# nh273/caro-ai

Hardware: AMD Instinct MI355X
Metric: self-play MCTS node-expansions/sec/GPU (Connect4, 200 sims/move); 1->8 GPU scaling (higher is better)
Workload: dtype f32

## Files before the change

### caro_ai_amd/_lib.py

```python
import ctypes as C
import os

_HERE = os.path.dirname(os.path.abspath(__file__))
LIB_PATH = os.path.join(_HERE, "libcaro_hip.so")
if os.environ.get("CARO_HIP_LIB"):
    LIB_PATH = os.environ["CARO_HIP_LIB"]

GAME_CONNECT4, GAME_MNK, GAME_CARO = 0, 1, 2
RESIGNED = -2


class CaroError(RuntimeError):
    pass


class CaroConfig(C.Structure):
    _fields_ = [
        ("game_kind", C.c_int32), ("n", C.c_int32), ("k", C.c_int32), ("n_games", C.c_int32),
        ("n_stores", C.c_int32), ("n_nets", C.c_int32), ("max_batch", C.c_int32), ("node_cap", C.c_int32),
        ("steps_before_tau_0", C.c_int32), ("first_player_mode", C.c_int32),
        ("c_puct", C.c_float), ("alpha", C.c_double), ("explore", C.c_double),
        ("seed", C.c_uint64), ("uid_base", C.c_uint64), ("uid_stride", C.c_uint64),
        ("device_id", C.c_int32), ("evict", C.c_int32), ("stagger", C.c_int32), ("stagger_recycle", C.c_int32),
        ("games_limit", C.c_int64),
# ... 37 lines not shown
    "caro_leaf_counts": (C.c_int, [_P, _P, _P]),
    "caro_leaf_counts_dev": (C.c_int, [_P, _P]),
    "caro_net_packed_size": (C.c_int64, [C.c_int, C.c_int, C.c_int]),
    "caro_net_create": (C.c_int, [C.c_int, C.c_int, C.c_int, C.c_float, _P, C.c_int64, C.c_int, _P]),
    "caro_net_max_depth": (C.c_int, []),
    "caro_net_packed_size_depth": (C.c_int64, [C.c_int, C.c_int, C.c_int, C.c_int]),
    "caro_net_create_depth": (C.c_int, [C.c_int, C.c_int, C.c_int, C.c_int, C.c_float, _P, C.c_int64, C.c_int, _P]),
    "caro_net_depth": (C.c_int, [_P]),
    "caro_net_winograd_size_depth": (C.c_int64, [C.c_int]),
    "caro_net_winograd2d_size_depth": (C.c_int64, [C.c_int]),
    "caro_net_split_bf16_size_depth": (C.c_int64, [C.c_int]),
    "caro_net_destroy": (None, [_P]),
    "caro_net_enable_winograd": (C.c_int, [_P, _P, C.c_int64]),
    "caro_net_winograd2d_size": (C.c_int, []),
    "caro_net_winograd2d_supported": (C.c_int, [C.c_int, C.c_int]),
    "caro_net_enable_winograd2d": (C.c_int, [_P, _P, C.c_int64]),
    "caro_net_split_bf16_size": (C.c_int64, []),
    "caro_net_enable_split_bf16": (C.c_int, [_P, _P, C.c_int64]),
    "caro_net_boards_per_workgroup": (C.c_int, [_P]),
    "caro_net_uses_slot_list": (C.c_int, [_P]),
    "caro_net_stream_evictions": (C.c_int64, [_P]),
    "caro_net_forward": (C.c_int, [_P, _P, _P, C.c_int, C.c_int64, _P, _P, _P]),
    "caro_stream_create_partition": (C.c_int, [C.c_int, C.c_int, C.c_int, _P]),
    "caro_stream_destroy": (C.c_int, [_P]),
    "caro_search_batch": (C.c_int, [_P, _P, _P, C.c_int, C.c_int, _P, _P, _P, _P, _P, _P]),
    "caro_search_move": (C.c_int, [_P, _P, _P, C.c_int, C.c_int] + [_P] * 10),
    "caro_net_forward_pair": (C.c_int, [_P, _P, _P, _P, C.c_int64, _P, _P, _P]),
    "caro_net_forward_pair_at": (C.c_int, [_P, _P, _P, _P, C.c_int64, C.c_int64, _P, _P, _P]),
    "caro_net_forward_slots": (C.c_int, [_P, _P, _P, _P, _P, C.c_int, C.c_int, _P, _P, _P]),
    "caro_net_forward_slot_list": (C.c_int, [_P, _P, _P, _P, _P, _P, C.c_int, C.c_int, _P, _P, _P]),
    "caro_net_create_hash": (C.c_int, [C.c_int, C.c_int, C.c_int, C.c_uint64, C.c_int, _P]),
    "caro_net_forward_stamped": (C.c_int, [_P, _P, _P, C.c_int, C.c_int64, _P, _P, _P, _P]),
    "caro_net_debug_stamps": (C.c_int, [_P, _P]),
    "caro_get_descent": (C.c_int, [_P, C.c_int, C.c_int, _P, _P, _P, _P, _P, _P]),
    "caro_select_cancel": (C.c_int, [_P]),
    "caro_expand_backup": (C.c_int, [_P, _P, _P, _P]),
    "caro_policy": (C.c_int, [_P, _P, _P, _P]),
    "caro_step": (C.c_int, [_P, _P, _P, _P, _P, _P]),
    "caro_drain_tuples": (C.c_int, [_P, C.c_int64, _P, _P, _P, _P, _P, C.c_int, _P, _P, _P]),
    "caro_drain_tuples_begin": (C.c_int, [_P, C.c_int64, _P, _P, _P, _P, _P, C.c_int, _P]),
    "caro_drain_tuples_end": (C.c_int, [_P, _P, _P]),
    "caro_search_staggered": (C.c_int, [_P, _P, _P, C.c_int, C.c_int, _P, _P, _P, _P, _P]),
    "caro_drain_parked_begin": (C.c_int, [_P, C.c_int64, _P, _P, _P, _P, _P, _P]),
    "caro_engine_set_resign": (C.c_int, [_P, C.c_double, C.c_double]),
    "caro_drain_tuples_begin_q": (C.c_int, [_P, C.c_int64, _P, _P, _P, _P, _P, C.c_int, _P, _P]),
    "caro_drain_parked_begin_q": (C.c_int, [_P, C.c_int64, _P, _P, _P, _P, _P, _P, _P]),
    "caro_engine_set_playout_cap": (C.c_int, [_P, C.c_double, C.c_int]),
    "caro_drain_tuples_begin_x": (C.c_int, [_P, C.c_int64, _P, _P, _P, _P, _P, C.c_int, _P, _P, _P]),
    "caro_drain_parked_begin_x": (C.c_int, [_P, C.c_int64, _P, _P, _P, _P, _P, _P, _P, _P]),
    "caro_engine_set_early_stop": (C.c_int, [_P, C.c_int]),
    "caro_drain_tuples_begin_ex": (C.c_int, [_P, C.c_int64, _P, _P, _P, _P, _P, C.c_int, C.POINTER(CaroDrainExtra), _P]),
    "caro_drain_parked_begin_ex": (C.c_int, [_P, C.c_int64, _P, _P, _P, _P, _P, C.POINTER(CaroDrainExtra), _P]),
    "caro_counters": (C.c_int, [_P, _P, _P]),
    "caro_live_games": (C.c_int, [_P, _P, _P]),
    "caro_pending_leaves": (C.c_int, [_P, _P, _P]),
    "caro_debug_stamps": (C.c_int, [_P, C.c_int]),
    "caro_debug_read": (C.c_int, [_P, _P, C.c_int64, _P]),
    "caro_debug_sqrt_check": (C.c_int, [C.c_uint32, _P]),
    "caro_profile_enable": (C.c_int, [_P, C.c_int]),
    "caro_profile_read": (C.c_int, [_P, _P, _P, C.c_int]),
    "caro_profile_begin": (C.c_int, [_P, C.c_int, _P]),
    "caro_profile_end": (None, [_P, C.c_int, _P]),
    "caro_tree_sizes": (C.c_int, [_P, _P, _P]),
    "caro_tree_live": (C.c_int, [_P, _P, _P]),
    "caro_lookup_nodes": (C.c_int, [_P, C.c_int64] + [_P] * 10),
    "caro_get_roots": (C.c_int, [_P] * 6),
    "caro_poke_nodes": (C.c_int, [_P, C.c_int64] + [_P] * 9),
    "caro_backup_path": (C.c_int, [_P, C.c_int, C.c_int, C.c_float, C.c_int, C.c_int, _P, _P, _P]),
    "caro_dump_tree": (C.c_int, [_P, C.c_int, C.c_int, C.c_int64] + [_P] * 8),
}
EXPORTS = sorted(_SIGNATURES)

_lib = None


def load():
    global _lib
    if _lib is not None:
        return _lib
    if not os.path.exists(LIB_PATH):
        raise CaroError("%s is missing: build it with `python -m caro_ai_amd.build` "
                        "(hipcc --offload-arch=gfx950); there is no CPU fallback" % LIB_PATH)
    try:
        lib = C.CDLL(LIB_PATH)
    except OSError as e:
        raise CaroError("cannot load %s: %s" % (LIB_PATH, e))
    for name, (res, args) in _SIGNATURES.items():
        fn = getattr(lib, name)
        fn.restype = res
        fn.argtypes = args
    _lib = lib
    return lib


def check(rc):
    if rc != 0:
        msg = load().caro_last_error()
        raise CaroError("libcaro_hip error %d: %s" % (rc, msg.decode() if msg else "?"))
```

### caro_ai_amd/csrc/caro_engine.hip

```cpp
#include <hip/hip_runtime.h>

#include <cstddef>
#include <cstdio>
#include <cstdlib>
#include <cstring>
#include <string>
#include <type_traits>
#include <vector>

#include "../../include/caro_hip.h"
#include "../../include/caro_noise.h"
#include "caro_rules.h"
#include "caro_variants.h"

namespace caro {

constexpr uint32_t NSTRONG = 1u << 30;
constexpr uint32_t NMASK = NSTRONG - 1u;
constexpr int ST_DROPPED = 0, ST_TERMINAL = 1, ST_LEAF = 2;
constexpr int MAXB = 64;

enum Counter { C_SIMS, C_LEVELS, C_EXPANSIONS, C_TERMINALS, C_DROPPED, C_OVERFLOW, C_PLIES, C_FINISHED, C_N };

struct View {
  GameParams gp;
  int G, n_stores, n_nets, cap, hcap, A, HW, maxply, maxd, maxB, sbt0, first_mode, ntab, etab;
  int tstride;
  uint32_t slot_rot;
  float c_puct;
  double alpha, explore;
  uint64_t seed, uid_base, uid_stride;
  long long games_limit;
  int32_t* tbl;
  uint64_t* node_key;
  uint32_t* edges;
  int32_t* n_nodes;
  int32_t* n_created;
  uint64_t* root;
  int32_t* player;
  int32_t* ply;
  int32_t* step;
  uint64_t* uid;
  int32_t* done;
  int32_t* result;
  int32_t* final_r;
  int32_t* first;
  uint64_t* h_key;
  int32_t* h_player;
  double* h_pi;
  double* h_q;
  int q_on;
  double resign_t, resign_p;
  int cap_on, cap_fast;
  double cap_p;
  uint8_t* fast;
  uint8_t* h_full;
  int es_on, es_min, ls_M;
  uint8_t* es_cut;
  uint16_t* es_cnt;
  uint16_t* h_mb;
  uint4* d_rec;
  uint4* path_rec;
  uint64_t* d_key;
  int32_t* g_nleaf;
  int32_t* g_off;
  int32_t* g_tree;
  int32_t* g_class;
  int32_t* g_pack;
  int32_t* slot_list;
  int32_t* leaf_count;
  unsigned long long* counters;
  unsigned long long* counters_sum;
  unsigned long long* dbg;
  int stag_S;
  int stag_recycle;
  int stag_pool;
  int32_t* handed;
  int32_t* lm;
  int32_t* pend;
  int32_t* wait;
  int32_t* dirty;
  int32_t* pk_flag;
  int32_t* pk_ply; int32_t* pk_final_r; int32_t* pk_first; int32_t* pk_result; int32_t* pk_step;
  uint64_t* pk_uid;
  uint64_t* ph_key; int32_t* ph_player; double* ph_pi; double* ph_q; uint8_t* ph_full; uint16_t* ph_mb;
  int32_t* dr_off;
  int32_t* dr_gidx;
  int32_t* dr_sel;
  int64_t* dr_tot;
};

template <class R>
__device__ __forceinline__ typename R::Board load_board(const uint64_t* p) {
  typename R::Board b;
#pragma unroll
  for (int i = 0; i < R::KW; ++i) b.w[i] = p[i];
  return b;
}
template <class R>
__device__ __forceinline__ void store_board(uint64_t* p, const typename R::Board& b) {
#pragma unroll
  for (int i = 0; i < R::KW; ++i) p[i] = b.w[i];
}

__device__ __forceinline__ size_t tbase(const View& v, int t) {
  return (size_t)(t * v.ntab + (v.ntab == 2 ? v.tbl[t] : 0)) * (size_t)v.tstride;
}
__device__ __forceinline__ size_t ebase(const View& v, int t) {
  return (size_t)(t * v.etab + (v.etab == 2 ? v.tbl[t] : 0)) * (size_t)v.tstride;
}

constexpr uint64_t EMPTY_KEY = ~0ULL;

template <class R>
__device__ __forceinline__ uint32_t home_slot(const View& v, int t, const typename R::Board& b) {
  return ((uint32_t)R::hash(b) + (uint32_t)t * v.slot_rot) & ((uint32_t)v.hcap - 1u);
}

__device__ __forceinline__ uint8_t cap_is_fast(const View& v, uint64_t uid, int ply) {
  return caro_cap_uniform(v.seed, uid, (uint32_t)ply) < v.cap_p ? 0 : 1;
}
__device__ __forceinline__ void es_ply_start(const View& v, int g) {
  v.es_cut[g] = 0;
  v.es_cnt[g] = 0;
}

template <class GEO>
struct GameRegs {
  typename GEO::R::Board root;
  int done, player, ply, step;
  int tbl[2], nn[2];
  uint64_t uid;
};
template <class GEO>
__device__ __forceinline__ GameRegs<GEO> load_game(const View& v, int g) {
  using R = typename GEO::R;
  GameRegs<GEO> r;
  r.done = v.done[g];
  r.player = v.player[g];
  r.ply = v.ply[g];
  r.step = v.step[g];
  r.uid = v.uid[g];
  r.root = load_board<R>(v.root + (size_t)g * GEO::KW);
#pragma unroll
  for (int st = 0; st < 2; ++st) {
    const int t = g * v.n_stores + (st < v.n_stores ? st : 0);
    r.tbl[st] = v.ntab == 2 ? v.tbl[t] : 0;
    r.nn[st] = v.n_nodes[t];
  }
  return r;
}
__device__ __forceinline__ size_t tbase_sel(const View& v, int t, int sel) {
  return (size_t)(t * v.ntab + sel) * (size_t)v.tstride;
}
__device__ __forceinline__ size_t ebase_sel(const View& v, int t, int sel) {
  return (size_t)(t * v.etab + (v.etab == 2 ? sel : 0)) * (size_t)v.tstride;
}

template <bool ONE>
__device__ __forceinline__ void block_sync() {
  if constexpr (ONE) {
    asm volatile("" ::: "memory");
    __builtin_amdgcn_wave_barrier();
  } else {
    __syncthreads();
  }
}
template <bool ONE>
__device__ __forceinline__ int block_threads() { return ONE ? 64 : (int)blockDim.x; }

template <class R>
__device__ __forceinline__ int probe_from(const View& v, int t, const typename R::Board& b, uint32_t i) {
  const uint32_t mask = (uint32_t)v.hcap - 1u;
  const uint64_t* keys = v.node_key + tbase(v, t) * R::KW;
  for (int it = 0; it < v.hcap; ++it) {
    const uint64_t* k = keys + (size_t)i * R::KW;
    const uint64_t k0 = k[0];
// ... 343 lines not shown
    d.status = ST_TERMINAL;
    d.value = -1.0f;
    return false;
  }
  if (R::full(v.gp, d.cur)) {
    d.status = ST_TERMINAL;
    d.value = 0.0f;
    return false;
  }
  return d.depth < v.maxd;
}

template <class GEO>
__device__ __forceinline__ void early_stop_test(const View& v, int g, int B, int m, bool root_in, const NodeRow<GEO>& r,
                                                int l, int tid) {
  constexpr int LPD = GEO::LPD, APL = GEO::APL;
  int M = v.stag_S ? v.stag_S : v.ls_M;
  if (v.cap_on && v.fast[g]) M = v.cap_fast < M ? v.cap_fast : M;
  if (m < v.es_min || m > M - 2) return;
  int n[APL];
  int ln = -1, la = 0x7fffffff;
#pragma unroll
  for (int j = 0; j < APL; ++j) {
    const int a = l * APL + j;
    n[j] = (root_in && a < v.A) ? (int)(r.nraw[j] & NMASK) : (a < v.A ? 0 : -1);
    if (n[j] > ln) {
      ln = n[j];
      la = a;
    }
  }
  auto imax = [](int x, int y) { return x > y ? x : y; };
  const int n1 = group_allreduce_i32<LPD>(ln, imax);
  const int best = group_allreduce_i32<LPD>(ln == n1 ? la : 0x7fffffff, [](int x, int y) { return x < y ? x : y; });
  int l2 = 0;
#pragma unroll
  for (int j = 0; j < APL; ++j) l2 = (l * APL + j != best && n[j] > l2) ? n[j] : l2;
  const int n2 = group_allreduce_i32<LPD>(l2, imax);
  if (tid == 0 && n1 - n2 > (M - m) * B) v.es_cut[g] = 1;
}

extern __shared__ double caro_dyn_lds[];
template <class GEO>
static inline size_t mail_bytes(int B) {
  return GEO::APL > 1 ? (size_t)((B * GEO::LPD + 63) / 64) * (2 * GEO::AP) * sizeof(double) : 0;
}

template <class GEO>
constexpr int geo_max_batch() { return GEO::LPD >= 64 ? 16 : GEO::LPD >= 32 ? 32 : 64; }

template <class GEO, bool ONE = false>
__device__ __forceinline__ void select_body(const View& v, const GameRegs<GEO>& gr, int B, int mb_index,
                                            const double* __restrict__ noise, int32_t* __restrict__ rows,
                                            float* __restrict__ planes, uint64_t* __restrict__ leaf_keys,
                                            const double* helper_nz = nullptr, volatile int* helper_flag = nullptr) {
  using R = typename GEO::R;
  using Board = typename R::Board;
  constexpr int LPD = GEO::LPD, APL = GEO::APL, AP = GEO::AP, KW = GEO::KW;
  const int g = blockIdx.x;
  const int tid = threadIdx.x;
  const int b = tid / LPD, l = tid % LPD;
  const int first = (tid & 63) - l;

  constexpr int MB = geo_max_batch<GEO>();
  __shared__ uint64_t s_key[MB][KW];
  __shared__ int s_status[MB];
  __shared__ int s_first[MB];
  __shared__ int s_depth[MB];
  __shared__ int s_player[MB];
  __shared__ float s_value[MB];
  __shared__ uint32_t s_dhome[MB];

  if (gr.done || (v.cap_on && !v.stag_S && mb_index >= v.cap_fast && v.fast[g]) ||
      (v.es_on && v.ls_M && mb_index > 0 && v.es_cut[g])) {
    if (tid == 0) {
      v.g_nleaf[g] = 0;
      v.g_class[g] = 0;
      if (rows) v.g_pack[g] = 0;
    }
    return;
  }
  unsigned long long st0 = 0, st_noise = 0, st_root = 0, st_loop = 0;
  if (v.dbg) st0 = __builtin_amdgcn_s_memtime();
  Descent<GEO> d;
  d.cur = gr.root;
  d.aux = R::aux_of(v.gp, d.cur);
  d.lk = R::lane_k(v.gp, l);
  const int player0 = gr.player;
  d.player = player0;
  d.depth = 0;
  d.status = ST_LEAF;
  d.value = 0.0f;
  d.home = 0u;
  const int st_sel = v.n_stores == 2 ? player0 : 0;
  const int t = g * v.n_stores + st_sel;
  const int A = v.A;
  uint4* prec = v.path_rec + ((size_t)g * v.maxB + b) * v.maxd;
  const int tsel = st_sel ? gr.tbl[1] : gr.tbl[0];
  const size_t tb = tbase_sel(v, t, tsel);
  const uint64_t* tkeys = v.node_key + tb * KW;
  const uint32_t* tedges = v.edges + ebase_sel(v, t, tsel) * 4 * AP;

  NodeRow<GEO> r;
  load_row<GEO, true>(r, tkeys, tedges, home_slot<R>(v, t, d.cur), l);
  double nz[APL];
  if (noise) {
#pragma unroll
    for (int j = 0; j < APL; ++j) {
      const int a = l * APL + j;
      nz[j] = a < A ? noise[((size_t)g * B + b) * A + a] : 0.0;
    }
  } else if (helper_nz) {
    while (*helper_flag == 0) __builtin_amdgcn_s_sleep(2);
    __builtin_amdgcn_fence(__ATOMIC_ACQUIRE, "workgroup");
#pragma unroll
    for (int j = 0; j < APL; ++j) nz[j] = helper_nz[b * AP + l * APL + j];
  } else {
    const uint64_t key = caro_noise_key(v.seed, gr.uid, (uint32_t)gr.ply, (uint32_t)(mb_index * B + b));
    noise_group<LPD, APL>(key, l, A, v.alpha, nz, APL > 1 ? caro_dyn_lds + (tid >> 6) * (2 * AP) : nullptr);
  }
  if (v.dbg) st_noise = __builtin_amdgcn_s_memtime();

  constexpr int PREC_LDS = GEO::APL > 1 ? 1 : 512;
  __shared__ uint4 s_prec[PREC_LDS];
  const bool stage = B * v.maxd <= PREC_LDS;
  uint4* lprec = stage ? s_prec + b * v.maxd : nullptr;
  bool live = descend_level<GEO, true>(v, d, t, tkeys, tedges, prec, lprec, l, first, nz, r);
  if (v.es_on) {
    if (tid == 0) {
      v.es_cnt[g] = (uint16_t)(mb_index + 1);
      if (v.ls_M && mb_index == 0) v.es_cut[g] = 0;
    }
    if (v.sbt0 == 0 || gr.step >= v.sbt0) early_stop_test<GEO>(v, g, B, mb_index, d.depth > 0, r, l, tid);
  }
  if (v.dbg) st_root = __builtin_amdgcn_s_memtime();
  while (live) live = descend_level<GEO, false>(v, d, t, tkeys, tedges, prec, lprec, l, first, nullptr, r);
  if (stage) {
    __builtin_amdgcn_wave_barrier();
    for (int i = l; i < d.depth; i += LPD) prec[i] = s_prec[b * v.maxd + i];
  }
  if (v.dbg) st_loop = __builtin_amdgcn_s_memtime();

  if constexpr (ONE) {
    const bool head = l == 0;
    const int st = d.status;
    bool dup = false;
    for (int o = 0; o < B; ++o) {
      const int src = o * LPD;
      bool eq = o < b && __builtin_amdgcn_readlane(st, src) == ST_LEAF;
#pragma unroll
      for (int w = 0; w < KW; ++w) {
        const uint32_t lo = (uint32_t)__builtin_amdgcn_readlane((int)(uint32_t)d.cur.w[w], src);
        const uint32_t hi = (uint32_t)__builtin_amdgcn_readlane((int)(uint32_t)(d.cur.w[w] >> 32), src);
        eq = eq && ((((uint64_t)hi << 32) | lo) == d.cur.w[w]);
      }
      dup = dup || eq;
    }
    const bool first_seen = st == ST_LEAF && !dup;
    const unsigned long long m_first = __ballot(head && first_seen);
    const unsigned long long m_term = __ballot(head && st == ST_TERMINAL);
    const unsigned long long m_drop = __ballot(head && st == ST_LEAF && dup);
    const int my_rank = __popcll(m_first & ((1ull << tid) - 1ull));
    const int levels = group_sum_i32<64>(head ? d.depth : 0);
    int maxdep = 0;
    if (v.dbg) maxdep = group_allreduce_i32<64>(d.depth, [](int x, int y) { return x > y ? x : y; });
    if (head) {
      const size_t di = (size_t)g * v.maxB + b;
      const uint32_t stw = (uint32_t)((st == ST_LEAF && dup) ? ST_DROPPED : st);
      v.d_rec[di] = make_uint4(stw | ((uint32_t)d.depth << 8) | ((uint32_t)my_rank << 16) | ((uint32_t)d.player << 24),
                               __float_as_uint(d.value), d.home, 0u);
      store_board<R>(v.d_key + di * KW, d.cur);
    }
    const int nleaf = __popcll(m_first);
    if (tid == 0) {
      v.g_nleaf[g] = nleaf;
      v.g_tree[g] = t;
      v.g_class[g] = v.n_nets == 2 ? player0 : 0;
      if (v.dbg) {
        unsigned long long* dd = v.dbg + (size_t)g * 8;
        dd[0] = st_noise - st0; dd[1] = st_root - st0; dd[2] = st_loop - st0;
        dd[3] = __builtin_amdgcn_s_memtime() - st0; dd[4] = (unsigned long long)maxdep;
      }
      unsigned long long* ctr = v.counters + (size_t)g * C_N;
      atomicAdd(ctr + C_SIMS, (unsigned long long)B);
      atomicAdd(ctr + C_LEVELS, (unsigned long long)levels);
      atomicAdd(ctr + C_TERMINALS, (unsigned long long)__popcll(m_term));
      atomicAdd(ctr + C_DROPPED, (unsigned long long)__popcll(m_drop));
      if (rows) {
        const int cls = v.n_nets == 2 ? player0 : 0;
        if (nleaf) atomicAdd(rows + cls, nleaf);
        v.g_off[g] = g * B;
        v.g_pack[g] = nleaf | (cls << 8);
      }
    }
    if (rows) {
      const int HW = v.HW;
      int local = 0;
      typename R::PlaneAt pat[R::PLANE_ITEMS];
#pragma unroll
      for (int k = 0; k < R::PLANE_ITEMS; ++k) pat[k] = R::plane_at(v.gp, tid + 64 * k < 2 * HW ? tid + 64 * k : 0);
      for (unsigned long long m = m_first; m; m &= m - 1ull) {
        const int src = __ffsll(m) - 1;
        Board brd;
#pragma unroll
        for (int w = 0; w < KW; ++w) {
          const uint32_t lo = (uint32_t)__builtin_amdgcn_readlane((int)(uint32_t)d.cur.w[w], src);
          const uint32_t hi = (uint32_t)__builtin_amdgcn_readlane((int)(uint32_t)(d.cur.w[w] >> 32), src);
          brd.w[w] = ((uint64_t)hi << 32) | lo;
        }
        const int who = __builtin_amdgcn_readlane(d.player, src);
        const int rowi = g * B + local++;
        float* dst = planes + (size_t)rowi * 2 * HW;
#pragma unroll
        for (int k = 0; k < R::PLANE_ITEMS; ++k)
          if (tid + 64 * k < 2 * HW) dst[tid + 64 * k] = R::plane_val(brd, who, pat[k]);
        if (leaf_keys && tid < KW) {
          uint64_t kw = brd.w[0];
#pragma unroll
          for (int w = 1; w < KW; ++w) kw = tid == w ? brd.w[w] : kw;
          leaf_keys[(size_t)rowi * KW + tid] = kw;
        }
      }
    }
    return;
  }
  if (l == 0) {
#pragma unroll
    for (int w = 0; w < KW; ++w) s_key[b][w] = d.cur.w[w];
    s_status[b] = d.status;
    s_depth[b] = d.depth;
    s_player[b] = d.player;
    s_value[b] = d.value;
    s_dhome[b] = d.home;
  }
  block_sync<ONE>();
  if (tid < 64) {
    const int bb = tid;
    const bool mine = bb < B;
    const int st = mine ? s_status[bb] : ST_DROPPED;
    const int dep = mine ? s_depth[bb] : 0;
    Board key;
#pragma unroll
    for (int w = 0; w < KW; ++w) key.w[w] = mine ? s_key[bb][w] : 0ull;
    bool dup = false;
// ... 121 lines not shown
    const int who = (int)(rx >> 24);
    float* dst = planes + (size_t)rowi * 2 * HW;
    for (int i = tid; i < 2 * HW; i += blockDim.x) dst[i] = R::plane(v.gp, brd, who, i / HW, i % HW);
    if (leaf_keys && tid < KW) leaf_keys[(size_t)rowi * KW + tid] = v.d_key[di * KW + tid];
  }
}

template <int AP>
__device__ __forceinline__ void backup_path(const View& v, int t, float value, bool strong_val, const int32_t* pn,
                                            const int32_t* pa, int len) {
  float cur = -value;
  for (int i = len - 1; i >= 0; --i) {
    uint32_t* row = v.edges + (ebase(v, t) + pn[i]) * 4 * AP;
    const int a = pa[i];
    const uint32_t nraw = row[4 * a];
    const int n = (int)(nraw & NMASK) + 1;
    const uint32_t strong = (nraw & NSTRONG) | (strong_val ? NSTRONG : 0u);
    const float w = __uint_as_float(row[4 * a + 1]) + cur;
    const float q = w / (float)n;
    row[4 * a] = (uint32_t)n | strong;
    row[4 * a + 1] = __float_as_uint(w);
    row[4 * a + 2] = __float_as_uint(q);
    cur = -cur;
  }
}
template <int AP>
__device__ __forceinline__ void backup_path_rec(const View& v, int t, float value, bool strong_val, const uint4* rec,
                                                int len) {
  float cur = -value;
  for (int i = len - 1; i >= 0; --i) {
    const uint32_t na = rec[i].x;
    uint32_t* row = v.edges + (ebase(v, t) + (na & 0xFFFFFFu)) * 4 * AP;
    const int a = (int)(na >> 24);
    const uint32_t nraw = row[4 * a];
    const int n = (int)(nraw & NMASK) + 1;
    const uint32_t strong = (nraw & NSTRONG) | (strong_val ? NSTRONG : 0u);
    const float w = __uint_as_float(row[4 * a + 1]) + cur;
    row[4 * a] = (uint32_t)n | strong;
    row[4 * a + 1] = __float_as_uint(w);
    row[4 * a + 2] = __float_as_uint(w / (float)n);
    cur = -cur;
  }
}

template <class GEO>
struct ExpandPre {
  static constexpr int NPR = (MAXB * 0 + 64 * GEO::APL + 63) / 64;
  uint4 rec;
  typename GEO::R::Board brd;
  float row_val;
  uint4 p0, p1;
  float pr[NPR];
  int nleaf;
};
template <class GEO, bool ONE>
__device__ __forceinline__ ExpandPre<GEO> expand_preload(const View& v, int g, int B, int off, const float* __restrict__ probs,
                                                         const float* __restrict__ values) {
  using R = typename GEO::R;
  constexpr int KW = GEO::KW, AP = GEO::AP;
  ExpandPre<GEO> e;
  const int lane = threadIdx.x;
  e.nleaf = v.g_nleaf[g];
  e.rec = make_uint4(ST_DROPPED, 0u, 0u, 0u);
  e.row_val = 0.f;
#pragma unroll
  for (int w = 0; w < KW; ++w) e.brd.w[w] = 0;
  if (lane < B) {
    const size_t di = (size_t)g * v.maxB + lane;
    e.rec = v.d_rec[di];
    e.brd = load_board<R>(v.d_key + di * KW);
    if ((long long)off + lane < (long long)v.G * v.maxB) e.row_val = values[off + lane];
  }
  e.p0 = e.p1 = make_uint4(0u, 0u, 0u, 0u);
  if (B <= 8 && lane < 64 && (lane >> 3) < B) {
    const uint4* pr = v.path_rec + ((size_t)g * v.maxB + (lane >> 3)) * v.maxd;
    if ((lane & 7) < v.maxd) e.p0 = pr[lane & 7];
    if (8 + (lane & 7) < v.maxd) e.p1 = pr[8 + (lane & 7)];
  }
#pragma unroll
  for (int k = 0; k < ExpandPre<GEO>::NPR; ++k) {
    e.pr[k] = 0.f;
    if (ONE) {
      const int idx = lane + 64 * k, b = idx / AP, a = idx - b * AP;
      if (idx < B * AP && a < v.A && lane < 64) e.pr[k] = probs[(size_t)(off + b) * v.A + a];
    }
  }
  return e;
}

template <class GEO, bool ONE = false>
__device__ __forceinline__ void expand_body(const View& v, GameRegs<GEO>& gr, int B, const ExpandPre<GEO>& pre, int off,
                                            const float* __restrict__ probs) {
  using R = typename GEO::R;
  using Board = typename R::Board;
  constexpr int AP = GEO::AP, KW = GEO::KW;
  constexpr int MAXE = GEO::APL > 1 ? 256 : 512;
  constexpr int MAXB = geo_max_batch<GEO>();
  __shared__ int e_node[MAXE];
  __shared__ short e_act[MAXE];
  __shared__ float e_val[MAXE];
  __shared__ unsigned char e_strong[MAXE];
  __shared__ uint32_t e_n[MAXE], e_w[MAXE];
  __shared__ int s_total;
  __shared__ uint64_t s_brd[MAXB][KW];
  __shared__ int s_node[MAXB], s_row[MAXB];
  __shared__ uint32_t s_home[MAXB];
  __shared__ unsigned char s_free[MAXB];
  __shared__ int q_len[MAXB], q_off[MAXB], q_b[MAXB];
  __shared__ float q_val[MAXB];
  __shared__ unsigned char q_strong[MAXB];
  __shared__ int s_nq;
  __shared__ uint4 s_p0[64], s_p1[64];
  __shared__ float s_rowval[MAXB];
  const int g = blockIdx.x;
  if (gr.done) return;
  const int lane = threadIdx.x;
  unsigned long long* xs = v.dbg ? v.dbg + ((size_t)v.G + g) * 8 : nullptr;
#define CARO_XS(n) if (xs && lane == 0) xs[n] = __builtin_amdgcn_s_memtime();
  CARO_XS(0)
  const int st_sel = v.n_stores == 2 ? gr.player : 0;
  const int t = g * v.n_stores + st_sel;
  const int nleaf = pre.nleaf;
  const int base = st_sel ? gr.nn[1] : gr.nn[0];
  const bool overflow = base + nleaf > v.cap;
  const int A = v.A;
  const int tsel = st_sel ? gr.tbl[1] : gr.tbl[0];
  const size_t tb = tbase_sel(v, t, tsel);
  const size_t eb = ebase_sel(v, t, tsel);
  const int my_st = (int)(pre.rec.x & 0xFFu), my_len = (int)((pre.rec.x >> 8) & 0xFFu);
  const int my_local = (int)((pre.rec.x >> 16) & 0xFFu);
  const uint32_t my_home = pre.rec.z;
  float my_val = __uint_as_float(pre.rec.y);
  const Board& brd = pre.brd;
  const bool pre_paths = B <= 8 && block_threads<ONE>() >= 64;
  if (pre_paths && lane < 64) {
    s_p0[lane] = pre.p0;
    s_p1[lane] = pre.p1;
  }
  const bool is_leaf = lane < B && my_st == ST_LEAF && !overflow;
  if (lane < B) s_rowval[lane] = pre.row_val;
  block_sync<ONE>();
  if (lane < B) {
    s_node[lane] = -2;
    if (is_leaf) {
      my_val = s_rowval[my_local];
      s_home[lane] = my_home & 0x7fffffffu;
      s_free[lane] = (my_home >> 31) != 0u;
      s_row[lane] = off + my_local;
      s_node[lane] = -1;
#pragma unroll
      for (int w = 0; w < KW; ++w) s_brd[lane][w] = brd.w[w];
    }
  }
  block_sync<ONE>();
  CARO_XS(1)
  const bool whole_wave = ONE || blockDim.x >= 64;
  const bool wave0 = whole_wave && lane < 64;
  if (!overflow) {
    if (wave0) {
      bool clash = false;
      for (int bb = 0; bb < B; ++bb) {
        const int ob = __builtin_amdgcn_readlane((int)is_leaf, bb);
        const uint32_t oh = (uint32_t)__builtin_amdgcn_readlane((int)(my_home & 0x7fffffffu), bb);
        clash = clash || (bb < lane && ob && oh == (my_home & 0x7fffffffu));
      }
      const bool fast = is_leaf && (my_home >> 31) != 0u && !clash;
      if (fast) {
        uint64_t* k = v.node_key + (tb + (my_home & 0x7fffffffu)) * KW;
#pragma unroll
        for (int w = KW - 1; w >= 0; --w) k[w] = brd.w[w];
        s_node[lane] = (int)(my_home & 0x7fffffffu);
      }
      const unsigned long long slow = __ballot(is_leaf && !fast);
      if (slow) {
        asm volatile("" ::: "memory");
        __builtin_amdgcn_wave_barrier();
        if (lane == 0)
          for (unsigned long long m = slow; m; m &= m - 1ull) {
            const int b = __ffsll(m) - 1;
            Board lb;
#pragma unroll
            for (int w = 0; w < KW; ++w) lb.w[w] = s_brd[b][w];
            s_node[b] = insert_key<R>(v, t, lb);
          }
      }
    } else if (!whole_wave && lane == 0) {
      for (int b = 0; b < B; ++b) {
        if (s_node[b] == -2) continue;
        Board lb;
#pragma unroll
        for (int w = 0; w < KW; ++w) lb.w[w] = s_brd[b][w];
        s_node[b] = insert_key<R>(v, t, lb);
      }
    }
    if (lane == 0) {
      unsigned long long* ctr = v.counters + (size_t)g * C_N;
      v.n_nodes[t] = base + nleaf;
      atomicAdd(v.n_created + t, nleaf);
      atomicAdd(ctr + C_EXPANSIONS, (unsigned long long)nleaf);
    }
    if (st_sel) gr.nn[1] = base + nleaf;
    else gr.nn[0] = base + nleaf;
  } else if (lane == 0) {
    atomicAdd(v.counters + (size_t)g * C_N + C_OVERFLOW, 1ull);
  }
  CARO_XS(2)
  const unsigned long long m_term = __ballot(lane < B && my_st == ST_TERMINAL);
  const unsigned long long m_leaf = __ballot(is_leaf);
  const int n_term = __popcll(m_term);
  const unsigned long long below = (1ull << lane) - 1ull;
  int qpos = -1;
  if (lane < B && my_st == ST_TERMINAL) qpos = __popcll(m_term & below);
  else if (is_leaf) qpos = n_term + __popcll(m_leaf & below);
  if (qpos >= 0) {
    q_len[qpos] = my_len;
    q_b[qpos] = lane;
    q_val[qpos] = my_val;
    q_strong[qpos] = my_st == ST_LEAF;
  }
  if (lane == 0) s_nq = n_term + __popcll(m_leaf);
  block_sync<ONE>();
  const int nq = s_nq;
  if (lane == 0) {
    int acc = 0;
    for (int k = 0; k < nq; ++k) {
      q_off[k] = acc;
      acc += q_len[k];
    }
    s_total = acc;
  }
  block_sync<ONE>();
  CARO_XS(3)
  const int total = s_total;
  if (total <= MAXE)
    for (int j = lane; j < total; j += block_threads<ONE>()) {
      int k = 0;
      while (k + 1 < nq && q_off[k + 1] <= j) ++k;
      const int r = j - q_off[k];
      const int i = q_len[k] - 1 - r;
      uint4 rec;
      if (pre_paths && i < 8) rec = s_p0[q_b[k] * 8 + i];
      else if (pre_paths && i < 16) rec = s_p1[q_b[k] * 8 + i - 8];
      else rec = v.path_rec[((size_t)g * v.maxB + q_b[k]) * v.maxd + i];
      e_node[j] = (int)(rec.x & 0xFFFFFFu);
      e_act[j] = (short)(rec.x >> 24);
      e_n[j] = rec.y;
      e_w[j] = rec.z;
      e_val[j] = (r & 1) ? q_val[k] : -q_val[k];
      e_strong[j] = q_strong[k];
    }
  CARO_XS(4)
  if (!overflow)
    for (int idx = lane; idx < B * AP; idx += block_threads<ONE>()) {
      const int b = idx / AP, a = idx - b * AP;
      const int node = s_node[b];
      float pv = 0.f;
      if (ONE) {
        const int src = node >= 0 ? (s_row[b] - off) * AP + a : lane;
#pragma unroll
        for (int k = 0; k < ExpandPre<GEO>::NPR; ++k) {
          const float x = __shfl(pre.pr[k], src & 63, 64);
          pv = (src >> 6) == k ? x : pv;
        }
      } else if (node >= 0 && a < A) {
        pv = probs[(size_t)s_row[b] * A + a];
      }
      if (node < 0) continue;
      uint32_t* row = v.edges + (eb + node) * 4 * AP;
      if (a >= A) pv = 0.f;
      reinterpret_cast<uint4*>(row)[a] = make_uint4(0u, 0u, 0u, __float_as_uint(pv));
    }
  if (total > MAXE) {
    if (lane == 0)
      for (int k = 0; k < nq; ++k) {
        const size_t di = (size_t)g * v.maxB + q_b[k];
        backup_path_rec<AP>(v, t, q_val[k], q_strong[k] != 0, v.path_rec + di * v.maxd, q_len[k]);
      }
    return;
  }
  block_sync<ONE>();
  CARO_XS(5)
  const int n = total;
  if (whole_wave && n <= 128) {
    if (wave0) {
    const int j0 = lane, j1 = lane + 64;
    const bool v0 = j0 < n, v1 = j1 < n;
    const int key0 = v0 ? (e_node[j0] << 8) | (int)(unsigned short)e_act[j0] : -1;
    const int key1 = v1 ? (e_node[j1] << 8) | (int)(unsigned short)e_act[j1] : -1;
    unsigned long long todo0 = __ballot(v0), todo1 = __ballot(v1);
    bool own0 = false, own1 = false;
    unsigned long long g0m0 = 0ull, g0m1 = 0ull, g1m1 = 0ull;
    while (todo0 | todo1) {
      const bool lo = todo0 != 0ull;
      const int lead = lo ? __ffsll((unsigned long long)todo0) - 1 : __ffsll((unsigned long long)todo1) - 1;
      const int k = lo ? __builtin_amdgcn_readlane(key0, lead) : __builtin_amdgcn_readlane(key1, lead);
      const unsigned long long m0 = __ballot(v0 && key0 == k);
      const unsigned long long m1 = __ballot(v1 && key1 == k);
      if (lane == lead) {
        if (lo) { own0 = true; g0m0 = m0; g0m1 = m1; }
        else { own1 = true; g1m1 = m1; }
      }
      todo0 &= ~m0;
      todo1 &= ~m1;
    }
    uint32_t* row0 = own0 ? v.edges + (eb + (key0 >> 8)) * 4 * AP : nullptr;
    uint32_t* row1 = own1 ? v.edges + (eb + (key1 >> 8)) * 4 * AP : nullptr;
    const int a0 = key0 & 0xff, a1 = key1 & 0xff;
    if (own0) {
      const uint32_t n0 = e_n[j0];
      int cnt = (int)(n0 & NMASK);
      uint32_t strong = n0 & NSTRONG;
      float w = __uint_as_float(e_w[j0]);
      for (unsigned long long m = g0m0; m; m &= m - 1ull) {
        const int e = __ffsll(m) - 1;
        cnt += 1;
        w = w + e_val[e];
        if (e_strong[e]) strong = NSTRONG;
      }
      for (unsigned long long m = g0m1; m; m &= m - 1ull) {
        const int e = 64 + __ffsll(m) - 1;
        cnt += 1;
        w = w + e_val[e];
        if (e_strong[e]) strong = NSTRONG;
      }
// ... 22 lines not shown
    const int node = e_node[j], a = e_act[j];
    bool owner = true;
    for (int k = 0; k < j; ++k) owner = owner && !(e_node[k] == node && e_act[k] == a);
    if (!owner) continue;
    uint32_t* row = v.edges + (eb + node) * 4 * AP;
    const uint32_t nraw = e_n[j];
    int cnt = (int)(nraw & NMASK);
    uint32_t strong = nraw & NSTRONG;
    float w = __uint_as_float(e_w[j]);
    for (int k = j; k < n; ++k) {
      if (e_node[k] == node && e_act[k] == a) {
        cnt += 1;
        w = w + e_val[k];
        if (e_strong[k]) strong = NSTRONG;
      }
    }
    row[4 * a] = (uint32_t)cnt | strong;
    row[4 * a + 1] = __float_as_uint(w);
    row[4 * a + 2] = __float_as_uint(w / (float)cnt);
  }
  CARO_XS(6)
  if (xs && lane == 0) xs[7] = (unsigned long long)total;
#undef CARO_XS
}

template <class GEO>
__global__ void k_expand_backup(View v, const float* __restrict__ probs, const float* __restrict__ values) {
  GameRegs<GEO> gr = load_game<GEO>(v, blockIdx.x);
  const int B = v.leaf_count[2], off = v.g_off[blockIdx.x];
  const ExpandPre<GEO> pre = expand_preload<GEO, false>(v, blockIdx.x, B, off, probs, values);
  expand_body<GEO>(v, gr, B, pre, off, probs);
}

template <class GEO>
__device__ __forceinline__ void noise_wave(const View& v, int B, int go, uint64_t uid, uint32_t ply, int mb,
                                           double* s_nz, volatile int* s_flag) {
  constexpr int LPD = GEO::LPD, APL = GEO::APL, AP = GEO::AP;
  const int lane = threadIdx.x & 63;
  const int b = lane / LPD, l = lane % LPD;
  if (go) {
    double nz[APL];
    const uint64_t key = caro_noise_key(v.seed, uid, ply, (uint32_t)(mb * B + b));
    __shared__ double s_mail[APL > 1 ? 2 * AP : 1];
    noise_group<LPD, APL>(key, l, v.A, v.alpha, nz, s_mail);
#pragma unroll
    for (int j = 0; j < APL; ++j) s_nz[b * AP + l * APL + j] = nz[j];
  }
  __builtin_amdgcn_fence(__ATOMIC_RELEASE, "workgroup");
  __builtin_amdgcn_wave_barrier();
  if (lane == 0) *s_flag = 1;
}

template <class GEO>
__global__ void k_tree(View v, int B, int mb_index, const double* __restrict__ noise, const float* __restrict__ probs,
                       const float* __restrict__ values, float* __restrict__ planes, uint64_t* __restrict__ leaf_keys,
                       int32_t* __restrict__ rows_cur, int32_t* __restrict__ rows_next, int do_expand,
                       int do_select) {
  __shared__ double s_nz[MAXB * 0 + 64 * GEO::APL];
  __shared__ int s_flag;
  if (threadIdx.x == 0) s_flag = 0;
  __syncthreads();
  if (threadIdx.x >= 64) {
    const int g = blockIdx.x;
    const int go = do_select && !noise && !v.done[g] && !(v.cap_on && mb_index >= v.cap_fast && v.fast[g]) &&
                   !(v.es_on && mb_index > 0 && v.es_cut[g]);
    noise_wave<GEO>(v, B, go, go ? v.uid[g] : 0ull, go ? (uint32_t)v.ply[g] : 0u, mb_index, s_nz, &s_flag);
    return;
  }
  __builtin_amdgcn_s_setprio(3);
  if (blockIdx.x == 0 && threadIdx.x == 0) {
    rows_next[0] = 0;
    rows_next[1] = 0;
    rows_next[2] = B;
    rows_cur[2] = B;
  }
  unsigned long long t0 = 0;
  if (v.dbg) t0 = __builtin_amdgcn_s_memtime();
  GameRegs<GEO> gr = load_game<GEO>(v, blockIdx.x);
  const ExpandPre<GEO> pre = expand_preload<GEO, true>(v, blockIdx.x, B, blockIdx.x * B, probs, values);
  if (do_expand) {
    expand_body<GEO, true>(v, gr, B, pre, blockIdx.x * B, probs);
    block_sync<true>();
  }
  const unsigned long long t1 = v.dbg ? __builtin_amdgcn_s_memtime() : 0;
  if (v.dbg && threadIdx.x == 0 && !do_select) v.dbg[(size_t)blockIdx.x * 8 + 5] = t1 - t0;
  if (do_select) select_body<GEO, true>(v, gr, B, mb_index, noise, rows_cur, planes, leaf_keys, s_nz, &s_flag);
  if (v.dbg && threadIdx.x == 0 && do_select) {
    v.dbg[(size_t)blockIdx.x * 8 + 6] = t1 - t0;
    v.dbg[(size_t)blockIdx.x * 8 + 7] = __builtin_amdgcn_s_memtime() - t0;
  }
}

template <class GEO>
__device__ __forceinline__ void root_policy(const View& v, int g, int t, const typename GEO::R::Board& root,
                                            double* s_pi, int* s_n) {
  using R = typename GEO::R;
  constexpr int AP = GEO::AP;
  const int node = probe<R>(v, t, root);
  for (int a = threadIdx.x; a < AP; a += blockDim.x)
    s_n[a] = (node >= 0 && a < v.A) ? (int)(v.edges[((ebase(v, t) + node) * AP + a) * 4] & NMASK) : 0;
  __syncthreads();
  __shared__ int s_best;
  __shared__ double s_total;
  if (threadIdx.x == 0) {
    const int tau = (v.sbt0 > 0 && v.step[g] < v.sbt0) ? 1 : 0;
    int best = 0;
    long long tot = 0;
    for (int a = 0; a < v.A; ++a) {
      if (s_n[a] > s_n[best]) best = a;
      tot += s_n[a];
    }
    s_best = tau == 0 ? best : -1;
    s_total = (double)tot;
  }
  __syncthreads();
  for (int a = threadIdx.x; a < AP; a += blockDim.x) {
    double p = 0.0;
    if (a < v.A) p = s_best >= 0 ? (a == s_best ? 1.0 : 0.0) : (double)s_n[a] / s_total;
    s_pi[a] = p;
  }
  __syncthreads();
}

template <class GEO>
__global__ void k_policy(View v, double* __restrict__ pi_out, int32_t* __restrict__ counts_out) {
  using R = typename GEO::R;
  constexpr int AP = GEO::AP, KW = GEO::KW;
  __shared__ double s_pi[AP];
  __shared__ int s_n[AP];
  const int g = blockIdx.x;
  const typename R::Board root = load_board<R>(v.root + (size_t)g * KW);
  const int t = g * v.n_stores + (v.n_stores == 2 ? v.player[g] : 0);
  root_policy<GEO>(v, g, t, root, s_pi, s_n);
  for (int a = threadIdx.x; a < v.A; a += blockDim.x) {
    if (pi_out) pi_out[(size_t)g * v.A + a] = s_pi[a];
    if (counts_out) counts_out[(size_t)g * v.A + a] = s_n[a];
  }
}

// ... 417 lines not shown
    v.pk_step[g] = gr.step;
    v.pk_uid[g] = uid;
    v.pk_flag[g] = 1;
  }
  block_sync<ONE>();
  if (!v.stag_recycle || v.stag_pool || !game_wanted(v, g, uid + v.uid_stride)) {
    if (threadIdx.x == 0) v.done[g] = 2;
    gr.done = 2;
    return false;
  }
  const uint64_t nuid = uid + v.uid_stride;
  const int fp = v.first_mode == 2 ? (int)(nuid & 1ull) : v.first_mode;
  gr.root = R::initial(v.gp);
  gr.player = fp;
  gr.ply = 0;
  gr.step = 0;
  gr.uid = nuid;
  gr.done = 0;
  const bool flip = v.etab != 2;
#pragma unroll
  for (int st = 0; st < 2; ++st) {
    if (flip) gr.tbl[st] = 1 - gr.tbl[st];
    gr.nn[st] = 0;
  }
  if (threadIdx.x == 0) {
#pragma unroll
    for (int st = 0; st < 2; ++st) {
      if (st < v.n_stores) {
        const int t = g * v.n_stores + st;
        if (flip) {
          v.tbl[t] = gr.tbl[st];
          v.dirty[t] = 1;
        }
        v.n_nodes[t] = 0;
        v.n_created[t] = 0;
      }
    }
    store_board<R>(v.root + (size_t)g * KW, gr.root);
    v.player[g] = fp;
    v.first[g] = fp;
    v.ply[g] = 0;
    v.step[g] = 0;
    v.uid[g] = nuid;
    v.done[g] = 0;
    v.result[g] = 0;
    v.final_r[g] = 0;
    if (v.cap_on) v.fast[g] = cap_is_fast(v, nuid, 0);
    if (v.es_on) es_ply_start(v, g);
  }
  return true;
}

template <class GEO>
__global__ void k_tree_stag(View v, int B, const float* __restrict__ probs, const float* __restrict__ values,
                            float* __restrict__ planes, uint64_t* __restrict__ leaf_keys,
                            int32_t* __restrict__ rows_cur, int32_t* __restrict__ rows_next) {
  constexpr int AP = GEO::AP;
  __shared__ double s_pi[AP];
  __shared__ int s_n[AP];
  __shared__ double s_nz[64 * GEO::APL];
  __shared__ int s_flag;
  const int g = blockIdx.x;
  if (threadIdx.x == 0) s_flag = 0;
  const int w = v.wait[g];
  int lm = v.lm[g];
  const int pend = v.pend[g];
  const int due = (v.cap_on && v.fast[g]) ? v.cap_fast : v.stag_S;
  const int cut = v.es_on ? v.es_cut[g] : 0;
  GameRegs<GEO> gr = load_game<GEO>(v, g);
  ExpandPre<GEO> pre;
  if (threadIdx.x < 64) pre = expand_preload<GEO, true>(v, g, B, g * B, probs, values);
  __syncthreads();
  if (threadIdx.x >= 64) {
    const int go = w == 0 && gr.done == 0;
    int lm_h = go ? lm : 0;
    uint32_t ply_h = go ? (uint32_t)gr.ply : 0u;
    if (lm_h >= due || (go && cut)) {
      lm_h = 0;
      ply_h += 1u;
    }
    noise_wave<GEO>(v, B, go, go ? gr.uid : 0ull, ply_h, lm_h, s_nz, &s_flag);
    return;
  }
  __builtin_amdgcn_s_setprio(3);
  if (blockIdx.x == 0 && threadIdx.x == 0) {
    rows_next[0] = 0;
    rows_next[1] = 0;
    rows_next[2] = B;
    rows_cur[2] = B;
  }
  const unsigned long long t0 = v.dbg ? __builtin_amdgcn_s_memtime() : 0;
  if (w > 0) {
    if (threadIdx.x == 0) {
      v.wait[g] = w - 1;
      v.g_nleaf[g] = 0;
      v.g_class[g] = 0;
      v.g_pack[g] = 0;
    }
    return;
  }
  if (gr.done == 2) {
    if (threadIdx.x == 0) {
      v.g_nleaf[g] = 0;
      v.g_class[g] = 0;
      v.g_pack[g] = 0;
    }
    return;
  }
  if (pend) {
    expand_body<GEO, true>(v, gr, B, pre, g * B, probs);
    block_sync<true>();
  }
  const unsigned long long t1 = v.dbg ? __builtin_amdgcn_s_memtime() : 0;
  int over = gr.done == 1;
  if (!over && (lm >= due || cut)) {
    over = step_body<GEO, true>(v, g, gr, nullptr, s_pi, s_n, nullptr, nullptr, nullptr);
    lm = 0;
  }
  if (over) {
    if (park_and_restart<GEO>(v, g, gr)) over = 0;
  }
  const unsigned long long t2 = v.dbg ? __builtin_amdgcn_s_memtime() : 0;
  select_body<GEO, true>(v, gr, B, lm, nullptr, rows_cur, planes, leaf_keys, s_nz, &s_flag);
  if (threadIdx.x == 0) {
    v.lm[g] = over ? 0 : lm + 1;
    v.pend[g] = over ? 0 : 1;
    if (v.dbg) {
      v.dbg[(size_t)g * 8 + 5] = ((t2 - t1) & 0xFFFFFFull) | (__builtin_amdgcn_s_memrealtime() << 24);
      v.dbg[(size_t)g * 8 + 6] = t1 - t0;
      v.dbg[(size_t)g * 8 + 7] = __builtin_amdgcn_s_memtime() - t0;
      v.dbg[(size_t)g * 8 + 4] |= (unsigned long long)__builtin_amdgcn_s_getreg((31 << 11) | 4) << 8;
    }
  }
}

template <class GEO>
__global__ void k_tree_stag_mw(View v, int B, const float* __restrict__ probs, const float* __restrict__ values,
                               float* __restrict__ planes, uint64_t* __restrict__ leaf_keys,
                               int32_t* __restrict__ rows_cur, int32_t* __restrict__ rows_next) {
  constexpr int AP = GEO::AP;
  __shared__ double s_pi[AP];
  __shared__ int s_n[AP];
  const int g = blockIdx.x;
  if (g == 0 && threadIdx.x == 0) {
    rows_next[0] = 0;
    rows_next[1] = 0;
    rows_next[2] = B;
    rows_cur[2] = B;
  }
  const int w = v.wait[g];
  int lm = v.lm[g];
  const int pend = v.pend[g];
  const int due = (v.cap_on && v.fast[g]) ? v.cap_fast : v.stag_S;
  const int cut = v.es_on ? v.es_cut[g] : 0;
  GameRegs<GEO> gr = load_game<GEO>(v, g);
  const ExpandPre<GEO> pre = expand_preload<GEO, false>(v, g, B, g * B, probs, values);
  __syncthreads();
  if (w > 0 || gr.done == 2) {
    if (threadIdx.x == 0) {
      if (w > 0) v.wait[g] = w - 1;
      v.g_nleaf[g] = 0;
      v.g_class[g] = 0;
      v.g_pack[g] = 0;
    }
    return;
  }
  if (pend) {
    expand_body<GEO, false>(v, gr, B, pre, g * B, probs);
    __syncthreads();
  }
  int over = gr.done == 1;
  if (!over && (lm >= due || cut)) {
    over = step_body<GEO>(v, g, gr, nullptr, s_pi, s_n, nullptr, nullptr, nullptr);
    lm = 0;
    if (v.etab == 2) {
      __syncthreads();
// ... 426 lines not shown
template <class GEO>
__global__ void k_noise(uint64_t seed, long long M, int A, double alpha, const uint64_t* uid, const uint32_t* ply,
                        const uint32_t* sim, double* out) {
  constexpr int LPD = GEO::LPD, APL = GEO::APL;
  const int grp = threadIdx.x / LPD, l = threadIdx.x % LPD;
  const long long m = (long long)blockIdx.x * (blockDim.x / LPD) + grp;
  const long long mm = m < M ? m : M - 1;
  const uint64_t key = caro_noise_key(seed, uid[mm], ply[mm], sim[mm]);
  double nz[APL];
  __shared__ double s_mail[APL > 1 ? 2 * GEO::AP : 1];
  noise_group<LPD, APL>(key, l, A, alpha, nz, s_mail);
  if (m < M)
    for (int j = 0; j < APL; ++j) {
      const int a = l * APL + j;
      if (a < A) out[(size_t)m * A + a] = nz[j];
    }
}

}

using namespace caro;

static thread_local std::string g_err;
static int fail(int code, const std::string& msg) {
  g_err = msg;
  return code;
}
#define HIPCHK(x)                                                                                  \
  do {                                                                                             \
    hipError_t e_ = (x);                                                                           \
    if (e_ != hipSuccess)                                                                          \
      return fail(CARO_E_HIP, std::string(#x) + ": " + hipGetErrorString(e_));                     \
  } while (0)

struct caro_engine {
  caro_config cfg;
  Variant var;
  View v;
  std::vector<void*> allocs;
  int32_t* pinned;
  int64_t* pinned64;
  int32_t* scratch;
  int32_t* live;
  int select_pending;
  int drain_pending;
  int ls_mid;
  int stag_batch;
  hipEvent_t drain_ev;
  int prof_on;
  int prof_gate;
  uint64_t prof_ctr;
  uint64_t prof_cal;
  int32_t* rows;
  int rows_par;
  int fused_ok;
  std::vector<hipEvent_t> ev;
  std::vector<int> ev_kind;
  size_t ev_used;
  double prof_ms[8];
  long long prof_n[8];
};

constexpr unsigned PROF_EVERY = 23;
enum ProfKind { PK_SELECT = 0, PK_COMPACT = 1, PK_EXPAND = 2, PK_STEP = 3, PK_NET = 4, PK_NULL1 = 5, PK_NULL2 = 6, PK_N = 8 };
__global__ void k_prof_null() {}
static void prof_calibrate(caro_engine* h, hipStream_t st);

static void prof_flush(caro_engine* h) {
  for (size_t i = 0; i < h->ev_used; ++i) {
    float ms = 0.f;
    if (hipEventSynchronize(h->ev[2 * i + 1]) == hipSuccess &&
        hipEventElapsedTime(&ms, h->ev[2 * i], h->ev[2 * i + 1]) == hipSuccess) {
      h->prof_ms[h->ev_kind[i]] += ms;
      h->prof_n[h->ev_kind[i]] += 1;
    }
  }
  h->ev_used = 0;
}
static int prof_begin(caro_engine* h, int kind, hipStream_t st) {
  if (!h->prof_on || !h->prof_gate) return -1;
  if (h->ev_used * 2 + 2 > h->ev.size()) {
    if (h->ev.size() >= 2 * 16384) prof_flush(h);
    else
      for (int i = 0; i < 512; ++i) {
        hipEvent_t e;
        if (hipEventCreate(&e) != hipSuccess) return -1;
        h->ev.push_back(e);
      }
  }
  const int i = (int)h->ev_used++;
  if ((size_t)i >= h->ev_kind.size()) h->ev_kind.resize(i + 1);
  h->ev_kind[i] = kind;
  (void)hipEventRecord(h->ev[2 * i], st);
  return i;
}
static void prof_end(caro_engine* h, int i, hipStream_t st) {
  if (i >= 0) (void)hipEventRecord(h->ev[2 * i + 1], st);
}
static void prof_calibrate(caro_engine* h, hipStream_t st) {
  if (!h->prof_on || !h->prof_gate || (h->prof_cal++ & 3)) return;
  const int a = prof_begin(h, PK_NULL1, st);
  hipLaunchKernelGGL(k_prof_null, dim3(1), dim3(64), 0, st);
  prof_end(h, a, st);
  const int b = prof_begin(h, PK_NULL2, st);
  hipLaunchKernelGGL(k_prof_null, dim3(1), dim3(64), 0, st);
  hipLaunchKernelGGL(k_prof_null, dim3(1), dim3(64), 0, st);
  prof_end(h, b, st);
}

template <class T>
static int dalloc(caro_engine* h, T** p, size_t n) {
  void* q = nullptr;
  hipError_t e = hipMalloc(&q, n * sizeof(T) + 256);
  if (e != hipSuccess) return fail(CARO_E_NOMEM, std::string("hipMalloc failed: ") + hipGetErrorString(e));
  h->allocs.push_back(q);
  *p = (T*)q;
  return 0;
}

extern "C" {

const char* caro_last_error(void) { return g_err.c_str(); }
void caro__set_error(const char* msg) { g_err = msg ? msg : ""; }
int caro_version(void) { return 101; }

#include "caro_host.inc"

int caro_rules_move_batch(int kind, int n, int k, int64_t M, uint64_t* keys, const int32_t* moves,
                          const int32_t* players, int32_t* won, int32_t* full, void* stream) {
  const Variant var = pick_variant(kind, n);
  const GameParams gp = make_gp(kind, n, k);
  if (M <= 0) return 0;
  const unsigned grid = (unsigned)((M + 255) / 256);
  DISPATCH(var, hipLaunchKernelGGL(k_rules_move<GEO>, dim3(grid), dim3(256), 0, (hipStream_t)stream, gp,
                                   (long long)M, keys, moves, players, won, full));
  HIPCHK(hipGetLastError());
  return 0;
}
int caro_rules_legal_batch(int kind, int n, int k, int64_t M, const uint64_t* keys, uint8_t* legal, void* stream) {
  const Variant var = pick_variant(kind, n);
  const GameParams gp = make_gp(kind, n, k);
  if (M <= 0) return 0;
  const unsigned grid = (unsigned)((M * gp.A + 255) / 256);
  DISPATCH(var, hipLaunchKernelGGL(k_rules_legal<GEO>, dim3(grid), dim3(256), 0, (hipStream_t)stream, gp,
                                   (long long)M, keys, legal));
  HIPCHK(hipGetLastError());
  return 0;
}
int caro_rules_encode_batch(int kind, int n, int k, int64_t M, const uint64_t* keys, const int32_t* who,
                            float* planes, void* stream) {
  const Variant var = pick_variant(kind, n);
  const GameParams gp = make_gp(kind, n, k);
  if (M <= 0) return 0;
  const unsigned grid = (unsigned)((M * 2 * gp.rows * gp.cols + 255) / 256);
  DISPATCH(var, hipLaunchKernelGGL(k_rules_encode<GEO>, dim3(grid), dim3(256), 0, (hipStream_t)stream, gp,
                                   (long long)M, keys, who, planes));
  HIPCHK(hipGetLastError());
  return 0;
}
int caro_noise_batch(uint64_t seed, int64_t M, int A, double alpha, const uint64_t* uid, const uint32_t* ply,
                     const uint32_t* sim, double* out, void* stream) {
  if (M <= 0) return 0;
  Variant var = A == 7 ? V_C4 : A <= 16 ? V_M16 : A <= 32 ? V_M32 : A <= 64 ? V_M64 : A <= 128 ? V_M128 : V_M256;
  if (A > 256) return fail(CARO_E_INVAL, "A out of range");
  const int lpd = variant_lpd(var);
  const int per_block = 64 / lpd;
  const unsigned grid = (unsigned)((M + per_block - 1) / per_block);
  DISPATCH(var, hipLaunchKernelGGL(k_noise<GEO>, dim3(grid), dim3(64), 0, (hipStream_t)stream, seed, (long long)M, A,
                                   alpha, uid, ply, sim, out));
  HIPCHK(hipGetLastError());
  return 0;
}

static int reset_games_impl(caro_engine* h, const int32_t* first_player_dev, void* stream);
static void apply_run_params(caro_engine* h, const caro_config* cfg) {
  View& v = h->v;
  v.sbt0 = cfg->steps_before_tau_0;
  v.first_mode = cfg->first_player_mode;
  v.c_puct = cfg->c_puct;
  v.alpha = cfg->alpha;
  v.explore = cfg->explore;
  v.seed = cfg->seed;
  v.uid_base = cfg->uid_base;
  v.uid_stride = cfg->uid_stride ? cfg->uid_stride : (uint64_t)cfg->n_games;
  v.games_limit = cfg->games_limit > 0 ? (long long)cfg->games_limit : 0;
  if (cfg->stagger > 0) {
    v.stag_S = cfg->stagger;
    v.stag_recycle = cfg->stagger_recycle ? 1 : 0;
    v.stag_pool = (cfg->stagger_recycle == 2 && cfg->games_limit > 0) ? 1 : 0;
  }
}
static int fresh_state(caro_engine* h, hipStream_t st) {
  View& v = h->v;
  const size_t T = (size_t)v.G * v.n_stores, G = (size_t)v.G;
  HIPCHK(hipMemsetAsync(v.counters, 0, sizeof(unsigned long long) * C_N * G, st));
  HIPCHK(hipMemsetAsync(v.leaf_count, 0, sizeof(int32_t) * 4, st));
  HIPCHK(hipMemsetAsync(h->rows, 0, sizeof(int32_t) * 8, st));
  HIPCHK(hipMemsetAsync(v.g_nleaf, 0, sizeof(int32_t) * G, st));
  HIPCHK(hipMemsetAsync(v.g_pack, 0, sizeof(int32_t) * G, st));
  h->rows_par = 0;
  h->stag_batch = 0;
  const int rc = reset_games_impl(h, nullptr, st);
  if (rc) return rc;
  if (v.stag_S) {
    HIPCHK(hipMemsetAsync(v.dirty, 0, sizeof(int32_t) * T, st));
    hipLaunchKernelGGL(k_stag_init, dim3((v.G + 255) / 256), dim3(256), 0, st, v);
    HIPCHK(hipGetLastError());
  }
  return 0;
}
int caro_engine_create(const caro_config* cfg, caro_engine** out) {
  if (!cfg || !out) return fail(CARO_E_INVAL, "null argument");
  const Variant var = pick_variant(cfg->game_kind, cfg->n);
  if (var == V_BAD) return fail(CARO_E_INVAL, "unsupported game (connect four, or m,n,k / caro with 2 <= n <= 15)");
  if (cfg->n_games < 1) return fail(CARO_E_INVAL, "n_games must be >= 1");
  if (cfg->n_stores != 1 && cfg->n_stores != 2) return fail(CARO_E_INVAL, "n_stores must be 1 or 2");
  if (cfg->n_nets != 1 && cfg->n_nets != 2) return fail(CARO_E_INVAL, "n_nets must be 1 or 2");
  const int lpd = variant_lpd(var);
  if (cfg->max_batch < 1 || cfg->max_batch > MAXB || cfg->max_batch * lpd > 1024)
    return fail(CARO_E_INVAL, "max_batch out of range for this game (batch * lanes-per-descent <= 1024, batch <= 64)");
  if ((cfg->game_kind == CARO_GAME_MNK || cfg->game_kind == CARO_GAME_CARO) && (cfg->k < 2 || cfg->k > cfg->n))
    return fail(CARO_E_INVAL, "k must satisfy 2 <= k <= n");
  if (cfg->stagger < 0) return fail(CARO_E_INVAL, "stagger must be >= 0");
  if (cfg->stagger > 0) {
    if (cfg->max_batch * lpd < 64 || (cfg->max_batch * lpd) % 64 != 0)
      return fail(CARO_E_INVAL, "staggered mode needs whole wavefronts per game (max_batch x lanes per descent a multiple of 64)");
    if (cfg->evict && cfg->max_batch * lpd == 64)
      return fail(CARO_E_INVAL, "staggered mode with eviction: the multi-wavefront kernel only (max_batch x lanes per descent > 64)");
  }
  int ndev = 0;
  if (hipGetDeviceCount(&ndev) != hipSuccess || ndev <= 0)
    return fail(CARO_E_NODEV, "no HIP device: libcaro_hip needs a GPU (there is no CPU fallback)");
  if (cfg->device_id < 0 || cfg->device_id >= ndev) return fail(CARO_E_INVAL, "device_id out of range");
  HIPCHK(hipSetDevice(cfg->device_id));

  caro_engine* h = new caro_engine();
  h->cfg = *cfg;
  h->var = var;
  h->select_pending = 0;
  h->ls_mid = 0;
  h->prof_on = 0;
  h->prof_gate = 1;
  h->prof_ctr = 0;
  h->prof_cal = 0;
  h->rows = nullptr;
  h->rows_par = 0;
  {
    const char* e = getenv("CARO_NO_FUSED_TREE");
    h->fused_ok = !(e && e[0] == '1');
  }
  h->ev_used = 0;
  for (int i = 0; i < 8; ++i) { h->prof_ms[i] = 0; h->prof_n[i] = 0; }
  View& v = h->v;
  memset(&v, 0, sizeof v);
  v.gp = make_gp(cfg->game_kind, cfg->n, cfg->k);
  v.G = cfg->n_games;
  v.n_stores = cfg->n_stores;
  v.n_nets = cfg->n_nets;
  v.A = v.gp.A;
  v.HW = v.gp.rows * v.gp.cols;
  v.maxply = v.HW;
  v.maxd = v.HW;
  v.maxB = cfg->max_batch;
  v.ntab = (cfg->evict || cfg->stagger > 0) ? 2 : 1;
  v.etab = cfg->evict ? 2 : 1;
  apply_run_params(h, cfg);
  v.cap = cfg->node_cap > 0 ? cfg->node_cap : 4096;
  static_assert(MAXB <= 255, "leaf rank travels in 8 bits of d_rec.x");
  if (v.cap > (1 << 23)) { delete h; return fail(CARO_E_INVAL, "node_cap too large: at most 2^23 nodes per tree (slot ids travel in 24 bits)"); }
  int hc = 64;
  while (hc < 2 * v.cap) hc <<= 1;
  v.hcap = hc;
  if (v.A > 256 || v.maxd > 255) { delete h; return fail(CARO_E_INVAL, "board too large for the path records (actions < 256, depth <= 255)"); }
  {
    const char* e = getenv("CARO_TREE_SKEW");
    const long skew = e ? strtol(e, nullptr, 0) : 0;
    if (skew < 0 || skew > 65536) { delete h; return fail(CARO_E_INVAL, "CARO_TREE_SKEW must be 0 .. 65536 slots"); }
    v.tstride = hc + (int)skew;
    e = getenv("CARO_SLOT_ROT");
    v.slot_rot = e ? (uint32_t)strtoul(e, nullptr, 0) : 0u;
  }
  const int KW = variant_kw(var), AP = variant_ap(var);
  const size_t T = (size_t)v.G * v.n_stores, G = (size_t)v.G;
  int rc = 0;
#define DA(p, n) if ((rc = dalloc(h, &p, (n))) != 0) { caro_engine_destroy(h); return rc; }
  DA(v.tbl, T);
  DA(v.node_key, T * v.ntab * v.tstride * KW);
  DA(v.edges, T * v.etab * v.tstride * 4 * AP);
  DA(v.n_nodes, T);
  DA(v.n_created, T);
  DA(v.root, G * KW);
  DA(v.player, G); DA(v.ply, G); DA(v.step, G); DA(v.uid, G); DA(v.done, G); DA(v.result, G); DA(v.final_r, G);
  DA(v.first, G);
  DA(v.h_key, G * v.maxply * KW);
  DA(v.h_player, G * v.maxply);
  DA(v.h_pi, G * v.maxply * v.A);
  DA(v.path_rec, G * v.maxB * v.maxd);
  DA(v.d_rec, G * v.maxB);
  DA(v.d_key, G * v.maxB * KW);
  DA(v.g_nleaf, G); DA(v.g_off, G); DA(v.g_tree, G); DA(v.g_class, G); DA(v.g_pack, G);
  DA(v.slot_list, 2 * G * v.maxB);
  DA(v.leaf_count, 4);
  DA(v.counters, G * C_N);
  DA(v.counters_sum, C_N);
  DA(v.dr_off, G); DA(v.dr_gidx, G); DA(v.dr_sel, G); DA(v.dr_tot, 2);
  DA(h->scratch, (size_t)v.maxd + 8);
  DA(h->live, 1);
  DA(h->rows, 8);
  if (cfg->stagger > 0) {
    DA(v.lm, G); DA(v.pend, G); DA(v.wait, G); DA(v.dirty, T);
    DA(v.pk_flag, G); DA(v.pk_ply, G); DA(v.pk_final_r, G); DA(v.pk_first, G); DA(v.pk_result, G); DA(v.pk_step, G);
    DA(v.pk_uid, G);
    DA(v.handed, 1);
    DA(v.ph_key, G * v.maxply * KW);
    DA(v.ph_player, G * v.maxply);
    DA(v.ph_pi, G * v.maxply * v.A);
  }
#undef DA
  HIPCHK(hipHostMalloc((void**)&h->pinned, 64, hipHostMallocDefault));
  HIPCHK(hipHostMalloc((void**)&h->pinned64, 128, hipHostMallocDefault));
  *out = h;
  rc = fresh_state(h, nullptr);
  if (rc) { caro_engine_destroy(h); *out = nullptr; return rc; }
  HIPCHK(hipDeviceSynchronize());
  return 0;
}

int caro_engine_restart(caro_engine* h, const caro_config* cfg, void* stream) {
  if (!h || !cfg) return fail(CARO_E_INVAL, "null argument");
  const caro_config& o = h->cfg;
  if (cfg->game_kind != o.game_kind || cfg->n != o.n || cfg->k != o.k || cfg->n_games != o.n_games ||
      cfg->n_stores != o.n_stores || cfg->n_nets != o.n_nets || cfg->max_batch != o.max_batch ||
      cfg->node_cap != o.node_cap || (cfg->evict != 0) != (o.evict != 0) || cfg->device_id != o.device_id ||
      (cfg->stagger > 0) != (o.stagger > 0))
    return fail(CARO_E_INVAL, "caro_engine_restart: the configuration differs from the engine's in a field that shapes its "
                              "memory (game, n_games, n_stores, n_nets, max_batch, node_cap, evict, device, staggered or not)");
  if (cfg->stagger < 0) return fail(CARO_E_INVAL, "stagger must be >= 0");
  if (h->drain_pending) return fail(CARO_E_STATE, "caro_engine_restart with a drain pending (caro_drain_tuples_end first)");
  if (h->select_pending) return fail(CARO_E_STATE, "caro_engine_restart with a pending caro_select");
  HIPCHK(hipSetDevice(o.device_id));
  h->cfg = *cfg;
  apply_run_params(h, cfg);
  return fresh_state(h, (hipStream_t)stream);
}

int caro_engine_set_resign(caro_engine* h, double threshold, double playthrough) {
  if (!h) return fail(CARO_E_INVAL, "null engine");
  if (!(threshold >= -1.0 && threshold <= 1.0)) return fail(CARO_E_INVAL, "resign threshold must be in [-1, 1]");
  if (!(playthrough >= 0.0 && playthrough <= 1.0)) return fail(CARO_E_INVAL, "resign playthrough must be in [0, 1]");
  View& v = h->v;
  if (!v.q_on) {
    HIPCHK(hipSetDevice(h->cfg.device_id));
    const size_t n = (size_t)v.G * v.maxply;
    int rc = dalloc(h, &v.h_q, n);
    if (rc) return rc;
    HIPCHK(hipMemset(v.h_q, 0, n * sizeof(double)));
    if (v.stag_S) {
      if ((rc = dalloc(h, &v.ph_q, n)) != 0) return rc;
      HIPCHK(hipMemset(v.ph_q, 0, n * sizeof(double)));
    }
    v.q_on = 1;
  }
  v.resign_t = threshold;
  v.resign_p = playthrough;
  return 0;
}

int caro_engine_set_playout_cap(caro_engine* h, double p_full, int fast) {
  if (!h) return fail(CARO_E_INVAL, "null engine");
  if (!(p_full >= 0.0 && p_full <= 1.0)) return fail(CARO_E_INVAL, "playout cap p_full must be in [0, 1]");
  if (fast < 2) return fail(CARO_E_INVAL, "playout cap fast must be >= 2 (a fast first ply must expand its root)");
  View& v = h->v;
  if (v.stag_S && fast > v.stag_S) return fail(CARO_E_INVAL, "playout cap fast must be <= caro_config.stagger");
// ... 83 lines not shown
  return 0;
}

static int select_impl(caro_engine* h, int batch, int mb_index, int budget, const double* noise, float* planes,
                       uint64_t* leaf_keys, void* stream);
int caro_select(caro_engine* h, int batch, int mb_index, const double* noise, float* planes, uint64_t* leaf_keys,
                void* stream) {
  return select_impl(h, batch, mb_index, 0, noise, planes, leaf_keys, stream);
}
static int select_impl(caro_engine* h, int batch, int mb_index, int budget, const double* noise, float* planes,
                       uint64_t* leaf_keys, void* stream) {
  if (!h || !planes) return fail(CARO_E_INVAL, "null argument");
  if (batch < 1 || batch > h->v.maxB) return fail(CARO_E_INVAL, "batch exceeds max_batch of the engine");
  if (h->v.stag_S) return fail(CARO_E_STATE, "caro_select: the engine runs in staggered mode (per-game clocks, pending minibatches, parked games); use caro_search_staggered / caro_drain_parked_begin");
  if (h->select_pending) return fail(CARO_E_STATE, "caro_select called twice without caro_expand_backup");
  const int lpd = variant_lpd(h->var);
  hipStream_t st = (hipStream_t)stream;
  const int p0 = prof_begin(h, PK_SELECT, st);
  View sv = h->v;
  sv.ls_M = budget;
  DISPATCH(h->var, hipLaunchKernelGGL(k_select<GEO>, dim3(h->v.G), dim3(batch * lpd), mail_bytes<GEO>(batch), st, sv,
                                      batch, mb_index, noise));
  prof_end(h, p0, st);
  const int p1 = prof_begin(h, PK_COMPACT, st);
  DISPATCH(h->var, hipLaunchKernelGGL(k_encode<GEO>, dim3(h->v.G), dim3(128), 0, st, h->v, batch, planes, leaf_keys));
  prof_end(h, p1, st);
  HIPCHK(hipGetLastError());
  h->select_pending = 1;
  h->ls_mid = 1;
  return 0;
}

int caro_leaf_counts(caro_engine* h, int32_t counts[2], void* stream) {
  if (!h || !counts) return fail(CARO_E_INVAL, "null argument");
  HIPCHK(hipMemcpyAsync(h->pinned, h->v.leaf_count, 2 * sizeof(int32_t), hipMemcpyDeviceToHost, (hipStream_t)stream));
  HIPCHK(hipStreamSynchronize((hipStream_t)stream));
  counts[0] = h->pinned[0];
  counts[1] = h->pinned[1];
  return 0;
}

int caro_expand_backup(caro_engine* h, const float* probs, const float* values, void* stream) {
  if (!h) return fail(CARO_E_INVAL, "null engine");
  if (!h->select_pending) return fail(CARO_E_STATE, "caro_expand_backup without a pending caro_select");
  const int p0 = prof_begin(h, PK_EXPAND, (hipStream_t)stream);
  DISPATCH(h->var, hipLaunchKernelGGL(k_expand_backup<GEO>, dim3(h->v.G), dim3(64), 0, (hipStream_t)stream, h->v,
                                      probs, values));
  prof_end(h, p0, (hipStream_t)stream);
  HIPCHK(hipGetLastError());
  h->select_pending = 0;
  return 0;
}

static int search_batch_impl(caro_engine* h, caro_net* net0, caro_net* net1, int searches, int batch, const double* noise,
                             float* planes, uint64_t* leaf_keys, float* probs, float* values, void* stream, int with_step,
                             const double* uniforms, int32_t* actions, int32_t* done, int32_t* result) {
  if (!h || !net0 || !planes || !probs || !values) return fail(CARO_E_INVAL, "null argument");
  if (h->v.n_nets == 2 && !net1) return fail(CARO_E_INVAL, "engine has two nets, net1 is null");
  if (searches < 1) return fail(CARO_E_INVAL, "searches must be >= 1");
  const int64_t max_rows = (int64_t)h->v.G * batch;
  const size_t noise_stride = (size_t)h->v.G * batch * h->v.A;
  if (batch < 1 || batch > h->v.maxB) return fail(CARO_E_INVAL, "batch exceeds max_batch of the engine");
  if (h->v.stag_S) return fail(CARO_E_STATE, "caro_search_batch: the engine runs in staggered mode (per-game clocks, pending minibatches, parked games); use caro_search_staggered / caro_drain_parked_begin");
  if (h->select_pending) return fail(CARO_E_STATE, "caro_search_batch with a pending caro_select");
  hipStream_t st = (hipStream_t)stream;
  const int bthreads = batch * variant_lpd(h->var);
  const bool fused1 = h->fused_ok && bthreads == 64;
  const bool fused = h->fused_ok && bthreads >= 64 && bthreads % 64 == 0;
  h->ls_mid = 1;
  View sv = h->v;
  sv.ls_M = searches;
  if (!caro_net_uses_slot_list(net0)) sv.slot_list = nullptr;
  for (int mb = 0; mb < searches; ++mb) {
    h->prof_gate = (h->prof_ctr++ % PROF_EVERY) == 0;
    int rc = 0;
    const int32_t* counts = h->v.leaf_count;
    if (fused) {
      int32_t* cur = h->rows + 4 * h->rows_par;
      int32_t* nxt = h->rows + 4 * (h->rows_par ^ 1);
      h->rows_par ^= 1;
      counts = cur;
      const int p1 = prof_begin(h, PK_SELECT, st);
      if (fused1) {
        DISPATCH(h->var, hipLaunchKernelGGL(k_tree<GEO>, dim3(h->v.G), dim3(128), 0, st, sv, batch, mb,
                                            noise ? noise + (size_t)mb * noise_stride : nullptr, probs, values, planes,
                                            leaf_keys, cur, nxt, mb > 0 ? 1 : 0, 1));
      } else {
        DISPATCH(h->var, hipLaunchKernelGGL(k_tree_mw<GEO>, dim3(h->v.G), dim3(bthreads), mail_bytes<GEO>(batch), st,
                                            sv, batch, mb, noise ? noise + (size_t)mb * noise_stride : nullptr, probs,
                                            values, planes, leaf_keys, cur, nxt, mb > 0 ? 1 : 0, 1, 0,
                                            (const double*)nullptr, (int32_t*)nullptr, (int32_t*)nullptr,
                                            (int32_t*)nullptr));
      }
      prof_end(h, p1, st);
      if (hipGetLastError() != hipSuccess) { h->prof_gate = 1; return fail(CARO_E_HIP, "k_tree launch failed"); }
    } else {
      rc = select_impl(h, batch, mb, searches, noise ? noise + (size_t)mb * noise_stride : nullptr, planes, leaf_keys,
                       stream);
      if (rc) { h->prof_gate = 1; return rc; }
    }
    const int p0 = prof_begin(h, PK_NET, st);
    if (fused)
      rc = caro_net_forward_slot_list(net0, h->v.n_nets == 2 ? net1 : nullptr, planes, counts, h->v.g_pack,
                                      fused1 ? nullptr : sv.slot_list, h->v.G, batch, probs, values, stream);
    else if (h->v.n_nets == 2)
      rc = caro_net_forward_pair_at(net0, net1, planes, counts, -1, max_rows, probs, values, stream);
    else rc = caro_net_forward(net0, planes, counts, 0, max_rows, probs, values, stream);
    prof_end(h, p0, st);
    prof_calibrate(h, st);
    if (!rc && !fused) rc = caro_expand_backup(h, probs, values, stream);
    if (rc) { h->prof_gate = 1; return rc; }
  }
  if (fused) {
    int32_t* cur = h->rows + 4 * h->rows_par;
    int32_t* nxt = h->rows + 4 * (h->rows_par ^ 1);
    h->rows_par ^= 1;
    const int p1 = prof_begin(h, PK_EXPAND, st);
    if (fused1) {
      DISPATCH(h->var, hipLaunchKernelGGL(k_tree<GEO>, dim3(h->v.G), dim3(128), 0, st, h->v, batch, searches,
                                          (const double*)nullptr, probs, values, planes, leaf_keys, cur, nxt, 1, 0));
    } else {
      DISPATCH(h->var, hipLaunchKernelGGL(k_tree_mw<GEO>, dim3(h->v.G), dim3(bthreads), 0, st, h->v, batch, searches,
                                          (const double*)nullptr, probs, values, planes, leaf_keys, cur, nxt, 1, 0,
                                          with_step ? 1 : 0, uniforms, actions, done, result));
      if (with_step) {
        with_step = 0;
        h->ls_mid = 0;
      }
    }
    prof_end(h, p1, st);
    if (hipGetLastError() != hipSuccess) { h->prof_gate = 1; return fail(CARO_E_HIP, "k_tree launch failed"); }
  }
  h->prof_gate = 1;
  return with_step ? caro_step(h, uniforms, actions, done, result, stream) : 0;
}

int caro_search_batch(caro_engine* h, caro_net* net0, caro_net* net1, int searches, int batch, const double* noise,
                      float* planes, uint64_t* leaf_keys, float* probs, float* values, void* stream) {
  return search_batch_impl(h, net0, net1, searches, batch, noise, planes, leaf_keys, probs, values, stream, 0, nullptr,
                           nullptr, nullptr, nullptr);
}

int caro_search_move(caro_engine* h, caro_net* net0, caro_net* net1, int searches, int batch, const double* noise,
                     const double* uniforms, float* planes, uint64_t* leaf_keys, float* probs, float* values,
                     int32_t* actions, int32_t* done, int32_t* result, void* stream) {
  return search_batch_impl(h, net0, net1, searches, batch, noise, planes, leaf_keys, probs, values, stream, 1, uniforms,
                           actions, done, result);
}

int caro_search_staggered(caro_engine* h, caro_net* net0, caro_net* net1, int launches, int batch, float* planes,
                          uint64_t* leaf_keys, float* probs, float* values, void* stream) {
  if (!h || !net0 || !planes || !probs || !values) return fail(CARO_E_INVAL, "null argument");
  if (!h->v.stag_S) return fail(CARO_E_STATE, "the engine was not created in staggered mode (caro_config.stagger)");
  if (h->v.n_nets == 2 && !net1) return fail(CARO_E_INVAL, "engine has two nets, net1 is null");
  if (launches < 1) return fail(CARO_E_INVAL, "launches must be >= 1");
  const int bthreads = batch * variant_lpd(h->var);
  if (batch < 1 || batch > h->v.maxB || bthreads < 64 || bthreads % 64 != 0)
    return fail(CARO_E_INVAL, "staggered mode: batch x lanes per descent must be a multiple of 64");
  if (h->cfg.evict && bthreads == 64)
    return fail(CARO_E_INVAL, "staggered mode with eviction: batch x lanes per descent must be above 64");
  if (h->stag_batch && h->stag_batch != batch) return fail(CARO_E_INVAL, "staggered mode: the batch size is fixed by the first call");
  h->stag_batch = batch;
  hipStream_t st = (hipStream_t)stream;
  View sv = h->v;
  if (!caro_net_uses_slot_list(net0)) sv.slot_list = nullptr;
  for (int j = 0; j < launches; ++j) {
    h->prof_gate = (h->prof_ctr++ % PROF_EVERY) == 0;
    int32_t* cur = h->rows + 4 * h->rows_par;
    int32_t* nxt = h->rows + 4 * (h->rows_par ^ 1);
    h->rows_par ^= 1;
    const int p1 = prof_begin(h, PK_SELECT, st);
    if (bthreads == 64) {
      DISPATCH(h->var, hipLaunchKernelGGL(k_tree_stag<GEO>, dim3(h->v.G), dim3(128), 0, st, h->v, batch, probs, values,
                                          planes, leaf_keys, cur, nxt));
    } else {
      DISPATCH(h->var, hipLaunchKernelGGL(k_tree_stag_mw<GEO>, dim3(h->v.G), dim3(bthreads), mail_bytes<GEO>(batch), st,
                                          sv, batch, probs, values, planes, leaf_keys, cur, nxt));
    }
    prof_end(h, p1, st);
    if (hipGetLastError() != hipSuccess) { h->prof_gate = 1; return fail(CARO_E_HIP, "k_tree_stag launch failed"); }
    const int p0 = prof_begin(h, PK_NET, st);
    const int rc = caro_net_forward_slot_list(net0, h->v.n_nets == 2 ? net1 : nullptr, planes, cur, h->v.g_pack,
                                              bthreads == 64 ? nullptr : sv.slot_list, h->v.G, batch, probs, values,
                                              stream);
    prof_end(h, p0, st);
    prof_calibrate(h, st);
    if (rc) { h->prof_gate = 1; return rc; }
    if (h->v.stag_pool && j % 5 == 4)
      DISPATCH(h->var, hipLaunchKernelGGL(k_stag_assign<GEO>, dim3(1), dim3(1024), 0, st, h->v));
  }
  h->prof_gate = 1;
  return 0;
}

int caro_drain_parked_begin(caro_engine* h, int64_t cap, uint64_t* states, int32_t* players, double* pi, int32_t* z,
                            int64_t* games, void* stream) {
  return caro_drain_parked_begin_q(h, cap, states, players, pi, z, games, nullptr, stream);
}
int caro_drain_parked_begin_q(caro_engine* h, int64_t cap, uint64_t* states, int32_t* players, double* pi, int32_t* z,
                              int64_t* games, double* root_q, void* stream) {
  return caro_drain_parked_begin_x(h, cap, states, players, pi, z, games, root_q, nullptr, stream);
}
int caro_drain_parked_begin_x(caro_engine* h, int64_t cap, uint64_t* states, int32_t* players, double* pi, int32_t* z,
                              int64_t* games, double* root_q, uint8_t* full, void* stream) {
  caro_drain_extra ex = {(uint32_t)sizeof(caro_drain_extra), root_q, full, nullptr};
  return caro_drain_parked_begin_ex(h, cap, states, players, pi, z, games, &ex, stream);
}
static int drain_extra(const caro_drain_extra* in, caro_drain_extra* out) {
  *out = caro_drain_extra{(uint32_t)sizeof(caro_drain_extra), nullptr, nullptr, nullptr};
  if (!in) return 0;
  if (in->size < offsetof(caro_drain_extra, root_q_dev)) return fail(CARO_E_INVAL, "caro_drain_extra.size is not set");
  if (in->size >= offsetof(caro_drain_extra, root_q_dev) + sizeof(double*)) out->root_q_dev = in->root_q_dev;
  if (in->size >= offsetof(caro_drain_extra, full_dev) + sizeof(uint8_t*)) out->full_dev = in->full_dev;
  if (in->size >= offsetof(caro_drain_extra, minibatches_dev) + sizeof(uint16_t*)) out->minibatches_dev = in->minibatches_dev;
  return 0;
}
int caro_drain_parked_begin_ex(caro_engine* h, int64_t cap, uint64_t* states, int32_t* players, double* pi, int32_t* z,
                               int64_t* games, const caro_drain_extra* extra, void* stream) {
  if (!h || !states || !players || !pi || !z) return fail(CARO_E_INVAL, "null argument");
  caro_drain_extra ex;
  if (int rc = drain_extra(extra, &ex)) return rc;
  double* root_q = ex.root_q_dev;
  uint8_t* full = ex.full_dev;
  uint16_t* mbs = ex.minibatches_dev;
  if (mbs && !h->v.es_on) return fail(CARO_E_STATE, "caro_drain_parked_begin_ex: minibatches_dev before caro_engine_set_early_stop (no minibatch counts recorded)");
  if (root_q && !h->v.q_on) return fail(CARO_E_STATE, "caro_drain_parked_begin_q before caro_engine_set_resign (no root Q recorded)");
  if (full && !h->v.cap_on) return fail(CARO_E_STATE, "caro_drain_parked_begin_x before caro_engine_set_playout_cap (no ply classes recorded)");
  if (!h->v.stag_S) return fail(CARO_E_STATE, "the engine was not created in staggered mode (caro_config.stagger)");
  if (h->drain_pending) return fail(CARO_E_STATE, "caro_drain_parked_begin twice without caro_drain_tuples_end");
  hipStream_t st = (hipStream_t)stream;
  if (!h->drain_ev) HIPCHK(hipEventCreateWithFlags(&h->drain_ev, hipEventDisableTiming));
  View pv = h->v;
  pv.done = h->v.pk_flag; pv.ply = h->v.pk_ply; pv.final_r = h->v.pk_final_r; pv.first = h->v.pk_first;
  pv.result = h->v.pk_result; pv.step = h->v.pk_step; pv.uid = h->v.pk_uid;
  pv.h_key = h->v.ph_key; pv.h_player = h->v.ph_player; pv.h_pi = h->v.ph_pi; pv.h_q = h->v.ph_q;
  pv.h_full = h->v.ph_full;
  pv.h_mb = h->v.ph_mb;
// ... 41 lines not shown
  return caro_drain_tuples_begin_x(h, cap, states, players, pi, z, games, recycle, root_q, nullptr, stream);
}
int caro_drain_tuples_begin_x(caro_engine* h, int64_t cap, uint64_t* states, int32_t* players, double* pi, int32_t* z,
                              int64_t* games, int recycle, double* root_q, uint8_t* full, void* stream) {
  caro_drain_extra ex = {(uint32_t)sizeof(caro_drain_extra), root_q, full, nullptr};
  return caro_drain_tuples_begin_ex(h, cap, states, players, pi, z, games, recycle, &ex, stream);
}
int caro_drain_tuples_begin_ex(caro_engine* h, int64_t cap, uint64_t* states, int32_t* players, double* pi, int32_t* z,
                               int64_t* games, int recycle, const caro_drain_extra* extra, void* stream) {
  if (!h || !states || !players || !pi || !z) return fail(CARO_E_INVAL, "null argument");
  caro_drain_extra ex;
  if (int rc = drain_extra(extra, &ex)) return rc;
  double* root_q = ex.root_q_dev;
  uint8_t* full = ex.full_dev;
  uint16_t* mbs = ex.minibatches_dev;
  if (mbs && !h->v.es_on) return fail(CARO_E_STATE, "caro_drain_tuples_begin_ex: minibatches_dev before caro_engine_set_early_stop (no minibatch counts recorded)");
  if (root_q && !h->v.q_on) return fail(CARO_E_STATE, "caro_drain_tuples_begin_q before caro_engine_set_resign (no root Q recorded)");
  if (full && !h->v.cap_on) return fail(CARO_E_STATE, "caro_drain_tuples_begin_x before caro_engine_set_playout_cap (no ply classes recorded)");
  if (h->v.stag_S) return fail(CARO_E_STATE, "caro_drain_tuples_begin: the engine runs in staggered mode (per-game clocks, pending minibatches, parked games); use caro_search_staggered / caro_drain_parked_begin");
  if (h->select_pending) return fail(CARO_E_STATE, "caro_drain_tuples with a pending caro_select");
  if (h->drain_pending) return fail(CARO_E_STATE, "caro_drain_tuples_begin twice without caro_drain_tuples_end");
  hipStream_t st = (hipStream_t)stream;
  if (!h->drain_ev) HIPCHK(hipEventCreateWithFlags(&h->drain_ev, hipEventDisableTiming));
  hipLaunchKernelGGL(k_drain_scan, dim3(1), dim3(1024), 0, st, h->v, (long long)cap);
  DISPATCH(h->var, hipLaunchKernelGGL(k_drain_copy<GEO>, dim3(h->v.G), dim3(256), 0, st, h->v, states, players, pi, z,
                                      games, root_q, full, mbs, recycle));
  HIPCHK(hipGetLastError());
  HIPCHK(hipMemcpyAsync(h->pinned64 + 8, h->v.dr_tot, 2 * sizeof(int64_t), hipMemcpyDeviceToHost, st));
  HIPCHK(hipEventRecord(h->drain_ev, st));
  h->drain_pending = 1;
  return 0;
}

int caro_drain_tuples_end(caro_engine* h, int64_t* n_tuples, int64_t* n_games) {
  if (!h || !n_tuples || !n_games) return fail(CARO_E_INVAL, "null argument");
  if (!h->drain_pending) return fail(CARO_E_STATE, "caro_drain_tuples_end without caro_drain_tuples_begin");
  HIPCHK(hipEventSynchronize(h->drain_ev));
  h->drain_pending = 0;
  *n_tuples = h->pinned64[8];
  *n_games = h->pinned64[9];
  return 0;
}

int caro_drain_tuples(caro_engine* h, int64_t cap, uint64_t* states, int32_t* players, double* pi, int32_t* z,
                      int64_t* games, int recycle, int64_t* n_tuples, int64_t* n_games, void* stream) {
  if (!n_tuples || !n_games) return fail(CARO_E_INVAL, "null argument");
  const int rc = caro_drain_tuples_begin(h, cap, states, players, pi, z, games, recycle, stream);
  return rc ? rc : caro_drain_tuples_end(h, n_tuples, n_games);
}

int caro_counters(caro_engine* h, int64_t counters[8], void* stream) {
  if (!h || !counters) return fail(CARO_E_INVAL, "null argument");
  hipLaunchKernelGGL(k_sum_counters, dim3(1), dim3(256), 0, (hipStream_t)stream, h->v);
  HIPCHK(hipMemcpyAsync(h->pinned64, h->v.counters_sum, C_N * sizeof(int64_t), hipMemcpyDeviceToHost,
                        (hipStream_t)stream));
  HIPCHK(hipStreamSynchronize((hipStream_t)stream));
  for (int i = 0; i < 8; ++i) counters[i] = i < C_N ? h->pinned64[i] : 0;
  return 0;
}

int caro_leaf_counts_dev(caro_engine* h, const int32_t** counts_dev) {
  if (!h || !counts_dev) return fail(CARO_E_INVAL, "null argument");
  *counts_dev = h->v.leaf_count;
  return 0;
}

int caro_stream_create_partition(int device_id, int part, int nparts, void** stream_out) {
  if (!stream_out || nparts < 1 || part < 0 || part >= nparts) return fail(CARO_E_INVAL, "bad partition");
  HIPCHK(hipSetDevice(device_id));
  hipDeviceProp_t prop;
  HIPCHK(hipGetDeviceProperties(&prop, device_id));
  const int ncu = prop.multiProcessorCount;
  const int words = (ncu + 31) / 32;
  std::vector<uint32_t> mask(words, 0u);
  const int lo = (int)((long long)ncu * part / nparts), hi = (int)((long long)ncu * (part + 1) / nparts);
  for (int c = lo; c < hi; ++c) mask[c >> 5] |= 1u << (c & 31);
  hipStream_t st = nullptr;
  HIPCHK(hipExtStreamCreateWithCUMask(&st, (uint32_t)words, mask.data()));
  *stream_out = (void*)st;
  return 0;
}
int caro_stream_destroy(void* stream) {
  if (stream) HIPCHK(hipStreamDestroy((hipStream_t)stream));
  return 0;
}

int caro_debug_stamps(caro_engine* h, int on) {
  if (!h) return fail(CARO_E_INVAL, "null engine");
  if (on && !h->v.dbg) {
    void* q = nullptr;
    HIPCHK(hipMalloc(&q, (size_t)h->v.G * 16 * sizeof(unsigned long long)));
    HIPCHK(hipMemset(q, 0, (size_t)h->v.G * 16 * sizeof(unsigned long long)));
    h->allocs.push_back(q);
    h->v.dbg = (unsigned long long*)q;
  } else if (!on) {
    h->v.dbg = nullptr;
  }
  return 0;
}
int caro_debug_read(caro_engine* h, uint64_t* out_host, int64_t n_u64, void* stream) {
  if (!h || !out_host || !h->v.dbg) return fail(CARO_E_INVAL, "no stamp buffer");
  if (n_u64 > (int64_t)h->v.G * 16) n_u64 = (int64_t)h->v.G * 16;
  HIPCHK(hipStreamSynchronize((hipStream_t)stream));
  HIPCHK(hipMemcpy(out_host, h->v.dbg, n_u64 * sizeof(uint64_t), hipMemcpyDeviceToHost));
  return 0;
}

int caro_debug_sqrt_check(uint32_t n_max, uint64_t* bad_host) {
  if (!bad_host || n_max > (1u << 24)) return fail(CARO_E_INVAL, "bad argument");
  unsigned long long* bad = nullptr;
  HIPCHK(hipMalloc(&bad, sizeof(unsigned long long)));
// ... 152 lines not shown
```

### caro_ai_amd/csrc/caro_net.hip

```cpp
#include <hip/hip_runtime.h>

#include <algorithm>
#include <cstdlib>
#include <cstring>
#include <string>
#include <vector>

#include "../../include/caro_hip.h"
#include "../../include/caro_noise.h"

namespace cnet {

typedef float f32x16 __attribute__((ext_vector_type(16)));

constexpr int NF = 64;
constexpr int ZROW = 255;
constexpr int ACT = 256 * NF;
constexpr int WCHUNK = 64 * 64;
constexpr int NRES = 5;
constexpr int MAX_NRES = 40;
constexpr int TPC = 3;
constexpr int NTAPS = NRES * 9;
constexpr int LDS_FLOATS = ACT + 2 * TPC * WCHUNK;

// ... 250 lines not shown
  }
  for (int k = tid; k < nb * A; k += NTH) {
    const int bi = k / A;
    float mx = -3.4e38f;
    if (wide) {
      const float* pm = pmax + bi * 16;
#pragma unroll
      for (int j = 0; j < 16; ++j) mx = fmaxf(mx, pm[j]);
    } else {
      const float* lg = logit + bi * A;
      int a = 0;
      for (; a + 8 <= A; a += 8) {
        const float t0 = lg[a], t1 = lg[a + 1], t2 = lg[a + 2], t3 = lg[a + 3], t4 = lg[a + 4], t5 = lg[a + 5], t6 = lg[a + 6], t7 = lg[a + 7];
        mx = fmaxf(fmaxf(fmaxf(fmaxf(mx, t0), fmaxf(t1, t2)), fmaxf(fmaxf(t3, t4), fmaxf(t5, t6))), t7);
      }
      for (; a < A; ++a) mx = fmaxf(mx, lg[a]);
    }
    ebuf[k] = expf(logit[k] - mx);
  }
  __syncthreads();
  if (wide) {
    for (int idx = tid; idx < nb * 16; idx += NTH) {
      const int bi = idx >> 4, j = idx & 15;
      const float* eb = ebuf + bi * A;
      float part = 0.f;
      for (int a = j; a < A; a += 16) part += eb[a];
      pmax[idx] = part;
    }
    __syncthreads();
    if (tid < nb) {
      float sum = 0.f;
#pragma unroll
      for (int j = 0; j < 16; ++j) sum += pmax[tid * 16 + j];
      stat[2 * tid + 1] = sum;
    }
  } else if (tid < nb) {
    float sum = 0.f;
    const float* eb = ebuf + tid * A;
    int a = 0;
    for (; a + 8 <= A; a += 8) {
      const float t0 = eb[a], t1 = eb[a + 1], t2 = eb[a + 2], t3 = eb[a + 3], t4 = eb[a + 4], t5 = eb[a + 5], t6 = eb[a + 6], t7 = eb[a + 7];
      sum += t0; sum += t1; sum += t2; sum += t3; sum += t4; sum += t5; sum += t6; sum += t7;
    }
    for (; a < A; ++a) sum += eb[a];
    stat[2 * tid + 1] = sum;
  }
  __syncthreads();
  for (int k = tid; k < nb * A; k += NTH) {
    const int bi = k / A;
    probs[(size_t)omap[bi] * A + (k - bi * A)] = ebuf[k] / stat[2 * bi + 1];
  }
}

template <int NTH = NT>
__device__ __forceinline__ void tile_rows(const int32_t* __restrict__ gpack, int G, int B, int cls, int base,
                                          int board0, int nb, int* sc, int* smap, int tid) {
  if (!gpack) {
    if (tid < nb) smap[tid] = base + tid;
    __syncthreads();
    return;
  }
  const int lane = tid & 63, wave = tid >> 6;
  const int cpt = (G + NTH - 1) / NTH;
  const int g_lo = min(G, tid * cpt), g_hi = min(G, g_lo + cpt);
  int mine = 0;
  for (int g = g_lo; g < g_hi; ++g) {
    const int v = gpack[g];
    mine += (v >> 8) == cls ? (v & 0xFF) : 0;
  }
  int inc = mine;
#pragma unroll
  for (int d = 1; d < 64; d <<= 1) {
    const int t = __shfl_up(inc, d, 64);
    if (lane >= d) inc += t;
  }
  if (lane == 63) sc[wave] = inc;
  __syncthreads();
  int ex = inc - mine;
  for (int w = 0; w < wave; ++w) ex += sc[w];
  if (ex < board0 + nb && ex + mine > board0) {
    for (int g = g_lo; g < g_hi; ++g) {
      const int v = gpack[g];
      if ((v >> 8) != cls) continue;
      const int n = v & 0xFF;
      for (int j = 0; j < n; ++j) {
        const int r = ex + j - board0;
        if (r >= 0 && r < nb) smap[r] = g * B + j;
      }
      ex += n;
    }
  }
  __syncthreads();
}


constexpr int GP_PRE = 4;
__device__ __forceinline__ void tile_rows_pre(const int (&gv)[GP_PRE], int cpt, int mine, int B, int cls, int board0,
                                              int nb, int* sc, int* smap, int tid) {
  const int lane = tid & 63, wave = tid >> 6;
  int inc = mine;
#pragma unroll
  for (int d = 1; d < 64; d <<= 1) {
    const int t = __shfl_up(inc, d, 64);
    if (lane >= d) inc += t;
  }
  if (lane == 63) sc[wave] = inc;
  __syncthreads();
  int ex = inc - mine;
  for (int w = 0; w < wave; ++w) ex += sc[w];
  if (ex < board0 + nb && ex + mine > board0) {
#pragma unroll
    for (int u = 0; u < GP_PRE; ++u) {
      const int v = gv[u];
      if (u >= cpt || (v >> 8) != cls) continue;
      const int n = v & 0xFF, g = tid * cpt + u;
      for (int j = 0; j < n; ++j) {
        const int r = ex + j - board0;
        if (r >= 0 && r < nb) smap[r] = g * B + j;
      }
      ex += n;
    }
  }
  __syncthreads();
}

__device__ __forceinline__ unsigned lds_addr(const void* q) {
  return (unsigned)(size_t)(__attribute__((address_space(3))) const void*)q;
}
__device__ __forceinline__ void dma_b128(const void* gsrc, unsigned lds_wave_base) {
  asm volatile("s_mov_b32 m0, %0\n\ts_nop 0\n\tglobal_load_lds_dwordx4 %1, off" ::"s"(lds_wave_base), "v"(gsrc) : "memory");
}
__device__ __forceinline__ void dma_b128_s(const void* sbase, unsigned voff, unsigned lds_wave_base) {
  asm volatile("s_mov_b32 m0, %0\n\ts_nop 0\n\tglobal_load_lds_dwordx4 %1, %2" ::"s"(lds_wave_base), "v"(voff), "s"(sbase) : "memory");
}

#ifndef CARO_X3_TIMERS
#define CARO_X3_TIMERS 0
#endif
typedef __bf16 bf16x8 __attribute__((ext_vector_type(8)));
typedef __bf16 bf16x2 __attribute__((ext_vector_type(2)));
typedef float f32x2 __attribute__((ext_vector_type(2)));
typedef float f32x4v __attribute__((ext_vector_type(4)));
constexpr int X3_H = 3 * 4 * 64;
constexpr int X3_TAP_U4 = 2 * X3_H;
constexpr int X3_PAD_TAPS = 2;
constexpr int X3_RING_H1 = 3 * X3_H;

__device__ __forceinline__ uint32_t pk_bf16(f32x2 v) { return __builtin_bit_cast(uint32_t, __builtin_convertvector(v, bf16x2)); }
__device__ __forceinline__ f32x2 unpk_bf16(uint32_t w) {
  f32x2 r;
  r.x = __builtin_bit_cast(float, w << 16);
  r.y = __builtin_bit_cast(float, w & 0xFFFF0000u);
  return r;
}
__device__ __forceinline__ void split3(f32x2 v, uint32_t& hi, uint32_t& mid, uint32_t& lo) {
  hi = pk_bf16(v);
  const f32x2 r1 = v - unpk_bf16(hi);
  mid = pk_bf16(r1);
  const f32x2 r2 = r1 - unpk_bf16(mid);
  lo = pk_bf16(r2);
}
__device__ __forceinline__ f32x2 join3(uint32_t hi, uint32_t mid, uint32_t lo) {
  return (unpk_bf16(hi) + unpk_bf16(mid)) + unpk_bf16(lo);
}

__global__ __launch_bounds__(NT, 2) void k_net_forward_x3(NetParams p0, NetParams p1, const float* __restrict__ planes,
                                                            const int32_t* __restrict__ counts, int which, int row1,
                                                            float* __restrict__ probs, float* __restrict__ values,
                                                            unsigned long long* __restrict__ stamps,
                                                            const int32_t* __restrict__ gpack, int gG, int gB,
                                                            float* __restrict__ featbuf, int32_t* __restrict__ rowlist) {
  __shared__ __attribute__((aligned(16))) float lds[LDS_FLOATS];
  float* act = lds;
  float* wbuf = lds + ACT;

  int L, row0, board0;
// ... 939 lines not shown
      const float bias = p.b_p[a];
#pragma unroll
      for (int r = 0; r < 16; ++r) logit[(8 * (r >> 2) + 4 * h + (r & 3)) * HLG + a] = acc[r] + bias;
    }
  }
  for (int k = tid; k < nbrd * 20; k += NT) {
    const int bi = k / 20, u = k - bi * 20;
    float s = p.b_v1[u];
    const float* w = wv1 + u * HW;
    const float* f = F + bi * HFS;
#pragma unroll 8
    for (int c = 0; c < HW; ++c) s = fmaf(f[c], w[c], s);
    hid[k] = leaky(s, slope);
  }
  __syncthreads();
  if (tid < nbrd) {
    float s = p.b_v2[0];
    for (int u = 0; u < 20; ++u) s = fmaf(hid[tid * 20 + u], p.w_v2[u], s);
    values[orow[tid]] = tanhf(s);
  }
  const int bi = tid >> 4, j = tid & 15;
  float* lg = logit + bi * HLG;
  float mx = -3.4e38f;
  for (int a = j; a < A; a += 16) mx = fmaxf(mx, lg[a]);
#pragma unroll
  for (int m = 1; m < 16; m <<= 1) mx = fmaxf(mx, __shfl_xor(mx, m, 16));
  float ps = 0.f;
  for (int a = j; a < A; a += 16) {
    const float e = expf(lg[a] - mx);
    lg[a] = e;
    ps += e;
  }
  part[tid] = ps;
  __syncthreads();
  if (j == 0) {
    float sum = 0.f;
#pragma unroll
    for (int q = 0; q < 16; ++q) sum += part[bi * 16 + q];
    rsum[bi] = sum;
  }
  __syncthreads();
  if (bi < nbrd) {
    const float sum = rsum[bi];
    float* out = probs + (size_t)orow[bi] * A;
    for (int a = j; a < A; a += 16) out[a] = lg[a] / sum;
  }
}


__global__ __launch_bounds__(256) void k_net_hash(int HW2, int A, unsigned long long salt0, unsigned long long salt1,
                                                  const float* __restrict__ planes,
                                                  const int32_t* __restrict__ counts, int which, int row1,
                                                  float* __restrict__ probs, float* __restrict__ values,
                                                  const int32_t* __restrict__ gpack, int gG, int gB) {
  const int lane = threadIdx.x & 63;
  const long long w = (long long)blockIdx.x * 4 + (threadIdx.x >> 6);
  long long row;
  int cls = 0;
  if (gpack) {
    const int g = (int)(w / gB), j = (int)(w - (long long)g * gB);
    if (g >= gG) return;
    const int v = gpack[g];
    if (j >= (v & 0xFF)) return;
    cls = v >> 8;
    row = w;
  } else if (which < 2) {
    if (w >= counts[which]) return;
    row = w + (which ? counts[0] : 0);
    cls = 0;
  } else {
    const int L0 = counts[0], L1 = counts[1];
    if (w < L0) { row = w; cls = 0; }
    else if (w < L0 + L1) { row = (row1 >= 0 ? row1 : L0) + (w - L0); cls = 1; }
    else return;
  }
  const float* pl = planes + (size_t)row * HW2;
  unsigned long long h = 0;
  for (int j = lane; j < HW2; j += 64)
    if (pl[j] != 0.0f) h += caro_mix64(0x5851f42d4c957f2dULL + (unsigned long long)j) | 1ULL;
#pragma unroll
  for (int m = 1; m < 64; m <<= 1) h += __shfl_xor(h, m, 64);
  h += cls ? salt1 : salt0;
  for (int a = lane; a < A; a += 64) {
    const unsigned long long ha = caro_mix64(h + 0x9E3779B97F4A7C15ULL * (unsigned long long)(a + 1));
    probs[(size_t)row * A + a] = (float)(((ha >> 20) & 1023ULL) + 1ULL) / 8192.0f;
  }
  if (lane == 0) {
    const unsigned long long hv = caro_mix64(h ^ 0xA5A5A5A5A5A5A5A5ULL);
    values[row] = (float)((long long)((hv >> 20) % 2001ULL) - 1000LL) / 1024.0f;
  }
}

}

extern "C" void caro__set_error(const char* msg);

struct caro_net {
  int kind;
  uint64_t salt;
  cnet::NetParams p;
  float* dev;
  float* ww_dev;
  uint32_t* wtab_dev;
  float* ww2_dev;
  float* wpT_dev;
  uint16_t* wx3_dev;
  struct HeadRows { void* stream; float* feat; int32_t* rowl; int64_t rows; uint64_t used; } hrows[8];
  int n_hrows;
  uint64_t hrows_clock;
  int64_t hrows_evictions;
  int device;
  unsigned long long* dbg_stamps;
};

static int nfail(int code, const std::string& m) {
  caro__set_error(m.c_str());
  return code;
}

static unsigned net_grid(const caro_net* n, int64_t max_rows) {
  int64_t grid = (max_rows + n->p.TB - 1) / n->p.TB;
  if (n->p.ww && n->p.ncu > 0) {
    const int64_t ncu = n->p.ncu, full = ncu * n->p.TB;
    const int tbs[2] = {n->p.TB4, n->p.TB2};
    for (int tb : tbs) {
      if (tb <= 0) continue;
      int64_t small = (max_rows + tb - 1) / tb;
      if (small > ncu) small = ncu;
      if (small > grid) grid = small;
      if (max_rows > full) {
        int64_t split = ncu + (max_rows - full + tb - 1) / tb;
        if (split > 2 * ncu) split = 2 * ncu;
        if (split > grid) grid = split;
      }
    }
  }
  return (unsigned)grid;
}

extern "C" {

static bool depth_ok(int depth) { return depth >= 1 && depth <= cnet::MAX_NRES; }
static int bad_depth(int depth) {
  return nfail(CARO_E_INVAL, "unsupported net depth " + std::to_string(depth) + ": the kernels run 1 .. " +
                                 std::to_string(cnet::MAX_NRES) + " residual blocks");
}

int64_t caro_net_packed_size_depth(int H, int W, int A, int depth) {
  if (!depth_ok(depth)) return bad_depth(depth);
  const int64_t HW = (int64_t)H * W;
  return 9 * 2 * 64 + 64 + (int64_t)depth * 9 * cnet::WCHUNK + depth * 64 + 3 * 64 + 3 +
         20 * HW + 20 + 20 + 1 + (int64_t)A * 2 * HW + A;
}
int64_t caro_net_packed_size(int H, int W, int A) { return caro_net_packed_size_depth(H, W, A, cnet::NRES); }
int caro_net_max_depth(void) { return cnet::MAX_NRES; }
int caro_net_depth(const caro_net* n) { return n && n->kind == 0 ? n->p.nres : 0; }

int caro_net_create(int H, int W, int A, float negative_slope, const float* packed_host, int64_t n_floats,
                    int device_id, caro_net** out) {
  return caro_net_create_depth(H, W, A, cnet::NRES, negative_slope, packed_host, n_floats, device_id, out);
}

int caro_net_create_depth(int H, int W, int A, int depth, float negative_slope, const float* packed_host,
                          int64_t n_floats, int device_id, caro_net** out) {
  if (!packed_host || !out) return nfail(CARO_E_INVAL, "null argument");
  if (H < 2 || W < 2 || H > 15 || W > 15 || A < 1 || A > 255) return nfail(CARO_E_INVAL, "unsupported board / action count");
  if (!depth_ok(depth)) return bad_depth(depth);
  if (n_floats != caro_net_packed_size_depth(H, W, A, depth))
    return nfail(CARO_E_INVAL, depth == cnet::NRES ? "packed weight buffer has the wrong size"
                                                   : "packed weight buffer has the wrong size for a net of " +
                                                         std::to_string(depth) + " residual blocks");
  int ndev = 0;
  if (hipGetDeviceCount(&ndev) != hipSuccess || ndev <= 0)
    return nfail(CARO_E_NODEV, "no HIP device: libcaro_hip needs a GPU (there is no CPU fallback)");
  if (device_id < 0 || device_id >= ndev) return nfail(CARO_E_INVAL, "device_id out of range");
  if (hipSetDevice(device_id) != hipSuccess) return nfail(CARO_E_HIP, "hipSetDevice failed");
  caro_net* n = new caro_net();
  n->kind = 0;
  n->salt = 0;
  n->device = device_id;
  n->ww_dev = nullptr;
  n->wtab_dev = nullptr;
  n->ww2_dev = nullptr;
  n->wpT_dev = nullptr;
  n->wx3_dev = nullptr;
  n->n_hrows = 0;
  n->hrows_clock = 0;
  n->hrows_evictions = 0;
  const size_t pad = (size_t)cnet::TPC * cnet::WCHUNK;
  if (hipMalloc((void**)&n->dev, (n_floats + pad) * sizeof(float)) != hipSuccess) {
    delete n;
    return nfail(CARO_E_NOMEM, "hipMalloc failed");
  }
  if (hipMemset(n->dev + n_floats, 0, pad * sizeof(float)) != hipSuccess ||
      hipMemcpy(n->dev, packed_host, n_floats * sizeof(float), hipMemcpyHostToDevice) != hipSuccess) {
    (void)hipFree(n->dev);
    delete n;
    return nfail(CARO_E_HIP, "hipMemcpy failed");
  }
  cnet::NetParams& p = n->p;
  const int HW = H * W;
  p.H = H; p.W = W; p.HW = HW; p.A = A; p.TB = 255 / HW; p.slope = negative_slope;
  if (p.TB * A > 1024 || p.TB > 32) p.TB = p.TB > 32 ? 32 : p.TB;
  const float* q = n->dev;
  p.w_in = q;   q += 9 * 2 * 64;
  p.b_in = q;   q += 64;
  p.nres = depth;
  p.w_res = q;  q += (size_t)depth * 9 * cnet::WCHUNK;
  p.b_res = q;  q += depth * 64;
  p.w_head = q; q += 3 * 64;
  p.b_head = q; q += 3;
  p.w_v1 = q;   q += 20 * HW;
  p.b_v1 = q;   q += 20;
  p.w_v2 = q;   q += 20;
  p.b_v2 = q;   q += 1;
  p.w_p = q;    q += (size_t)A * 2 * HW;
  p.b_p = q;    q += A;
  p.ww = nullptr;
  p.wtab = nullptr;
  p.ww2 = nullptr;
  p.w_pT = nullptr;
  p.wx3 = nullptr;
  p.ncu = 0; p.TB2 = 0; p.TB4 = 0;
  if (cnet::head_span_host(HW, A) > cnet::HEAD_STAGE_MAX) {
    const size_t half = ((size_t)HW * A + 3) & ~(size_t)3, np = 2 * half;
    const float* wp_host = packed_host + (p.w_p - n->dev);
    std::vector<float> t(np, 0.f);
    const int nq = HW / 4;
    for (int a = 0; a < A; ++a)
      for (int pl = 0; pl < 2; ++pl)
// ... 130 lines not shown
  return 0;
}

int64_t caro_net_split_bf16_size(void) { return (int64_t)cnet::NTAPS * cnet::X3_TAP_U4 * 8; }
int64_t caro_net_split_bf16_size_depth(int depth) {
  return depth_ok(depth) ? (int64_t)depth * 9 * cnet::X3_TAP_U4 * 8 : bad_depth(depth);
}
int caro_net_enable_split_bf16(caro_net* n, const uint16_t* parts_host, int64_t n_u16) {
  if (!n || !parts_host) return nfail(CARO_E_INVAL, "null argument");
  if (n->kind != 0) return nfail(CARO_E_STATE, "not a conv net");
  if (n->p.ww || n->p.ww2) return nfail(CARO_E_STATE, "net is already in another arithmetic mode");
  if (n->p.nres != cnet::NRES)
    return nfail(CARO_E_INVAL, "bf16x3 form: built for nets of " + std::to_string(cnet::NRES) + " residual blocks only, this net has " +
                                   std::to_string(n->p.nres) + " (use a float32 mode)");
  const int64_t want = caro_net_split_bf16_size();
  if (n_u16 != want) return wrong_image(n, "split weight image");
  if (hipSetDevice(n->device) != hipSuccess) return nfail(CARO_E_HIP, "hipSetDevice failed");
  const size_t pad = (size_t)cnet::X3_PAD_TAPS * cnet::X3_TAP_U4 * 8;
  if (!n->wx3_dev) {
    if (hipMalloc((void**)&n->wx3_dev, (want + pad) * sizeof(uint16_t)) != hipSuccess) return nfail(CARO_E_NOMEM, "hipMalloc failed");
    if (hipMemset(n->wx3_dev + want, 0, pad * sizeof(uint16_t)) != hipSuccess) return nfail(CARO_E_HIP, "hipMemset failed");
  }
  if (hipMemcpy(n->wx3_dev, parts_host, want * sizeof(uint16_t), hipMemcpyHostToDevice) != hipSuccess)
    return nfail(CARO_E_HIP, "hipMemcpy failed");
  n->p.wx3 = n->wx3_dev;
  return 0;
}

int64_t caro_net_stream_evictions(const caro_net* n) { return n ? n->hrows_evictions : 0; }

void caro_net_destroy(caro_net* n) {
  if (!n) return;
  if (n->ww_dev) (void)hipFree(n->ww_dev);
  if (n->wtab_dev) (void)hipFree(n->wtab_dev);
  if (n->ww2_dev) (void)hipFree(n->ww2_dev);
  if (n->wpT_dev) (void)hipFree(n->wpT_dev);
  if (n->wx3_dev) (void)hipFree(n->wx3_dev);
  for (int k = 0; k < n->n_hrows; ++k) {
    if (n->hrows[k].feat) (void)hipFree(n->hrows[k].feat);
    if (n->hrows[k].rowl) (void)hipFree(n->hrows[k].rowl);
  }
  if (n->dev) (void)hipFree(n->dev);
  delete n;
}

int caro_net_create_hash(int H, int W, int A, uint64_t salt, int device_id, caro_net** out) {
  if (!out) return nfail(CARO_E_INVAL, "null argument");
  if (H < 2 || W < 2 || H > 15 || W > 15 || A < 1 || A > 255) return nfail(CARO_E_INVAL, "unsupported board / action count");
  int ndev = 0;
  if (hipGetDeviceCount(&ndev) != hipSuccess || ndev <= 0)
    return nfail(CARO_E_NODEV, "no HIP device: libcaro_hip needs a GPU (there is no CPU fallback)");
  if (device_id < 0 || device_id >= ndev) return nfail(CARO_E_INVAL, "device_id out of range");
  caro_net* n = new caro_net();
  memset(&n->p, 0, sizeof n->p);
  n->kind = 1;
  n->salt = salt;
  n->device = device_id;
  n->dev = nullptr;
  n->ww_dev = nullptr;
  n->wtab_dev = nullptr;
  n->ww2_dev = nullptr;
  n->wpT_dev = nullptr;
  n->wx3_dev = nullptr;
  n->n_hrows = 0;
  n->hrows_clock = 0;
  n->hrows_evictions = 0;
  n->p.H = H; n->p.W = W; n->p.HW = H * W; n->p.A = A; n->p.TB = 4;
  *out = n;
  return 0;
}

static int head_rows_for(caro_net* n0, void* stream, int64_t need, caro_net::HeadRows** out) {
  caro_net::HeadRows* hr = nullptr;
  for (int k = 0; k < n0->n_hrows; ++k)
    if (n0->hrows[k].stream == stream) hr = &n0->hrows[k];
  if (!hr) {
    if (n0->n_hrows == 8) {
      hr = &n0->hrows[0];
      for (int k = 1; k < 8; ++k)
        if (n0->hrows[k].used < hr->used) hr = &n0->hrows[k];
      if (hipDeviceSynchronize() != hipSuccess) return nfail(CARO_E_HIP, "hipDeviceSynchronize failed");
      n0->hrows_evictions += 1;
      hr->stream = stream;
    } else {
      hr = &n0->hrows[n0->n_hrows++];
      hr->stream = stream; hr->feat = nullptr; hr->rowl = nullptr; hr->rows = 0;
    }
  }
  hr->used = ++n0->hrows_clock;
  if (hr->rows < need) {
    if (hr->feat) (void)hipFree(hr->feat);
    if (hr->rowl) (void)hipFree(hr->rowl);
    hr->feat = nullptr; hr->rowl = nullptr; hr->rows = 0;
    if (hipMalloc((void**)&hr->feat, (size_t)need * 3 * n0->p.HW * sizeof(float)) != hipSuccess ||
        hipMalloc((void**)&hr->rowl, (size_t)need * sizeof(int32_t)) != hipSuccess)
      return nfail(CARO_E_NOMEM, "hipMalloc of the head feature rows failed");
    hr->rows = need;
  }
  *out = hr;
  return 0;
}

static int net_launch(caro_net* n0, caro_net* n1, const float* planes_dev, const int32_t* counts_dev, int which,
                      int row1, int64_t max_rows, float* probs_dev, float* values_dev, const int32_t* gpack, int G,
                      int B, unsigned long long* stamps, void* stream, const int32_t* slist = nullptr) {
  hipStream_t st = (hipStream_t)stream;
  if (n0->kind == 1) {
    const int64_t waves = gpack ? (int64_t)G * B : max_rows;
    const unsigned grid = (unsigned)((waves + 3) / 4);
    hipLaunchKernelGGL(cnet::k_net_hash, dim3(grid), dim3(256), 0, st, 2 * n0->p.HW, n0->p.A,
                       (unsigned long long)n0->salt, (unsigned long long)n1->salt, planes_dev, counts_dev, which, row1,
                       probs_dev, values_dev, gpack, G, B);
  } else {
    const unsigned grid = net_grid(n0, max_rows) + (which == 2 ? 1u : 0u);
    const bool d5 = n0->p.nres == cnet::NRES && n1->p.nres == cnet::NRES;
    if (n0->p.ww2) {
      caro_net::HeadRows* hr = nullptr;
      if (int rc = head_rows_for(n0, stream, max_rows + (row1 > 0 ? row1 : 0) + 64, &hr)) return rc;
      hipLaunchKernelGGL(d5 ? cnet::k_net_forward_w2 : cnet::k_net_forward_w2_any, dim3(grid), dim3(cnet::NT), 0, st,
                         n0->p, n1->p, planes_dev, counts_dev, which, row1, probs_dev, values_dev,
                         stamps ? stamps : n0->dbg_stamps, gpack, G, B, hr->feat, hr->rowl, slist);
      if (hipGetLastError() != hipSuccess) return nfail(CARO_E_HIP, "net kernel launch failed");
      const unsigned hgrid = (unsigned)((max_rows + cnet::HB - 1) / cnet::HB) + (which == 2 ? 1u : 0u);
      hipLaunchKernelGGL(cnet::k_net_heads, dim3(hgrid), dim3(cnet::NT), 0, st, n0->p, n1->p, counts_dev, which, row1,
                         hr->feat, hr->rowl, probs_dev, values_dev);
    }
    else if (n0->p.ww)
      hipLaunchKernelGGL(d5 ? cnet::k_net_forward_w : cnet::k_net_forward_w_any, dim3(grid), dim3(cnet::NT), 0, st,
                         n0->p, n1->p, planes_dev, counts_dev, which, row1, probs_dev, values_dev,
                         stamps ? stamps : n0->dbg_stamps, gpack, G, B);
    else if (n0->p.wx3) {
      const bool batched = n0->p.TB == 1 && n0->p.w_pT && n0->p.HW <= cnet::HEADS_MAX_CELLS;
      caro_net::HeadRows* hr = nullptr;
      if (batched)
        if (int rc = head_rows_for(n0, stream, max_rows + (row1 > 0 ? row1 : 0) + 64, &hr)) return rc;
      hipLaunchKernelGGL(cnet::k_net_forward_x3, dim3(grid), dim3(cnet::NT), 0, st, n0->p, n1->p, planes_dev,
                         counts_dev, which, row1, probs_dev, values_dev, stamps, gpack, G, B, hr ? hr->feat : nullptr,
                         hr ? hr->rowl : nullptr);
      if (hr) {
        if (hipGetLastError() != hipSuccess) return nfail(CARO_E_HIP, "net kernel launch failed");
        const unsigned hgrid = (unsigned)((max_rows + cnet::HB - 1) / cnet::HB) + (which == 2 ? 1u : 0u);
        hipLaunchKernelGGL(cnet::k_net_heads, dim3(hgrid), dim3(cnet::NT), 0, st, n0->p, n1->p, counts_dev, which, row1,
                           hr->feat, hr->rowl, probs_dev, values_dev);
      }
    }
    else
      hipLaunchKernelGGL(d5 ? cnet::k_net_forward : cnet::k_net_forward_any, dim3(grid), dim3(cnet::NT), 0, st, n0->p,
                         n1->p, planes_dev, counts_dev, which, row1, probs_dev, values_dev, stamps, gpack, G, B);
  }
  if (hipGetLastError() != hipSuccess) return nfail(CARO_E_HIP, "net kernel launch failed");
  return 0;
}
static int pair_ok(const caro_net* n0, const caro_net* n1) {
  if (n0->p.H != n1->p.H || n0->p.W != n1->p.W || n0->p.A != n1->p.A) return nfail(CARO_E_INVAL, "nets differ in shape");
  if (n0->kind != n1->kind || 
      (n0->p.ww == nullptr) != (n1->p.ww == nullptr) || (n0->p.ww2 == nullptr) != (n1->p.ww2 == nullptr) ||
      (n0->p.wx3 == nullptr) != (n1->p.wx3 == nullptr))
    return nfail(CARO_E_INVAL, "nets differ in kind / arithmetic mode");
  return 0;
}

int caro_net_boards_per_workgroup(const caro_net* n) { return n ? n->p.TB : 0; }
int caro_net_uses_slot_list(const caro_net* n) { return n && n->p.ww2 ? 1 : 0; }

int caro_net_forward(caro_net* n, const float* planes_dev, const int32_t* counts_dev, int which, int64_t max_rows,
                     float* probs_dev, float* values_dev, void* stream) {
  if (!n || !planes_dev || !counts_dev || !probs_dev || !values_dev) return nfail(CARO_E_INVAL, "null argument");
  if (which != 0 && which != 1) return nfail(CARO_E_INVAL, "which must be 0 or 1");
  if (max_rows <= 0) return 0;
  return net_launch(n, n, planes_dev, counts_dev, which, -1, max_rows, probs_dev, values_dev, nullptr, 0, 0, nullptr,
                    stream);
}

int caro_net_forward_pair_at(caro_net* n0, caro_net* n1, const float* planes_dev, const int32_t* counts_dev,
                             int64_t row1_base, int64_t max_rows, float* probs_dev, float* values_dev, void* stream) {
  if (!n0 || !n1 || !planes_dev || !counts_dev || !probs_dev || !values_dev) return nfail(CARO_E_INVAL, "null argument");
  if (int rc = pair_ok(n0, n1)) return rc;
  if (max_rows <= 0) return 0;
  return net_launch(n0, n1, planes_dev, counts_dev, 2, (int)row1_base, max_rows, probs_dev, values_dev, nullptr, 0, 0,
                    nullptr, stream);
}

int caro_net_forward_pair(caro_net* n0, caro_net* n1, const float* planes_dev, const int32_t* counts_dev,
                          int64_t max_rows, float* probs_dev, float* values_dev, void* stream) {
  return caro_net_forward_pair_at(n0, n1, planes_dev, counts_dev, -1, max_rows, probs_dev, values_dev, stream);
}

int caro_net_forward_slots(caro_net* n0, caro_net* n1, const float* planes_dev, const int32_t* counts_dev,
                           const int32_t* gpack_dev, int n_games, int batch, float* probs_dev, float* values_dev,
                           void* stream) {
  if (!n0 || !planes_dev || !counts_dev || !gpack_dev || !probs_dev || !values_dev)
    return nfail(CARO_E_INVAL, "null argument");
  if (n_games < 1 || batch < 1 || batch > 255) return nfail(CARO_E_INVAL, "bad slot geometry");
  if (n1)
    if (int rc = pair_ok(n0, n1)) return rc;
  return net_launch(n0, n1 ? n1 : n0, planes_dev, counts_dev, n1 ? 2 : 0, -1, (int64_t)n_games * batch, probs_dev,
                    values_dev, gpack_dev, n_games, batch, nullptr, stream);
}

int caro_net_forward_slot_list(caro_net* n0, caro_net* n1, const float* planes_dev, const int32_t* counts_dev,
                               const int32_t* gpack_dev, const int32_t* slot_list_dev, int n_games, int batch,
                               float* probs_dev, float* values_dev, void* stream) {
  if (!n0 || !planes_dev || !counts_dev || !gpack_dev || !probs_dev || !values_dev)
    return nfail(CARO_E_INVAL, "null argument");
  if (n_games < 1 || batch < 1 || batch > 255) return nfail(CARO_E_INVAL, "bad slot geometry");
  if (n1)
    if (int rc = pair_ok(n0, n1)) return rc;
  return net_launch(n0, n1 ? n1 : n0, planes_dev, counts_dev, n1 ? 2 : 0, -1, (int64_t)n_games * batch, probs_dev,
                    values_dev, gpack_dev, n_games, batch, nullptr, stream, n0->p.ww2 ? slot_list_dev : nullptr);
}

int caro_net_forward_stamped(caro_net* n, const float* planes_dev, const int32_t* counts_dev, int which,
                             int64_t max_rows, float* probs_dev, float* values_dev, uint64_t* stamps_dev,
                             void* stream) {
  if (!n || !stamps_dev) return nfail(CARO_E_INVAL, "null argument");
  if (n->kind != 0) return nfail(CARO_E_STATE, "stamps: conv kernels only");
  return net_launch(n, n, planes_dev, counts_dev, which, -1, max_rows, probs_dev, values_dev, nullptr, 0, 0,
                    (unsigned long long*)stamps_dev, stream);
}

int caro_net_debug_stamps(caro_net* n, uint64_t* stamps_dev) {
  if (!n) return nfail(CARO_E_INVAL, "null argument");
  n->dbg_stamps = (unsigned long long*)stamps_dev;
  return 0;
}

}
```

### caro_ai_amd/csrc/caro_net_kernels.inc

```

__global__ __launch_bounds__(NT, 2) void CARO_KN(k_net_forward)(NetParams p0, NetParams p1, const float* __restrict__ planes,
                                                         const int32_t* __restrict__ counts, int which, int row1,
                                                         float* __restrict__ probs, float* __restrict__ values,
                                                         unsigned long long* __restrict__ stamps,
                                                         const int32_t* __restrict__ gpack, int gG, int gB) {
  __shared__ __attribute__((aligned(16))) float lds[LDS_FLOATS];
  float* act = lds;
  float* wbuf = lds + ACT;

  int L, row0, board0;
  bool second = false;
  if (which < 2) {
    L = counts[which];
    row0 = which ? counts[0] : 0;
    board0 = blockIdx.x * p0.TB;
  } else {
    const int L0 = counts[0];
    const int t0 = (L0 + p0.TB - 1) / p0.TB;
    second = (int)blockIdx.x >= t0;
    L = second ? counts[1] : L0;
    row0 = second ? (row1 >= 0 ? row1 : L0) : 0;
    board0 = (second ? (int)blockIdx.x - t0 : (int)blockIdx.x) * p0.TB;
  }
  if (board0 >= L) return;
// ... 98 lines not shown
    }
#undef CARO_LOAD_SET
#undef CARO_MFMA_SET
    if (last_in_chunk && has_next) {
      float4* dst = reinterpret_cast<float4*>(wbuf + (cur ^ 1) * TPC * WCHUNK);
      dst[tid] = wn0;
      dst[tid + NT] = wn1;
      dst[tid + 2 * NT] = wn2;
      dst[tid + 3 * NT] = wn3;
      dst[tid + 4 * NT] = wn4;
      dst[tid + 5 * NT] = wn5;
    }
    if (tap == 8) {
      __syncthreads();
      const float* bias = p.b_res + layer * NF;
      const float bc0 = bias[i], bc1 = bias[32 + i];
      float old0[16], old1[16];
#pragma unroll
      for (int e = 0; e < 16; ++e) {
        const int row = wave * 32 + (e & 3) + 8 * (e >> 2) + 4 * h;
        old0[e] = act[aoff(row, i)];
        old1[e] = act[aoff(row, 32 + i)];
      }
#pragma unroll
      for (int e = 0; e < 16; ++e) {
        const int row = wave * 32 + (e & 3) + 8 * (e >> 2) + 4 * h;
        const bool real = row < R;
        const float n0 = old0[e] + leaky(acc0[e] + bc0, slope);
        const float n1 = old1[e] + leaky(acc1[e] + bc1, slope);
        act[aoff(row, i)] = real ? n0 : 0.f;
        act[aoff(row, 32 + i)] = real ? n1 : 0.f;
        acc0[e] = 0.f;
        acc1[e] = 0.f;
      }
    }
    if (last_in_chunk || tap == 8) __syncthreads();
  }
  unsigned long long t_trunk1 = 0;
  if (stamps) t_trunk1 = __builtin_amdgcn_s_memtime();
  heads_f32<false>(p, act, wbuf, probs, values, slot_v, nb, R, tid);
  if (stamps && tid == 0) {
    stamps[4 * blockIdx.x] = __builtin_amdgcn_s_memtime() - t_c0;
    stamps[4 * blockIdx.x + 1] = __builtin_amdgcn_s_memrealtime() - t_r0;
    stamps[4 * blockIdx.x + 2] = t_trunk0 - t_c0;
    stamps[4 * blockIdx.x + 3] = t_trunk1 - t_c0;
  }
}

__global__ __launch_bounds__(NT, 2) void CARO_KN(k_net_forward_w)(NetParams p0, NetParams p1,
                                                           const float* __restrict__ planes,
                                                           const int32_t* __restrict__ counts, int which, int row1,
                                                           float* __restrict__ probs, float* __restrict__ values,
                                                           unsigned long long* __restrict__ stamps,
                                                           const int32_t* __restrict__ gpack, int gG, int gB) {
  __shared__ __attribute__((aligned(256))) float lds[LDS_FLOATS];
  float* act = lds;
  float* wbuf = lds + ACT;

  const unsigned long long t_abs0 = stamps ? __builtin_amdgcn_s_memrealtime() : 0;
  const int gcpt = gpack ? (gG + NT - 1) / NT : 0;
  const bool gpre = gpack && gcpt <= GP_PRE;
  int gv[GP_PRE];
#pragma unroll
  for (int u = 0; u < GP_PRE; ++u) {
    const int g = (int)threadIdx.x * gcpt + u;
    gv[u] = gpre && u < gcpt && g < gG ? gpack[g] : 0;
  }
  int L, row0, board0, nb, nb_cap = p0.TB;
  int ks = 1;
  bool second = false;
  if (which < 2) {
    L = counts[which];
    row0 = which ? counts[0] : 0;
    board0 = blockIdx.x * p0.TB;
    const int full = p0.ncu * p0.TB;
    if (p0.ncu > 0) {
      if (p0.TB4 > 0 && L <= p0.ncu * p0.TB4) ks = 4;
      else if (p0.TB2 > 0 && L <= p0.ncu * p0.TB2) ks = 2;
      if (ks > 1) {
        nb_cap = ks == 4 ? p0.TB4 : p0.TB2;
        board0 = (int)blockIdx.x * nb_cap;
      } else if (L > full) {
        const int over = L - full;
        if (p0.TB4 > 0 && over <= p0.ncu * p0.TB4) ks = 4;
        else if (p0.TB2 > 0 && over <= p0.ncu * p0.TB2) ks = 2;
        if (ks > 1) {
          if ((int)blockIdx.x < p0.ncu) {
            ks = 1;
          } else {
            nb_cap = ks == 4 ? p0.TB4 : p0.TB2;
            board0 = full + ((int)blockIdx.x - p0.ncu) * nb_cap;
          }
        }
      }
    }
  } else {
    const int L0 = counts[0], L1 = counts[1];
    if (p0.ncu > 1) {
      if (p0.TB4 > 0 && L0 + L1 <= (p0.ncu - 1) * p0.TB4) ks = 4;
      else if (p0.TB2 > 0 && L0 + L1 <= (p0.ncu - 1) * p0.TB2) ks = 2;
      if (ks > 1) nb_cap = ks == 4 ? p0.TB4 : p0.TB2;
    }
    const int t0 = (L0 + nb_cap - 1) / nb_cap;
    second = (int)blockIdx.x >= t0;
    L = second ? L1 : L0;
    row0 = second ? (row1 >= 0 ? row1 : L0) : 0;
    board0 = (second ? (int)blockIdx.x - t0 : (int)blockIdx.x) * nb_cap;
  }
  if (board0 >= L) return;
  const NetParams p = second ? p1 : p0;
  unsigned long long t_c0 = 0, t_r0 = 0;
  if (stamps) {
    t_c0 = __builtin_amdgcn_s_memtime();
    t_r0 = __builtin_amdgcn_s_memrealtime();
  }
  nb = min(nb_cap, L - board0);
  const int HW = p.HW;
  const int R = nb * HW;
  const int tid = threadIdx.x;

  int gmine = 0;
#pragma unroll
  for (int u = 0; u < GP_PRE; ++u) gmine += (gv[u] >> 8) == (second ? 1 : 0) ? (gv[u] & 0xFF) : 0;
  asm volatile("" : "+v"(gmine));
  float* win = wbuf + 2 * WCH;
  if (tid < 320) dma_b128(reinterpret_cast<const float4*>(p.w_in) + tid,
                          __builtin_amdgcn_readfirstlane(lds_addr(win) + (unsigned)(tid >> 6) * 1024u));
  fetch_chunk(p.ww, 0, lds_addr(wbuf), tid);
  fetch_chunk(p.ww, 1, lds_addr(wbuf), tid);
  for (int k = tid + (R * NF) / 4; k < ACT / 4; k += NT) reinterpret_cast<float4*>(lds)[k] = make_float4(0.f, 0.f, 0.f, 0.f);
  static_assert(2 * (WCH / 4 / NT) == 8, "s_waitcnt vmcnt(8) below counts 2 chunks x WCH / 4 / NT transfers per thread");
  static_assert(320 * 4 >= 9 * 2 * NF, "the 320-lane transfer must cover w_in [9][2][64]");
  asm volatile("s_waitcnt vmcnt(8)" ::: "memory");
  int* smap = reinterpret_cast<int*>(win + 1536);
  if (gpre) tile_rows_pre(gv, gcpt, gmine, gB, second ? 1 : 0, board0, nb, smap + 64, smap, tid);
  else tile_rows(gpack, gG, gB, second ? 1 : 0, row0 + board0, board0, nb, smap + 64, smap, tid);
  conv_in_mfma(p, planes, smap, act, win, R, tid);
  const int slot_v = tid < nb ? smap[tid] : 0;
  unsigned long long t_trunk0 = 0;
  if (stamps) t_trunk0 = __builtin_amdgcn_s_memtime();
  asm volatile("s_waitcnt vmcnt(0)" ::: "memory");
  __syncthreads();
  const int hspan = head_span(HW, p.A) <= HEAD_STAGE_MAX ? head_span(HW, p.A) : 0;
  if (ks == 1) trunk_w<1, CARO_NR>(p, act, wbuf, nb, tid, hspan);
  else if (ks == 2) trunk_w<2, CARO_NR>(p, act, wbuf, nb, tid, hspan);
  else trunk_w<4, CARO_NR>(p, act, wbuf, nb, tid, hspan);
  unsigned long long t_trunk1 = 0;
  if (stamps) t_trunk1 = __builtin_amdgcn_s_memtime();
  if (hspan) heads_f32<true>(p, act, wbuf, probs, values, slot_v, nb, R, tid);
  else heads_f32<false>(p, act, wbuf, probs, values, slot_v, nb, R, tid);
  if (stamps && tid == 0) {
    stamps[4 * blockIdx.x] = __builtin_amdgcn_s_memtime() - t_c0;
    stamps[4 * blockIdx.x + 1] = gpack ? ((__builtin_amdgcn_s_memrealtime() - t_abs0) & 0xFFFFFull) | (t_abs0 << 20)
                                       : __builtin_amdgcn_s_memrealtime() - t_r0;
    stamps[4 * blockIdx.x + 2] = t_trunk0 - t_c0;
    stamps[4 * blockIdx.x + 3] = t_trunk1 - t_c0;
  }
}

__global__ __launch_bounds__(NT, 2) void CARO_KN(k_net_forward_w2)(NetParams p0, NetParams p1,
                                                            const float* __restrict__ planes,
                                                            const int32_t* __restrict__ counts, int which, int row1,
                                                            float* __restrict__ probs, float* __restrict__ values,
                                                            unsigned long long* __restrict__ stamps,
                                                            const int32_t* __restrict__ gpack, int gG, int gB,
                                                            float* __restrict__ featbuf, int32_t* __restrict__ rowlist,
                                                            const int32_t* __restrict__ slist) {
  __shared__ __attribute__((aligned(256))) float lds[LDS_FLOATS];
  float* act = lds;
  float* wbuf = lds + ACT;
  const int gcpt = gpack && !slist ? (gG + NT - 1) / NT : 0;
  const bool gpre = gpack && !slist && gcpt <= GP_PRE;
  int gv[GP_PRE];
#pragma unroll
  for (int u = 0; u < GP_PRE; ++u) {
    const int g = (int)threadIdx.x * gcpt + u;
    gv[u] = gpre && u < gcpt && g < gG ? gpack[g] : 0;
  }
  int L, row0, board0;
  bool second = false;
  if (which < 2) {
    L = counts[which];
    row0 = which ? counts[0] : 0;
    board0 = blockIdx.x;
  } else {
    const int L0 = counts[0];
    second = (int)blockIdx.x >= L0;
    L = second ? counts[1] : L0;
    row0 = second ? (row1 >= 0 ? row1 : L0) : 0;
// ... 50 lines not shown
```

### caro_ai_amd/engine.py

```python
import ctypes as C

import numpy as np
import torch

from caro_ai_amd import _lib
from caro_ai_amd import early_stop
from caro_ai_amd import config as cfg

COUNTER_NAMES = ["sims", "levels", "expansions", "terminals", "dropped", "overflows", "plies", "finished"]


HIP_NET_MODES = {"hip": "f32", "hipw": "f32w", "hipw1": "f32w1", "hipw2": "f32w2", "hipx3": "bf16x3"}

def lanes_per_descent(game):
    A = game.action_space
    return 8 if A == 7 else 16 if A <= 16 else 32 if A <= 32 else 64


def staggered_geometry(game, batch, evict=False):
    t = int(batch) * lanes_per_descent(game)
    return t >= 64 and t % 64 == 0 and (t > 64 or not evict)


def _ptr(t):
    return C.c_void_p(t.data_ptr()) if t is not None else None


def torch_evaluator(net, form="gemm"):
    from caro_ai_amd.lib.model import GemmNet, Net
    net.eval()
    if form == "gemm" and isinstance(net, Net):
        dev = next(net.parameters()).device
        net = GemmNet(net).to(dev).eval()

    @torch.no_grad()
    def fn(planes):
        logits, values = net(planes)
        return torch.softmax(logits.float(), dim=1).contiguous(), values.float().reshape(-1).contiguous()

    return fn


class SelfPlayEngine:
    VIEW_LIMIT_BYTES = 16 << 20
    DEFAULT_CAP_LIMIT = 1 << 16
    EVICT_DEFAULT_CAP = 1 << 13

    def __init__(self, game, n_games, net1=None, net2=None, evaluators=None, n_stores=1, max_batch=None,
                 node_cap=None, steps_before_tau_0=cfg.STEPS_BEFORE_TAU_0, first_player_mode=2,
                 c_puct=cfg.C_PUCT, alpha=cfg.ALPHA, explore=cfg.EXPLORE, seed=0, uid_base=0, uid_stride=None,
                 device="cuda:0", searches_hint=cfg.MCTS_SEARCHES, inference="hipw", evict=False, stagger=False,
                 stagger_recycle=True, games_limit=0):
        if not torch.cuda.is_available():
            raise _lib.CaroError("SelfPlayEngine needs a GPU (torch.cuda.is_available() is False); "
                                 "there is no CPU fallback")
        self.L = _lib.load()
        self.game = game
        self.device = torch.device(device)
        self.G = int(n_games)
        self.A = game.action_space
        self.KW = game.key_words
        self.obs_shape = tuple(game.obs_shape)
        self.HW = self.obs_shape[1] * self.obs_shape[2]
        self.max_batch = int(max_batch or cfg.MCTS_BATCH_SIZE)
        if evaluators is None:
            nets = [net1] if net2 is None or net2 is net1 else [net1, net2]
            if inference in HIP_NET_MODES:
                from caro_ai_amd.net_hip import HipNet
                mode = HIP_NET_MODES[inference]
                evaluators = [HipNet(n, str(self.device), mode=mode) for n in nets]
            else:
                evaluators = [torch_evaluator(n.to(self.device), form=inference) for n in nets]
        self.evaluators = list(evaluators)
        self.async_net = all(getattr(e, "device_counts", False) for e in self.evaluators)
        self.n_nets = len(self.evaluators)
        assert self.n_nets in (1, 2)
        if node_cap is None:
            node_cap = self.default_node_cap(searches_hint, self.max_batch, self.HW, evict)
        c = _lib.CaroConfig()
        c.game_kind, c.n, c.k = game.kind, game.n, game.k
        c.n_games, c.n_stores, c.n_nets = self.G, n_stores, self.n_nets
        c.max_batch, c.node_cap = self.max_batch, int(node_cap)
        c.steps_before_tau_0, c.first_player_mode = steps_before_tau_0, first_player_mode
        c.c_puct, c.alpha, c.explore = c_puct, alpha, explore
        c.seed, c.uid_base = seed, uid_base
        c.uid_stride = uid_stride if uid_stride is not None else self.G
        c.device_id = self.device.index or 0
        c.evict = 1 if evict else 0
        self.stagger = bool(stagger)
        self.stag_S = int(searches_hint)
        if self.stagger and not self.async_net:
            raise _lib.CaroError("stagger=True needs device-side evaluators (the fused HIP net or HashNet)")
        c.stagger = self.stag_S if self.stagger else 0
        c.stagger_recycle = int(stagger_recycle)
        c.games_limit = int(games_limit or 0)
        self.stagger_recycle = bool(stagger_recycle)
        self.cfg = c
        self.n_stores = n_stores
        torch.cuda.set_device(self.device)
        h = C.c_void_p()
        _lib.check(self.L.caro_engine_create(C.byref(c), C.byref(h)))
        self.h = h
        rows = self.G * self.max_batch
        self.planes = torch.zeros((rows,) + self.obs_shape, dtype=torch.float32, device=self.device)
        self.leaf_keys = torch.zeros((rows, self.KW), dtype=torch.int64, device=self.device)
        self._probs = torch.zeros((rows, self.A), dtype=torch.float32, device=self.device)
        self._values = torch.zeros(rows, dtype=torch.float32, device=self.device)
        self._counts = (C.c_int32 * 2)()
        cd = C.c_void_p()
        _lib.check(self.L.caro_leaf_counts_dev(self.h, C.byref(cd)))
        self._counts_dev = cd
        self.maxply = self.HW
        self._row_bytes = 8 * self.KW + 8 * self.A + 8
        self.net_rows = 0
        self.net_calls = 0
        self._prof = False
        self._drain_open = False
        self.resign = None
        self.playout_cap = None
        self.early_stop = None

    @classmethod
    def default_node_cap(cls, searches, max_batch, cells, evict=False):
        bound = int(searches) * int(max_batch) * int(cells) + 64
        if bound <= cls.DEFAULT_CAP_LIMIT:
            return bound
        if not evict:
            raise _lib.CaroError(
                "SelfPlayEngine: %d searches x %d descents x %d cells needs up to %d nodes per tree, more than the %d a "
                "default tree holds; pass evict=True (unreachable nodes are dropped after every move, result-neutral: "
                "node_cap then bounds the LIVE nodes) or an explicit node_cap"
                % (searches, max_batch, cells, bound, cls.DEFAULT_CAP_LIMIT))
        return cls.EVICT_DEFAULT_CAP

    def close(self):
        if getattr(self, "h", None):
            self.L.caro_engine_destroy(self.h)
            self.h = None

    RUN_FIELDS = ("seed", "uid_base", "uid_stride", "games_limit", "steps_before_tau_0", "first_player_mode", "c_puct",
                  "alpha", "explore", "stagger_recycle")

    def restart(self, evaluators=None, searches=None, **run):
        bad = set(run) - set(self.RUN_FIELDS)
        assert not bad, "restart() cannot change %s: these shape the engine's memory" % sorted(bad)
        if self._drain_open:
            self.flush()
        c = self.cfg
        for k, val in run.items():
            setattr(c, k, int(val) if k == "stagger_recycle" else val)
        if searches is not None and self.stagger:
            self.stag_S = int(searches)
            c.stagger = self.stag_S
        self.stagger_recycle = bool(c.stagger_recycle)
        if evaluators is not None:
# ... 198 lines not shown
        _lib.check(self.L.caro_drain_tuples_end(self.h, C.addressof(nt), C.addressof(ng)))
        nt, ng = nt.value, ng.value
        if nt == 0 and ng == 0:
            self._dr = None
            out = {"states": s.new_empty((0, self.KW)), "players": p.new_empty((0,)), "pi": pi.new_empty((0, self.A)),
                   "z": z.new_empty((0,)), "games": games.new_empty((0, 4))}
            if q is not None:
                out["root_q"] = q.new_empty((0,))
            if f is not None:
                out["full"] = f.new_empty((0,))
            if m is not None:
                out["mb"] = m.new_empty((0,))
            return out
        out = {"states": s[:nt], "players": p[:nt], "pi": pi[:nt], "z": z[:nt], "games": games[:ng]}
        if q is not None:
            out["root_q"] = q[:nt]
        if f is not None:
            out["full"] = f[:nt]
        if m is not None:
            out["mb"] = m[:nt]
        if s.shape[0] * self._row_bytes > self.VIEW_LIMIT_BYTES and 4 * nt < s.shape[0]:
            out = {k: v.clone() for k, v in out.items()}
            self._dr = None
        return out

    def drain(self, recycle=True, cap=None):
        self.drain_begin(recycle, cap)
        return self.drain_end()

    def search_step(self, searches, batch):
        if self.async_net and not self.stagger:
            nets = [e.h for e in self.evaluators] + [None]
            _lib.check(self.L.caro_search_move(self.h, nets[0], nets[1], searches, batch, None, None, _ptr(self.planes),
                                               _ptr(self.leaf_keys), _ptr(self._probs), _ptr(self._values), None, None,
                                               None, self._stream()))
            self.net_calls += searches * self.n_nets
        else:
            self.search(searches, batch)
            self.step()

    def move(self, searches, batch, recycle=True):
        self.search_step(searches, batch)
        out = self.drain_end() if self._drain_open else None
        self.drain_begin(recycle)
        self._drain_open = True
        return out

    def flush(self):
        if not self._drain_open:
            return None
        self._drain_open = False
        return self.drain_end()

    def counters(self):
        out = (C.c_int64 * 8)()
        _lib.check(self.L.caro_counters(self.h, out, self._stream()))
        return dict(zip(COUNTER_NAMES, list(out)))

    def profile(self, on=True):
        _lib.check(self.L.caro_profile_enable(self.h, 1 if on else 0))
        self._prof = bool(on)

    def profile_read(self, reset=True):
        ms = (C.c_double * 8)()
        n = (C.c_int64 * 8)()
        _lib.check(self.L.caro_profile_read(self.h, ms, n, 1 if reset else 0))
        return {k: (ms[i], n[i]) for i, k in enumerate(["select", "compact", "expand_backup", "step", "net", "null1", "null2"])}

    def live_games(self):
        out = C.c_int32(0)
        _lib.check(self.L.caro_live_games(self.h, C.addressof(out), self._stream()))
        return out.value

    def pending_leaves(self):
        out = C.c_int32(0)
        _lib.check(self.L.caro_pending_leaves(self.h, C.addressof(out), self._stream()))
        return out.value

    def tree_sizes(self):
        out = torch.empty(self.G * self.n_stores, dtype=torch.int32, device=self.device)
        _lib.check(self.L.caro_tree_sizes(self.h, _ptr(out), self._stream()))
        return out.cpu().numpy().reshape(self.G, self.n_stores)

    def tree_live(self):
        out = torch.empty(self.G * self.n_stores, dtype=torch.int32, device=self.device)
        _lib.check(self.L.caro_tree_live(self.h, _ptr(out), self._stream()))
        return out.cpu().numpy().reshape(self.G, self.n_stores)

    def roots(self):
        keys = torch.empty((self.G, self.KW), dtype=torch.int64, device=self.device)
        pl = torch.empty(self.G, dtype=torch.int32, device=self.device)
        ply = torch.empty(self.G, dtype=torch.int32, device=self.device)
        uid = torch.empty(self.G, dtype=torch.int64, device=self.device)
        _lib.check(self.L.caro_get_roots(self.h, _ptr(keys), _ptr(pl), _ptr(ply), _ptr(uid), self._stream()))
        return (keys.cpu().numpy().view(np.uint64), pl.cpu().numpy(), ply.cpu().numpy(),
                uid.cpu().numpy().view(np.uint64))

    def lookup(self, games, stores, states):
        M = len(states)
        dev = self.device
        g = torch.as_tensor(games, dtype=torch.int32).to(dev)
        s = torch.as_tensor(stores, dtype=torch.int32).to(dev)
        keys = torch.from_numpy(self.game.to_keys(states).view(np.int64)).to(dev)
        found = torch.zeros(M, dtype=torch.int32, device=dev)
        N = torch.zeros((M, self.A), dtype=torch.int32, device=dev)
        strong = torch.zeros((M, self.A), dtype=torch.int32, device=dev)
# ... 190 lines not shown
```

### include/caro_hip.h

```cpp
#ifndef CARO_HIP_H
#define CARO_HIP_H

#include <stdint.h>

#ifdef __cplusplus
extern "C" {
#endif

#define CARO_GAME_CONNECT4 0
#define CARO_GAME_MNK 1
#define CARO_GAME_CARO 2

#define CARO_E_INVAL (-22)
#define CARO_E_NOMEM (-12)
#define CARO_E_HIP (-5)
#define CARO_E_NODEV (-19)
#define CARO_E_STATE (-71)

#define CARO_RESIGNED (-2)

typedef struct caro_engine caro_engine;

typedef struct caro_config {
  int32_t game_kind;
// ... 43 lines not shown
                     const uint32_t* sim_dev, double* out_dev, void* stream);

int caro_engine_create(const caro_config* cfg, caro_engine** out);
void caro_engine_destroy(caro_engine* h);
int caro_engine_restart(caro_engine* h, const caro_config* cfg, void* stream);
int caro_reset_games(caro_engine* h, const int32_t* first_player_dev, void* stream);
int caro_set_roots(caro_engine* h, const uint64_t* keys_dev, const int32_t* players_dev, void* stream);

int caro_select(caro_engine* h, int batch, int mb_index, const double* noise_dev, float* planes_dev,
                uint64_t* leaf_keys_dev, void* stream);
int caro_get_descent(caro_engine* h, int game, int b, int32_t* info_dev, float* value_dev, uint64_t* leaf_key_dev,
                     uint64_t* path_keys_dev, int32_t* path_actions_dev, void* stream);
int caro_select_cancel(caro_engine* h);
int caro_leaf_counts(caro_engine* h, int32_t counts[2], void* stream);
int caro_leaf_counts_dev(caro_engine* h, const int32_t** counts_dev);
int caro_expand_backup(caro_engine* h, const float* probs_dev, const float* values_dev, void* stream);

int caro_policy(caro_engine* h, double* pi_dev, int32_t* counts_dev, void* stream);
int caro_step(caro_engine* h, const double* uniforms_dev, int32_t* actions_dev, int32_t* done_dev,
              int32_t* result_dev, void* stream);
int caro_drain_tuples(caro_engine* h, int64_t cap, uint64_t* states_dev, int32_t* players_dev, double* pi_dev,
                      int32_t* z_dev, int64_t* games_dev, int recycle, int64_t* n_tuples, int64_t* n_games,
                      void* stream);
int caro_drain_tuples_begin(caro_engine* h, int64_t cap, uint64_t* states_dev, int32_t* players_dev, double* pi_dev,
                            int32_t* z_dev, int64_t* games_dev, int recycle, void* stream);
int caro_drain_tuples_end(caro_engine* h, int64_t* n_tuples, int64_t* n_games);

int caro_engine_set_resign(caro_engine* h, double threshold, double playthrough);
int caro_drain_tuples_begin_q(caro_engine* h, int64_t cap, uint64_t* states_dev, int32_t* players_dev, double* pi_dev,
                              int32_t* z_dev, int64_t* games_dev, int recycle, double* root_q_dev, void* stream);
int caro_drain_parked_begin_q(caro_engine* h, int64_t cap, uint64_t* states_dev, int32_t* players_dev, double* pi_dev,
                              int32_t* z_dev, int64_t* games_dev, double* root_q_dev, void* stream);

int caro_engine_set_playout_cap(caro_engine* h, double p_full, int fast);
int caro_drain_tuples_begin_x(caro_engine* h, int64_t cap, uint64_t* states_dev, int32_t* players_dev, double* pi_dev,
                              int32_t* z_dev, int64_t* games_dev, int recycle, double* root_q_dev, uint8_t* full_dev,
                              void* stream);
int caro_drain_parked_begin_x(caro_engine* h, int64_t cap, uint64_t* states_dev, int32_t* players_dev, double* pi_dev,
                              int32_t* z_dev, int64_t* games_dev, double* root_q_dev, uint8_t* full_dev, void* stream);

int caro_engine_set_early_stop(caro_engine* h, int min_minibatches);
typedef struct caro_drain_extra {
  uint32_t size;
  double* root_q_dev;
  uint8_t* full_dev;
  uint16_t* minibatches_dev;
} caro_drain_extra;
int caro_drain_tuples_begin_ex(caro_engine* h, int64_t cap, uint64_t* states_dev, int32_t* players_dev, double* pi_dev,
                               int32_t* z_dev, int64_t* games_dev, int recycle, const caro_drain_extra* extra,
                               void* stream);
int caro_drain_parked_begin_ex(caro_engine* h, int64_t cap, uint64_t* states_dev, int32_t* players_dev, double* pi_dev,
                               int32_t* z_dev, int64_t* games_dev, const caro_drain_extra* extra, void* stream);

int caro_counters(caro_engine* h, int64_t counters[8], void* stream);
int caro_profile_enable(caro_engine* h, int on);
int caro_profile_begin(caro_engine* h, int kind, void* stream);
void caro_profile_end(caro_engine* h, int slot, void* stream);
int caro_profile_read(caro_engine* h, double ms[8], int64_t launches[8], int reset);
int caro_debug_stamps(caro_engine* h, int on);
int caro_debug_read(caro_engine* h, uint64_t* out_host, int64_t n_u64, void* stream);
int caro_debug_sqrt_check(uint32_t n_max, uint64_t* bad_host);
int caro_live_games(caro_engine* h, int32_t* live, void* stream);
int caro_pending_leaves(caro_engine* h, int32_t* pending, void* stream);

int caro_tree_sizes(caro_engine* h, int32_t* out_dev, void* stream);
int caro_tree_live(caro_engine* h, int32_t* out_dev, void* stream);
int caro_lookup_nodes(caro_engine* h, int64_t M, const int32_t* game_dev, const int32_t* store_dev,
                      const uint64_t* keys_dev, int32_t* found_dev, int32_t* N_dev, float* W_dev, float* Q_dev,
                      float* P_dev, int32_t* strong_dev, void* stream);
int caro_get_roots(caro_engine* h, uint64_t* keys_dev, int32_t* players_dev, int32_t* ply_dev, uint64_t* uid_dev,
                   void* stream);
int caro_poke_nodes(caro_engine* h, int64_t M, const int32_t* game_dev, const int32_t* store_dev,
                    const uint64_t* keys_dev, const int32_t* N_dev, const float* W_dev, const float* Q_dev,
                    const float* P_dev, const int32_t* strong_dev, void* stream);
int caro_backup_path(caro_engine* h, int game, int store, float value, int value_is_f32, int len,
                     const uint64_t* keys_dev, const int32_t* actions_dev, void* stream);
int caro_dump_tree(caro_engine* h, int game, int store, int64_t cap, uint64_t* keys_dev, int32_t* N_dev,
                   float* W_dev, float* Q_dev, float* P_dev, int32_t* strong_dev, int64_t* n_nodes, void* stream);

typedef struct caro_net caro_net;
int64_t caro_net_packed_size(int H, int W, int A);
int caro_net_create(int H, int W, int A, float negative_slope, const float* packed_host, int64_t n_floats,
                    int device_id, caro_net** out);
int caro_net_max_depth(void);
int64_t caro_net_packed_size_depth(int H, int W, int A, int depth);
int caro_net_create_depth(int H, int W, int A, int depth, float negative_slope, const float* packed_host,
                          int64_t n_floats, int device_id, caro_net** out);
int caro_net_depth(const caro_net* n);
int64_t caro_net_winograd_size_depth(int depth);
int caro_net_enable_winograd(caro_net* n, const float* ww_host, int64_t n_floats);
int caro_net_winograd2d_size(void);
int64_t caro_net_winograd2d_size_depth(int depth);
int caro_net_winograd2d_supported(int H, int W);
int caro_net_enable_winograd2d(caro_net* n, const float* ww2_host, int64_t n_floats);
int64_t caro_net_split_bf16_size(void);
int64_t caro_net_split_bf16_size_depth(int depth);
int caro_net_enable_split_bf16(caro_net* n, const uint16_t* parts_host, int64_t n_u16);
int64_t caro_net_stream_evictions(const caro_net* n);
void caro_net_destroy(caro_net* n);
int caro_net_boards_per_workgroup(const caro_net* n);
int caro_net_uses_slot_list(const caro_net* n);
int caro_net_forward(caro_net* n, const float* planes_dev, const int32_t* counts_dev, int which, int64_t max_rows,
                     float* probs_dev, float* values_dev, void* stream);

int caro_net_forward_slots(caro_net* n0, caro_net* n1, const float* planes_dev, const int32_t* counts_dev,
                           const int32_t* gpack_dev, int n_games, int batch, float* probs_dev, float* values_dev,
                           void* stream);

int caro_net_forward_slot_list(caro_net* n0, caro_net* n1, const float* planes_dev, const int32_t* counts_dev,
                               const int32_t* gpack_dev, const int32_t* slot_list_dev, int n_games, int batch,
                               float* probs_dev, float* values_dev, void* stream);

int caro_net_create_hash(int H, int W, int A, uint64_t salt, int device_id, caro_net** out);

int caro_stream_create_partition(int device_id, int part, int nparts, void** stream_out);
int caro_stream_destroy(void* stream);
int caro_net_forward_pair(caro_net* n0, caro_net* n1, const float* planes_dev, const int32_t* counts_dev,
                          int64_t max_rows, float* probs_dev, float* values_dev, void* stream);
int caro_net_forward_pair_at(caro_net* n0, caro_net* n1, const float* planes_dev, const int32_t* counts_dev,
                             int64_t row1_base, int64_t max_rows, float* probs_dev, float* values_dev, void* stream);
int caro_net_forward_stamped(caro_net* n, const float* planes_dev, const int32_t* counts_dev, int which,
                             int64_t max_rows, float* probs_dev, float* values_dev, uint64_t* stamps_dev,
                             void* stream);
int caro_net_debug_stamps(caro_net* n, uint64_t* stamps_dev);
int caro_search_batch(caro_engine* h, caro_net* net0, caro_net* net1, int searches, int batch,
                      const double* noise_dev, float* planes_dev, uint64_t* leaf_keys_dev, float* probs_dev,
                      float* values_dev, void* stream);

int caro_search_move(caro_engine* h, caro_net* net0, caro_net* net1, int searches, int batch, const double* noise_dev,
                     const double* uniforms_dev, float* planes_dev, uint64_t* leaf_keys_dev, float* probs_dev,
                     float* values_dev, int32_t* actions_dev, int32_t* done_dev, int32_t* result_dev, void* stream);

int caro_search_staggered(caro_engine* h, caro_net* net0, caro_net* net1, int launches, int batch, float* planes_dev,
                          uint64_t* leaf_keys_dev, float* probs_dev, float* values_dev, void* stream);
int caro_drain_parked_begin(caro_engine* h, int64_t cap, uint64_t* states_dev, int32_t* players_dev, double* pi_dev,
                            int32_t* z_dev, int64_t* games_dev, void* stream);

#ifdef __cplusplus
}
#endif
#endif
```

Baseline: 8.494 million.

## Add GPU evaluation cache to skip network inference for repeated positions

Adds a device-side hash table keyed by board and player that stores policy and value outputs from earlier network evaluations. During selection, first-seen leaves probe the table, and on a hit the cached probabilities and value are written straight into the output rows. The network kernel gets a cached mode that runs only the missed rows, using a miss bitmask packed into g_pack. Expansion inserts new results with CAS-claimed slots and release stores, which adds atomics, extra global traffic and new counters. The cache is on by default when the geometry fits and can be disabled through an environment variable.

Measured after the change: 8.224 million. 0.968x the previous value.

```diff
diff --git a/caro_ai_amd/_lib.py b/caro_ai_amd/_lib.py
--- a/caro_ai_amd/_lib.py
+++ b/caro_ai_amd/_lib.py
@@ -113,6 +113,12 @@
     "caro_drain_tuples_begin_ex": (C.c_int, [_P, C.c_int64, _P, _P, _P, _P, _P, C.c_int, C.POINTER(CaroDrainExtra), _P]),
     "caro_drain_parked_begin_ex": (C.c_int, [_P, C.c_int64, _P, _P, _P, _P, _P, C.POINTER(CaroDrainExtra), _P]),
     "caro_counters": (C.c_int, [_P, _P, _P]),
+    "caro_engine_cache_counters": (C.c_int, [_P, _P, _P]),
+    "caro_engine_cache_clear": (C.c_int, [_P, _P]),
+    "caro_engine_set_cache": (C.c_int, [_P, C.c_int64]),
+    "caro_net_serial": (C.c_uint64, [_P]),
+    "caro_net_cache_ranges": (C.c_int, [_P, _P, _P]),
+    "caro_net_forward_slots_cached": (C.c_int, [_P, _P, _P, _P, _P, _P, C.c_int, C.c_int, _P, _P, C.c_int, _P]),
     "caro_live_games": (C.c_int, [_P, _P, _P]),
     "caro_pending_leaves": (C.c_int, [_P, _P, _P]),
     "caro_debug_stamps": (C.c_int, [_P, C.c_int]),
diff --git a/caro_ai_amd/csrc/caro_engine.hip b/caro_ai_amd/csrc/caro_engine.hip
--- a/caro_ai_amd/csrc/caro_engine.hip
+++ b/caro_ai_amd/csrc/caro_engine.hip
@@ -20,7 +20,8 @@
 constexpr int ST_DROPPED = 0, ST_TERMINAL = 1, ST_LEAF = 2;
 constexpr int MAXB = 64;
 
-enum Counter { C_SIMS, C_LEVELS, C_EXPANSIONS, C_TERMINALS, C_DROPPED, C_OVERFLOW, C_PLIES, C_FINISHED, C_N };
+enum Counter { C_SIMS, C_LEVELS, C_EXPANSIONS, C_TERMINALS, C_DROPPED, C_OVERFLOW, C_PLIES, C_FINISHED,
+               C_CACHE_HITS, C_NET_ROWS, C_CACHE_ROWS, C_N };
 
 struct View {
   GameParams gp;
@@ -84,6 +85,10 @@
   int32_t* pk_ply; int32_t* pk_final_r; int32_t* pk_first; int32_t* pk_result; int32_t* pk_step;
   uint64_t* pk_uid;
   uint64_t* ph_key; int32_t* ph_player; double* ph_pi; double* ph_q; uint8_t* ph_full; uint16_t* ph_mb;
+  int ec_on, ec_ew;
+  uint32_t ec_mask;
+  uint32_t* ec_tab;
+  int ec_lo, ec_full, ec_hi;
   int32_t* dr_off;
   int32_t* dr_gidx;
   int32_t* dr_sel;
@@ -123,6 +128,22 @@
 __device__ __forceinline__ void es_ply_start(const View& v, int g) {
   v.es_cut[g] = 0;
   v.es_cnt[g] = 0;
+}
+
+constexpr int EC_WIN = 4;
+template <class R>
+__device__ __forceinline__ uint64_t ec_tag(const typename R::Board& b, int player) {
+  uint64_t h = 0x9E3779B97F4A7C15ULL + (uint64_t)player;
+#pragma unroll
+  for (int w = 0; w < R::KW; ++w) h = caro_mix64(h ^ b.w[w]) + 0x632BE59BD9B4E019ULL;
+  h = caro_mix64(h);
+  return h < 2ull ? h + 2ull : h;
+}
+__device__ __forceinline__ uint32_t* ec_entry(const View& v, int cls, uint32_t e) {
+  return v.ec_tab + ((size_t)cls * ((size_t)v.ec_mask + 1u) + (e & v.ec_mask)) * (size_t)v.ec_ew;
+}
+__device__ __forceinline__ bool ec_full_form(const View& v, int F) {
+  return (F > v.ec_lo && F <= v.ec_full) || F > v.ec_hi;
 }
 
 template <class GEO>
@@ -572,7 +593,8 @@
 __device__ __forceinline__ void select_body(const View& v, const GameRegs<GEO>& gr, int B, int mb_index,
                                             const double* __restrict__ noise, int32_t* __restrict__ rows,
                                             float* __restrict__ planes, uint64_t* __restrict__ leaf_keys,
-                                            const double* helper_nz = nullptr, volatile int* helper_flag = nullptr) {
+                                            const double* helper_nz = nullptr, volatile int* helper_flag = nullptr,
+                                            float* ec_probs = nullptr, float* ec_values = nullptr) {
   using R = typename GEO::R;
   using Board = typename R::Board;
   constexpr int LPD = GEO::LPD, APL = GEO::APL, AP = GEO::AP, KW = GEO::KW;
@@ -679,7 +701,40 @@
     const unsigned long long m_first = __ballot(head && first_seen);
     const unsigned long long m_term = __ballot(head && st == ST_TERMINAL);
     const unsigned long long m_drop = __ballot(head && st == ST_LEAF && dup);
-    const int my_rank = __popcll(m_first & ((1ull << tid) - 1ull));
+    const int my_rank = __popcll(m_first & ((1ull << first) - 1ull));
+    uint32_t ec_note = 0u;
+    int miss_bits = 0;
+    if constexpr (APL == 1) {
+      if (v.ec_on) {
+        const int cls_ec = v.n_nets == 2 ? player0 : 0;
+        const uint64_t tg = ec_tag<R>(d.cur, d.player);
+        const uint32_t home = (uint32_t)(tg >> 20);
+        uint64_t seen = 1ull;
+        if (first_seen && l < EC_WIN)
+          seen = __hip_atomic_load(reinterpret_cast<const uint64_t*>(ec_entry(v, cls_ec, home + (uint32_t)l)),
+                                   __ATOMIC_ACQUIRE, __HIP_MEMORY_SCOPE_AGENT);
+        const uint32_t gm = (uint32_t)(__ballot(first_seen && l < EC_WIN && seen == tg) >> first) & ((1u << EC_WIN) - 1u);
+        const uint32_t ge = (uint32_t)(__ballot(first_seen && l < EC_WIN && seen == 0ull) >> first) & ((1u << EC_WIN) - 1u);
+        bool hit = false;
+        if (gm) {
+          const uint32_t* e = ec_entry(v, cls_ec, home + (uint32_t)(__ffs((int)gm) - 1));
+          bool same = (int)e[2 + 2 * KW] == d.player;
+#pragma unroll
+          for (int w = 0; w < KW; ++w) same = same && reinterpret_cast<const uint64_t*>(e)[1 + w] == d.cur.w[w];
+          const float* ef = reinterpret_cast<const float*>(e) + 2 + 2 * KW + 1;
+          const float pv = ef[l < A ? l : 0], vv = ef[A];
+          hit = same;
+          if (hit) {
+            const size_t rowi = (size_t)g * B + my_rank;
+            if (l < A) ec_probs[rowi * A + l] = pv;
+            if (l == 0) ec_values[rowi] = vv;
+          }
+        }
+        ec_note = hit ? 1u : (ge ? (uint32_t)__ffs((int)ge) << 8 : 0u);
+        miss_bits = group_allreduce_i32<64>((head && first_seen && !hit) ? 1 << my_rank : 0,
+                                            [](int x, int y) { return x | y; });
+      }
+    }
     const int levels = group_sum_i32<64>(head ? d.depth : 0);
     int maxdep = 0;
     if (v.dbg) maxdep = group_allreduce_i32<64>(d.depth, [](int x, int y) { return x > y ? x : y; });
@@ -687,7 +742,7 @@
       const size_t di = (size_t)g * v.maxB + b;
       const uint32_t stw = (uint32_t)((st == ST_LEAF && dup) ? ST_DROPPED : st);
       v.d_rec[di] = make_uint4(stw | ((uint32_t)d.depth << 8) | ((uint32_t)my_rank << 16) | ((uint32_t)d.player << 24),
-                               __float_as_uint(d.value), d.home, 0u);
+                               __float_as_uint(d.value), d.home, ec_note);
       store_board<R>(v.d_key + di * KW, d.cur);
     }
     const int nleaf = __popcll(m_first);
@@ -709,6 +764,10 @@
         const int cls = v.n_nets == 2 ? player0 : 0;
         if (nleaf) atomicAdd(rows + cls, nleaf);
         v.g_off[g] = g * B;
+        if (v.ec_on) {
+          if (miss_bits) atomicAdd(rows + 4 + cls, __popc(miss_bits));
+          v.g_pack[g] = nleaf | (cls << 8) | (miss_bits << 16) | (1 << 24);
+        } else
         v.g_pack[g] = nleaf | (cls << 8);
       }
     }
@@ -936,6 +995,7 @@
   uint4 p0, p1;
   float pr[NPR];
   int nleaf;
+  int ecF[2];
 };
 template <class GEO, bool ONE>
 __device__ __forceinline__ ExpandPre<GEO> expand_preload(const View& v, int g, int B, int off, const float* __restrict__ probs,
@@ -945,6 +1005,7 @@
   ExpandPre<GEO> e;
   const int lane = threadIdx.x;
   e.nleaf = v.g_nleaf[g];
+  e.ecF[0] = e.ecF[1] = 0;
   e.rec = make_uint4(ST_DROPPED, 0u, 0u, 0u);
   e.row_val = 0.f;
 #pragma unroll
@@ -1038,6 +1099,22 @@
   }
   block_sync<ONE>();
   CARO_XS(1)
+  bool ec_won = false;
+  uint32_t* ec_e = nullptr;
+  uint64_t ec_tg = 0ull;
+  int ec_nhit = 0;
+  if constexpr (ONE && GEO::APL == 1) {
+    if (v.ec_on) {
+      const uint32_t note = pre.rec.w;
+      const int cls = v.n_nets == 2 ? gr.player : 0;
+      ec_nhit = __popcll(__ballot(is_leaf && (note & 1u)));
+      if (is_leaf && !(note & 1u) && (note >> 8) && ec_full_form(v, cls ? pre.ecF[1] : pre.ecF[0])) {
+        ec_tg = ec_tag<R>(brd, (int)(pre.rec.x >> 24));
+        ec_e = ec_entry(v, cls, (uint32_t)(ec_tg >> 20) + (note >> 8) - 1u);
+        ec_won = atomicCAS(reinterpret_cast<unsigned long long*>(ec_e), 0ull, 1ull) == 0ull;
+      }
+    }
+  }
   const bool whole_wave = ONE || blockDim.x >= 64;
   const bool wave0 = whole_wave && lane < 64;
   if (!overflow) {
@@ -1082,6 +1159,8 @@
       v.n_nodes[t] = base + nleaf;
       atomicAdd(v.n_created + t, nleaf);
       atomicAdd(ctr + C_EXPANSIONS, (unsigned long long)nleaf);
+      if (ec_nhit) atomicAdd(ctr + C_CACHE_HITS, (unsigned long long)ec_nhit);
+      atomicAdd(ctr + C_NET_ROWS, (unsigned long long)(nleaf - ec_nhit));
     }
     if (st_sel) gr.nn[1] = base + nleaf;
     else gr.nn[0] = base + nleaf;
@@ -1154,6 +1233,25 @@
       if (a >= A) pv = 0.f;
       reinterpret_cast<uint4*>(row)[a] = make_uint4(0u, 0u, 0u, __float_as_uint(pv));
     }
+  if constexpr (ONE && GEO::APL == 1) {
+    if (v.ec_on) {
+      float* ef = reinterpret_cast<float*>(ec_e) + 2 + 2 * KW + 1;
+      for (int a = 0; a < A; ++a) {
+        const int src = lane < B ? my_local * AP + a : lane;
+        const float x = __shfl(pre.pr[0], src & 63, 64);
+        if (ec_won) ef[a] = x;
+      }
+      if (ec_won) {
+#pragma unroll
+        for (int w = 0; w < KW; ++w) reinterpret_cast<uint64_t*>(ec_e)[1 + w] = brd.w[w];
+        ec_e[2 + 2 * KW] = pre.rec.x >> 24;
+        ef[A] = my_val;
+        __hip_atomic_store(reinterpret_cast<uint64_t*>(ec_e), ec_tg, __ATOMIC_RELEASE, __HIP_MEMORY_SCOPE_AGENT);
+      }
+      const int nins = __popcll(__ballot(ec_won));
+      if (lane == 0 && nins) atomicAdd(v.counters + (size_t)g * C_N + C_CACHE_ROWS, (unsigned long long)nins);
+    }
+  }
   if (total > MAXE) {
     if (lane == 0)
       for (int k = 0; k < nq; ++k) {
@@ -1282,10 +1380,10 @@
 }
 
 template <class GEO>
-__global__ void k_tree(View v, int B, int mb_index, const double* __restrict__ noise, const float* __restrict__ probs,
-                       const float* __restrict__ values, float* __restrict__ planes, uint64_t* __restrict__ leaf_keys,
-                       int32_t* __restrict__ rows_cur, int32_t* __restrict__ rows_next, int do_expand,
-                       int do_select) {
+__global__ void k_tree(View v, int B, int mb_index, const double* __restrict__ noise, float* probs,
+                       float* values, float* __restrict__ planes, uint64_t* __restrict__ leaf_keys,
+                       int32_t* __restrict__ rows_cur, int32_t* __restrict__ rows_next,
+                       const int32_t* __restrict__ rows_prev, int do_expand, int do_select) {
   __shared__ double s_nz[MAXB * 0 + 64 * GEO::APL];
   __shared__ int s_flag;
   if (threadIdx.x == 0) s_flag = 0;
@@ -1302,19 +1400,25 @@
     rows_next[0] = 0;
     rows_next[1] = 0;
     rows_next[2] = B;
+    rows_next[4] = 0;
+    rows_next[5] = 0;
     rows_cur[2] = B;
   }
   unsigned long long t0 = 0;
   if (v.dbg) t0 = __builtin_amdgcn_s_memtime();
   GameRegs<GEO> gr = load_game<GEO>(v, blockIdx.x);
-  const ExpandPre<GEO> pre = expand_preload<GEO, true>(v, blockIdx.x, B, blockIdx.x * B, probs, values);
+  ExpandPre<GEO> pre = expand_preload<GEO, true>(v, blockIdx.x, B, blockIdx.x * B, probs, values);
+  if (v.ec_on) {
+    pre.ecF[0] = rows_prev[0];
+    pre.ecF[1] = rows_prev[1];
+  }
   if (do_expand) {
     expand_body<GEO, true>(v, gr, B, pre, blockIdx.x * B, probs);
     block_sync<true>();
   }
   const unsigned long long t1 = v.dbg ? __builtin_amdgcn_s_memtime() : 0;
   if (v.dbg && threadIdx.x == 0 && !do_select) v.dbg[(size_t)blockIdx.x * 8 + 5] = t1 - t0;
-  if (do_select) select_body<GEO, true>(v, gr, B, mb_index, noise, rows_cur, planes, leaf_keys, s_nz, &s_flag);
+  if (do_select) select_body<GEO, true>(v, gr, B, mb_index, noise, rows_cur, planes, leaf_keys, s_nz, &s_flag, probs, values);
   if (v.dbg && threadIdx.x == 0 && do_select) {
     v.dbg[(size_t)blockIdx.x * 8 + 6] = t1 - t0;
     v.dbg[(size_t)blockIdx.x * 8 + 7] = __builtin_amdgcn_s_memtime() - t0;
@@ -1838,9 +1942,10 @@
 }
 
 template <class GEO>
-__global__ void k_tree_stag(View v, int B, const float* __restrict__ probs, const float* __restrict__ values,
+__global__ void k_tree_stag(View v, int B, float* probs, float* values,
                             float* __restrict__ planes, uint64_t* __restrict__ leaf_keys,
-                            int32_t* __restrict__ rows_cur, int32_t* __restrict__ rows_next) {
+                            int32_t* __restrict__ rows_cur, int32_t* __restrict__ rows_next,
+                            const int32_t* __restrict__ rows_prev) {
   constexpr int AP = GEO::AP;
   __shared__ double s_pi[AP];
   __shared__ int s_n[AP];
@@ -1855,7 +1960,13 @@
   const int cut = v.es_on ? v.es_cut[g] : 0;
   GameRegs<GEO> gr = load_game<GEO>(v, g);
   ExpandPre<GEO> pre;
-  if (threadIdx.x < 64) pre = expand_preload<GEO, true>(v, g, B, g * B, probs, values);
+  if (threadIdx.x < 64) {
+    pre = expand_preload<GEO, true>(v, g, B, g * B, probs, values);
+    if (v.ec_on) {
+      pre.ecF[0] = rows_prev[0];
+      pre.ecF[1] = rows_prev[1];
+    }
+  }
   __syncthreads();
   if (threadIdx.x >= 64) {
     const int go = w == 0 && gr.done == 0;
@@ -1873,6 +1984,8 @@
     rows_next[0] = 0;
     rows_next[1] = 0;
     rows_next[2] = B;
+    rows_next[4] = 0;
+    rows_next[5] = 0;
     rows_cur[2] = B;
   }
   const unsigned long long t0 = v.dbg ? __builtin_amdgcn_s_memtime() : 0;
@@ -1907,7 +2020,7 @@
     if (park_and_restart<GEO>(v, g, gr)) over = 0;
   }
   const unsigned long long t2 = v.dbg ? __builtin_amdgcn_s_memtime() : 0;
-  select_body<GEO, true>(v, gr, B, lm, nullptr, rows_cur, planes, leaf_keys, s_nz, &s_flag);
+  select_body<GEO, true>(v, gr, B, lm, nullptr, rows_cur, planes, leaf_keys, s_nz, &s_flag, probs, values);
   if (threadIdx.x == 0) {
     v.lm[g] = over ? 0 : lm + 1;
     v.pend[g] = over ? 0 : 1;
@@ -2440,6 +2553,8 @@
   uint64_t prof_ctr;
   uint64_t prof_cal;
   int32_t* rows;
+  uint64_t ec_serial[2];
+  size_t ec_bytes;
   int rows_par;
   int fused_ok;
   std::vector<hipEvent_t> ev;
@@ -2510,7 +2625,7 @@
 
 const char* caro_last_error(void) { return g_err.c_str(); }
 void caro__set_error(const char* msg) { g_err = msg ? msg : ""; }
-int caro_version(void) { return 101; }
+int caro_version(void) { return 102; }
 
 #include "caro_host.inc"
 
@@ -2578,16 +2693,49 @@
     v.stag_pool = (cfg->stagger_recycle == 2 && cfg->games_limit > 0) ? 1 : 0;
   }
 }
+static int ec_resize(caro_engine* h, long long want) {
+  View& v = h->v;
+  const int lpd = variant_lpd(h->var);
+  const bool geo_ok = variant_ap(h->var) == lpd && h->cfg.max_batch * lpd == 64;
+  if (want < 0) want = 1 << 18;
+  if (!geo_ok) want = 0;
+  const char* e = getenv("CARO_EVAL_CACHE");
+  if (e && e[0] == '0') want = 0;
+  if (want > (1 << 26)) return fail(CARO_E_INVAL, "evaluation cache: at most 2^26 entries");
+  if (v.ec_tab) {
+    for (size_t i = 0; i < h->allocs.size(); ++i)
+      if (h->allocs[i] == (void*)v.ec_tab) { h->allocs.erase(h->allocs.begin() + i); break; }
+    (void)hipFree(v.ec_tab);
+    v.ec_tab = nullptr;
+  }
+  h->ec_serial[0] = h->ec_serial[1] = 0;
+  h->ec_bytes = 0;
+  if (want > 0) {
+    uint32_t n = 64;
+    while (n < (uint32_t)want) n <<= 1;
+    v.ec_mask = n - 1u;
+    v.ec_ew = (2 + 2 * variant_kw(h->var) + 1 + v.A + 1 + 3) & ~3;
+    h->ec_bytes = (size_t)n * v.ec_ew * sizeof(uint32_t);
+    if (int rc = dalloc(h, &v.ec_tab, (size_t)n * v.ec_ew * v.n_nets)) return rc;
+  }
+  return 0;
+}
+static int ec_clear(caro_engine* h, hipStream_t st) {
+  if (!h->v.ec_tab) return 0;
+  HIPCHK(hipMemsetAsync(h->v.ec_tab, 0, h->ec_bytes * (size_t)h->v.n_nets, st));
+  return 0;
+}
 static int fresh_state(caro_engine* h, hipStream_t st) {
   View& v = h->v;
   const size_t T = (size_t)v.G * v.n_stores, G = (size_t)v.G;
   HIPCHK(hipMemsetAsync(v.counters, 0, sizeof(unsigned long long) * C_N * G, st));
   HIPCHK(hipMemsetAsync(v.leaf_count, 0, sizeof(int32_t) * 4, st));
-  HIPCHK(hipMemsetAsync(h->rows, 0, sizeof(int32_t) * 8, st));
+  HIPCHK(hipMemsetAsync(h->rows, 0, sizeof(int32_t) * 24, st));
   HIPCHK(hipMemsetAsync(v.g_nleaf, 0, sizeof(int32_t) * G, st));
   HIPCHK(hipMemsetAsync(v.g_pack, 0, sizeof(int32_t) * G, st));
   h->rows_par = 0;
   h->stag_batch = 0;
+  if (int rc = ec_clear(h, st)) return rc;
   const int rc = reset_games_impl(h, nullptr, st);
   if (rc) return rc;
   if (v.stag_S) {
@@ -2694,7 +2842,10 @@
   DA(v.dr_off, G); DA(v.dr_gidx, G); DA(v.dr_sel, G); DA(v.dr_tot, 2);
   DA(h->scratch, (size_t)v.maxd + 8);
   DA(h->live, 1);
-  DA(h->rows, 8);
+  DA(h->rows, 24);
+  h->ec_serial[0] = h->ec_serial[1] = 0;
+  h->ec_bytes = 0;
+  if ((rc = ec_resize(h, -1)) != 0) { caro_engine_destroy(h); return rc; }
   if (cfg->stagger > 0) {
     DA(v.lm, G); DA(v.pend, G); DA(v.wait, G); DA(v.dirty, T);
     DA(v.pk_flag, G); DA(v.pk_ply, G); DA(v.pk_final_r, G); DA(v.pk_first, G); DA(v.pk_result, G); DA(v.pk_step, G);
@@ -2706,7 +2857,7 @@
   }
 #undef DA
   HIPCHK(hipHostMalloc((void**)&h->pinned, 64, hipHostMallocDefault));
-  HIPCHK(hipHostMalloc((void**)&h->pinned64, 128, hipHostMallocDefault));
+  HIPCHK(hipHostMalloc((void**)&h->pinned64, 512, hipHostMallocDefault));
   *out = h;
   rc = fresh_state(h, nullptr);
   if (rc) { caro_engine_destroy(h); *out = nullptr; return rc; }
@@ -2896,6 +3047,26 @@
   return 0;
 }
 
+static int ec_setup(caro_engine* h, View& sv, caro_net* net0, caro_net* net1, int bthreads, hipStream_t st) {
+  sv.ec_on = 0;
+  if (!h->v.ec_tab || bthreads != 64 || !h->fused_ok) return 0;
+  int32_t rg[3];
+  if (!caro_net_cache_ranges(net0, h->v.n_nets == 2 ? net1 : nullptr, rg)) return 0;
+  caro_net* nets[2] = {net0, net1};
+  for (int c = 0; c < h->v.n_nets; ++c) {
+    const uint64_t ser = caro_net_serial(nets[c]);
+    if (h->ec_serial[c] != ser) {
+      HIPCHK(hipMemsetAsync(reinterpret_cast<char*>(h->v.ec_tab) + h->ec_bytes * c, 0, h->ec_bytes, st));
+      h->ec_serial[c] = ser;
+    }
+  }
+  sv.ec_on = 1;
+  sv.ec_lo = rg[0];
+  sv.ec_full = rg[1];
+  sv.ec_hi = rg[2];
+  return 0;
+}
+
 static int search_batch_impl(caro_engine* h, caro_net* net0, caro_net* net1, int searches, int batch, const double* noise,
                              float* planes, uint64_t* leaf_keys, float* probs, float* values, void* stream, int with_step,
                              const double* uniforms, int32_t* actions, int32_t* done, int32_t* result) {
@@ -2915,20 +3086,24 @@
   View sv = h->v;
   sv.ls_M = searches;
   if (!caro_net_uses_slot_list(net0)) sv.slot_list = nullptr;
+  if (int rc = ec_setup(h, sv, net0, net1, fused1 ? 64 : 0, st)) return rc;
+  View cv = h->v;
+  cv.ec_on = sv.ec_on; cv.ec_lo = sv.ec_lo; cv.ec_full = sv.ec_full; cv.ec_hi = sv.ec_hi;
   for (int mb = 0; mb < searches; ++mb) {
     h->prof_gate = (h->prof_ctr++ % PROF_EVERY) == 0;
     int rc = 0;
     const int32_t* counts = h->v.leaf_count;
     if (fused) {
-      int32_t* cur = h->rows + 4 * h->rows_par;
-      int32_t* nxt = h->rows + 4 * (h->rows_par ^ 1);
-      h->rows_par ^= 1;
+      int32_t* cur = h->rows + 8 * h->rows_par;
+      int32_t* nxt = h->rows + 8 * ((h->rows_par + 1) % 3);
+      const int32_t* prv = h->rows + 8 * ((h->rows_par + 2) % 3);
+      h->rows_par = (h->rows_par + 1) % 3;
       counts = cur;
       const int p1 = prof_begin(h, PK_SELECT, st);
       if (fused1) {
         DISPATCH(h->var, hipLaunchKernelGGL(k_tree<GEO>, dim3(h->v.G), dim3(128), 0, st, sv, batch, mb,
                                             noise ? noise + (size_t)mb * noise_stride : nullptr, probs, values, planes,
-                                            leaf_keys, cur, nxt, mb > 0 ? 1 : 0, 1));
+                                            leaf_keys, cur, nxt, prv, mb > 0 ? 1 : 0, 1));
       } else {
         DISPATCH(h->var, hipLaunchKernelGGL(k_tree_mw<GEO>, dim3(h->v.G), dim3(bthreads), mail_bytes<GEO>(batch), st,
                                             sv, batch, mb, noise ? noise + (size_t)mb * noise_stride : nullptr, probs,
@@ -2945,8 +3120,8 @@
     }
     const int p0 = prof_begin(h, PK_NET, st);
     if (fused)
-      rc = caro_net_forward_slot_list(net0, h->v.n_nets == 2 ? net1 : nullptr, planes, counts, h->v.g_pack,
-                                      fused1 ? nullptr : sv.slot_list, h->v.G, batch, probs, values, stream);
+      rc = caro_net_forward_slots_cached(net0, h->v.n_nets == 2 ? net1 : nullptr, planes, counts, h->v.g_pack,
+                                         fused1 ? nullptr : sv.slot_list, h->v.G, batch, probs, values, sv.ec_on, stream);
     else if (h->v.n_nets == 2)
       rc = caro_net_forward_pair_at(net0, net1, planes, counts, -1, max_rows, probs, values, stream);
     else rc = caro_net_forward(net0, planes, counts, 0, max_rows, probs, values, stream);
@@ -2956,13 +3131,14 @@
     if (rc) { h->prof_gate = 1; return rc; }
   }
   if (fused) {
-    int32_t* cur = h->rows + 4 * h->rows_par;
-    int32_t* nxt = h->rows + 4 * (h->rows_par ^ 1);
-    h->rows_par ^= 1;
+    int32_t* cur = h->rows + 8 * h->rows_par;
+    int32_t* nxt = h->rows + 8 * ((h->rows_par + 1) % 3);
+    const int32_t* prv = h->rows + 8 * ((h->rows_par + 2) % 3);
+    h->rows_par = (h->rows_par + 1) % 3;
     const int p1 = prof_begin(h, PK_EXPAND, st);
     if (fused1) {
-      DISPATCH(h->var, hipLaunchKernelGGL(k_tree<GEO>, dim3(h->v.G), dim3(128), 0, st, h->v, batch, searches,
-                                          (const double*)nullptr, probs, values, planes, leaf_keys, cur, nxt, 1, 0));
+      DISPATCH(h->var, hipLaunchKernelGGL(k_tree<GEO>, dim3(h->v.G), dim3(128), 0, st, cv, batch, searches,
+                                          (const double*)nullptr, probs, values, planes, leaf_keys, cur, nxt, prv, 1, 0));
     } else {
       DISPATCH(h->var, hipLaunchKernelGGL(k_tree_mw<GEO>, dim3(h->v.G), dim3(bthreads), 0, st, h->v, batch, searches,
                                           (const double*)nullptr, probs, values, planes, leaf_keys, cur, nxt, 1, 0,
@@ -3008,15 +3184,19 @@
   hipStream_t st = (hipStream_t)stream;
   View sv = h->v;
   if (!caro_net_uses_slot_list(net0)) sv.slot_list = nullptr;
+  if (int rc = ec_setup(h, sv, net0, net1, bthreads, st)) return rc;
+  View tv = h->v;
+  tv.ec_on = sv.ec_on; tv.ec_lo = sv.ec_lo; tv.ec_full = sv.ec_full; tv.ec_hi = sv.ec_hi;
   for (int j = 0; j < launches; ++j) {
     h->prof_gate = (h->prof_ctr++ % PROF_EVERY) == 0;
-    int32_t* cur = h->rows + 4 * h->rows_par;
-    int32_t* nxt = h->rows + 4 * (h->rows_par ^ 1);
-    h->rows_par ^= 1;
+    int32_t* cur = h->rows + 8 * h->rows_par;
+    int32_t* nxt = h->rows + 8 * ((h->rows_par + 1) % 3);
+    const int32_t* prv = h->rows + 8 * ((h->rows_par + 2) % 3);
+    h->rows_par = (h->rows_par + 1) % 3;
     const int p1 = prof_begin(h, PK_SELECT, st);
     if (bthreads == 64) {
-      DISPATCH(h->var, hipLaunchKernelGGL(k_tree_stag<GEO>, dim3(h->v.G), dim3(128), 0, st, h->v, batch, probs, values,
-                                          planes, leaf_keys, cur, nxt));
+      DISPATCH(h->var, hipLaunchKernelGGL(k_tree_stag<GEO>, dim3(h->v.G), dim3(128), 0, st, tv, batch, probs, values,
+                                          planes, leaf_keys, cur, nxt, prv));
     } else {
       DISPATCH(h->var, hipLaunchKernelGGL(k_tree_stag_mw<GEO>, dim3(h->v.G), dim3(bthreads), mail_bytes<GEO>(batch), st,
                                           sv, batch, probs, values, planes, leaf_keys, cur, nxt));
@@ -3024,9 +3204,9 @@
     prof_end(h, p1, st);
     if (hipGetLastError() != hipSuccess) { h->prof_gate = 1; return fail(CARO_E_HIP, "k_tree_stag launch failed"); }
     const int p0 = prof_begin(h, PK_NET, st);
-    const int rc = caro_net_forward_slot_list(net0, h->v.n_nets == 2 ? net1 : nullptr, planes, cur, h->v.g_pack,
-                                              bthreads == 64 ? nullptr : sv.slot_list, h->v.G, batch, probs, values,
-                                              stream);
+    const int rc = caro_net_forward_slots_cached(net0, h->v.n_nets == 2 ? net1 : nullptr, planes, cur, h->v.g_pack,
+                                                 bthreads == 64 ? nullptr : sv.slot_list, h->v.G, batch, probs, values,
+                                                 sv.ec_on, stream);
     prof_end(h, p0, st);
     prof_calibrate(h, st);
     if (rc) { h->prof_gate = 1; return rc; }
@@ -3174,11 +3354,40 @@
 int caro_counters(caro_engine* h, int64_t counters[8], void* stream) {
   if (!h || !counters) return fail(CARO_E_INVAL, "null argument");
   hipLaunchKernelGGL(k_sum_counters, dim3(1), dim3(256), 0, (hipStream_t)stream, h->v);
-  HIPCHK(hipMemcpyAsync(h->pinned64, h->v.counters_sum, C_N * sizeof(int64_t), hipMemcpyDeviceToHost,
+  HIPCHK(hipMemcpyAsync(h->pinned64 + 16, h->v.counters_sum, C_N * sizeof(int64_t), hipMemcpyDeviceToHost,
                         (hipStream_t)stream));
   HIPCHK(hipStreamSynchronize((hipStream_t)stream));
-  for (int i = 0; i < 8; ++i) counters[i] = i < C_N ? h->pinned64[i] : 0;
-  return 0;
+  for (int i = 0; i < 8; ++i) counters[i] = h->pinned64[16 + i];
+  return 0;
+}
+
+int caro_engine_cache_counters(caro_engine* h, int64_t out[4], void* stream) {
+  if (!h || !out) return fail(CARO_E_INVAL, "null argument");
+  hipStream_t st = (hipStream_t)stream;
+  hipLaunchKernelGGL(k_sum_counters, dim3(1), dim3(256), 0, st, h->v);
+  HIPCHK(hipGetLastError());
+  HIPCHK(hipMemcpyAsync(h->pinned64 + 16, h->v.counters_sum, C_N * sizeof(int64_t), hipMemcpyDeviceToHost, st));
+  HIPCHK(hipStreamSynchronize(st));
+  out[0] = h->pinned64[16 + C_CACHE_HITS];
+  out[1] = h->pinned64[16 + C_NET_ROWS];
+  out[2] = h->pinned64[16 + C_CACHE_ROWS];
+  out[3] = h->v.ec_tab ? (int64_t)h->v.ec_mask + 1 : 0;
+  return 0;
+}
+int caro_engine_set_cache(caro_engine* h, int64_t entries) {
+  if (!h) return fail(CARO_E_INVAL, "null engine");
+  if (h->select_pending) return fail(CARO_E_STATE, "caro_engine_set_cache with a pending caro_select");
+  HIPCHK(hipSetDevice(h->cfg.device_id));
+  HIPCHK(hipDeviceSynchronize());
+  if (int rc = ec_resize(h, entries)) return rc;
+  if (int rc = ec_clear(h, nullptr)) return rc;
+  HIPCHK(hipDeviceSynchronize());
+  return 0;
+}
+int caro_engine_cache_clear(caro_engine* h, void* stream) {
+  if (!h) return fail(CARO_E_INVAL, "null engine");
+  h->ec_serial[0] = h->ec_serial[1] = 0;
+  return ec_clear(h, (hipStream_t)stream);
 }
 
 int caro_leaf_counts_dev(caro_engine* h, const int32_t** counts_dev) {
diff --git a/caro_ai_amd/csrc/caro_net.hip b/caro_ai_amd/csrc/caro_net.hip
--- a/caro_ai_amd/csrc/caro_net.hip
+++ b/caro_ai_amd/csrc/caro_net.hip
@@ -326,9 +326,10 @@
   }
 }
 
+__device__ __forceinline__ int gp_mask(int v) { return (v >> 24) & 1 ? (v >> 16) & 0xFF : (1 << min(v & 0xFF, 8)) - 1; }
 template <int NTH = NT>
 __device__ __forceinline__ void tile_rows(const int32_t* __restrict__ gpack, int G, int B, int cls, int base,
-                                          int board0, int nb, int* sc, int* smap, int tid) {
+                                          int board0, int nb, int* sc, int* smap, int tid, bool use_mask = false) {
   if (!gpack) {
     if (tid < nb) smap[tid] = base + tid;
     __syncthreads();
@@ -340,7 +341,7 @@
   int mine = 0;
   for (int g = g_lo; g < g_hi; ++g) {
     const int v = gpack[g];
-    mine += (v >> 8) == cls ? (v & 0xFF) : 0;
+    mine += ((v >> 8) & 0xFF) == cls ? (use_mask ? __popc(gp_mask(v)) : (v & 0xFF)) : 0;
   }
   int inc = mine;
 #pragma unroll
@@ -355,7 +356,14 @@
   if (ex < board0 + nb && ex + mine > board0) {
     for (int g = g_lo; g < g_hi; ++g) {
       const int v = gpack[g];
-      if ((v >> 8) != cls) continue;
+      if (((v >> 8) & 0xFF) != cls) continue;
+      if (use_mask) {
+        for (int m = gp_mask(v); m; m &= m - 1) {
+          const int r = ex++ - board0;
+          if (r >= 0 && r < nb) smap[r] = g * B + __ffs(m) - 1;
+        }
+        continue;
+      }
       const int n = v & 0xFF;
       for (int j = 0; j < n; ++j) {
         const int r = ex + j - board0;
@@ -370,7 +378,7 @@
 
 constexpr int GP_PRE = 4;
 __device__ __forceinline__ void tile_rows_pre(const int (&gv)[GP_PRE], int cpt, int mine, int B, int cls, int board0,
-                                              int nb, int* sc, int* smap, int tid) {
+                                              int nb, int* sc, int* smap, int tid, bool use_mask = false) {
   const int lane = tid & 63, wave = tid >> 6;
   int inc = mine;
 #pragma unroll
@@ -386,8 +394,15 @@
 #pragma unroll
     for (int u = 0; u < GP_PRE; ++u) {
       const int v = gv[u];
-      if (u >= cpt || (v >> 8) != cls) continue;
+      if (u >= cpt || ((v >> 8) & 0xFF) != cls) continue;
       const int n = v & 0xFF, g = tid * cpt + u;
+      if (use_mask) {
+        for (int m = gp_mask(v); m; m &= m - 1) {
+          const int r = ex++ - board0;
+          if (r >= 0 && r < nb) smap[r] = g * B + __ffs(m) - 1;
+        }
+        continue;
+      }
       for (int j = 0; j < n; ++j) {
         const int r = ex + j - board0;
         if (r >= 0 && r < nb) smap[r] = g * B + j;
@@ -396,6 +411,55 @@
     }
   }
   __syncthreads();
+}
+
+__device__ __forceinline__ int tile_rows_mixed(const int (&gv)[GP_PRE], int cpt, int B, int cls, int limit, int board0,
+                                               int TB, int* sc, int* smap, int tid) {
+  const int lane = tid & 63, wave = tid >> 6;
+  int tot = 0;
+#pragma unroll
+  for (int u = 0; u < GP_PRE; ++u) tot += (u < cpt && ((gv[u] >> 8) & 0xFF) == cls) ? (gv[u] & 0xFF) : 0;
+  int inc = tot;
+#pragma unroll
+  for (int d = 1; d < 64; d <<= 1) {
+    const int t = __shfl_up(inc, d, 64);
+    if (lane >= d) inc += t;
+  }
+  if (lane == 63) sc[wave] = inc;
+  __syncthreads();
+  int T = inc - tot;
+  for (int w = 0; w < wave; ++w) T += sc[w];
+  int em[GP_PRE], mine = 0;
+#pragma unroll
+  for (int u = 0; u < GP_PRE; ++u) {
+    const int v = gv[u];
+    const bool in = u < cpt && ((v >> 8) & 0xFF) == cls;
+    const int room = min(max(limit - T, 0), 8);
+    em[u] = in ? gp_mask(v) & ((1 << room) - 1) : 0;
+    mine += __popc(em[u]);
+    T += in ? (v & 0xFF) : 0;
+  }
+  inc = mine;
+#pragma unroll
+  for (int d = 1; d < 64; d <<= 1) {
+    const int t = __shfl_up(inc, d, 64);
+    if (lane >= d) inc += t;
+  }
+  if (lane == 63) sc[32 + wave] = inc;
+  __syncthreads();
+  int ex = inc - mine, all = 0;
+  for (int w = 0; w < NT / 64; ++w) {
+    if (w < wave) ex += sc[32 + w];
+    all += sc[32 + w];
+  }
+#pragma unroll
+  for (int u = 0; u < GP_PRE; ++u)
+    for (int m = em[u]; m; m &= m - 1) {
+      const int r = ex++ - board0;
+      if (r >= 0 && r < TB) smap[r] = (tid * cpt + u) * B + __ffs(m) - 1;
+    }
+  __syncthreads();
+  return all;
 }
 
 __device__ __forceinline__ unsigned lds_addr(const void* q) {
@@ -1441,7 +1505,7 @@
                                                   const float* __restrict__ planes,
                                                   const int32_t* __restrict__ counts, int which, int row1,
                                                   float* __restrict__ probs, float* __restrict__ values,
-                                                  const int32_t* __restrict__ gpack, int gG, int gB) {
+                                                  const int32_t* __restrict__ gpack, int gG, int gB, int cmode) {
   const int lane = threadIdx.x & 63;
   const long long w = (long long)blockIdx.x * 4 + (threadIdx.x >> 6);
   long long row;
@@ -1451,7 +1515,8 @@
     if (g >= gG) return;
     const int v = gpack[g];
     if (j >= (v & 0xFF)) return;
-    cls = v >> 8;
+    if (cmode && j < 8 && !((gp_mask(v) >> j) & 1)) return;
+    cls = (v >> 8) & 0xFF;
     row = w;
   } else if (which < 2) {
     if (w >= counts[which]) return;
@@ -1483,6 +1548,7 @@
 }
 
 extern "C" void caro__set_error(const char* msg);
+static uint64_t g_net_serial = 0;
 
 struct caro_net {
   int kind;
@@ -1499,6 +1565,7 @@
   uint64_t hrows_clock;
   int64_t hrows_evictions;
   int device;
+  uint64_t serial;
   unsigned long long* dbg_stamps;
 };
 
@@ -1565,6 +1632,7 @@
   if (device_id < 0 || device_id >= ndev) return nfail(CARO_E_INVAL, "device_id out of range");
   if (hipSetDevice(device_id) != hipSuccess) return nfail(CARO_E_HIP, "hipSetDevice failed");
   caro_net* n = new caro_net();
+  n->serial = ++g_net_serial;
   n->kind = 0;
   n->salt = 0;
   n->device = device_id;
@@ -1801,6 +1869,7 @@
     return nfail(CARO_E_NODEV, "no HIP device: libcaro_hip needs a GPU (there is no CPU fallback)");
   if (device_id < 0 || device_id >= ndev) return nfail(CARO_E_INVAL, "device_id out of range");
   caro_net* n = new caro_net();
+  n->serial = ++g_net_serial;
   memset(&n->p, 0, sizeof n->p);
   n->kind = 1;
   n->salt = salt;
@@ -1852,14 +1921,14 @@
 
 static int net_launch(caro_net* n0, caro_net* n1, const float* planes_dev, const int32_t* counts_dev, int which,
                       int row1, int64_t max_rows, float* probs_dev, float* values_dev, const int32_t* gpack, int G,
-                      int B, unsigned long long* stamps, void* stream, const int32_t* slist = nullptr) {
+                      int B, unsigned long long* stamps, void* stream, const int32_t* slist = nullptr, int cmode = 0) {
   hipStream_t st = (hipStream_t)stream;
   if (n0->kind == 1) {
     const int64_t waves = gpack ? (int64_t)G * B : max_rows;
     const unsigned grid = (unsigned)((waves + 3) / 4);
     hipLaunchKernelGGL(cnet::k_net_hash, dim3(grid), dim3(256), 0, st, 2 * n0->p.HW, n0->p.A,
                        (unsigned long long)n0->salt, (unsigned long long)n1->salt, planes_dev, counts_dev, which, row1,
-                       probs_dev, values_dev, gpack, G, B);
+                       probs_dev, values_dev, gpack, G, B, cmode);
   } else {
     const unsigned grid = net_grid(n0, max_rows) + (which == 2 ? 1u : 0u);
     const bool d5 = n0->p.nres == cnet::NRES && n1->p.nres == cnet::NRES;
@@ -1877,7 +1946,7 @@
     else if (n0->p.ww)
       hipLaunchKernelGGL(d5 ? cnet::k_net_forward_w : cnet::k_net_forward_w_any, dim3(grid), dim3(cnet::NT), 0, st,
                          n0->p, n1->p, planes_dev, counts_dev, which, row1, probs_dev, values_dev,
-                         stamps ? stamps : n0->dbg_stamps, gpack, G, B);
+                         stamps ? stamps : n0->dbg_stamps, gpack, G, B, which < 2 ? cmode : 0);
     else if (n0->p.wx3) {
       const bool batched = n0->p.TB == 1 && n0->p.w_pT && n0->p.HW <= cnet::HEADS_MAX_CELLS;
       caro_net::HeadRows* hr = nullptr;
@@ -1910,6 +1979,22 @@
 }
 
 int caro_net_boards_per_workgroup(const caro_net* n) { return n ? n->p.TB : 0; }
+uint64_t caro_net_serial(const caro_net* n) { return n ? n->serial : 0; }
+int caro_net_cache_ranges(const caro_net* n0, const caro_net* n1, int32_t ranges[3]) {
+  if (!n0 || !ranges) return 0;
+  if (n0->kind == 1) {
+    if (n1 && n1->kind != 1) return 0;
+    ranges[0] = -1; ranges[1] = INT32_MAX; ranges[2] = INT32_MAX;
+    return 1;
+  }
+  if (n1 || !n0->p.ww || n0->p.ww2 || n0->p.wx3) return 0;
+  const int64_t ncu = n0->p.ncu, full = ncu > 0 ? ncu * n0->p.TB : INT32_MAX;
+  const int64_t lo = ncu > 0 ? ncu * (n0->p.TB2 > 0 ? n0->p.TB2 : n0->p.TB4 > 0 ? n0->p.TB4 : 0) : 0;
+  ranges[0] = (int32_t)lo;
+  ranges[1] = (int32_t)full;
+  ranges[2] = (int32_t)(ncu > 0 && lo > 0 ? full + lo : full);
+  return 1;
+}
 int caro_net_uses_slot_list(const caro_net* n) { return n && n->p.ww2 ? 1 : 0; }
 
 int caro_net_forward(caro_net* n, const float* planes_dev, const int32_t* counts_dev, int which, int64_t max_rows,
@@ -1959,6 +2044,22 @@
                     values_dev, gpack_dev, n_games, batch, nullptr, stream, n0->p.ww2 ? slot_list_dev : nullptr);
 }
 
+int caro_net_forward_slots_cached(caro_net* n0, caro_net* n1, const float* planes_dev, const int32_t* counts_dev,
+                                  const int32_t* gpack_dev, const int32_t* slot_list_dev, int n_games, int batch,
+                                  float* probs_dev, float* values_dev, int cached, void* stream) {
+  if (!n0 || !planes_dev || !counts_dev || !gpack_dev || !probs_dev || !values_dev)
+    return nfail(CARO_E_INVAL, "null argument");
+  if (n_games < 1 || batch < 1 || batch > 255) return nfail(CARO_E_INVAL, "bad slot geometry");
+  if (n1)
+    if (int rc = pair_ok(n0, n1)) return rc;
+  int32_t rg[3];
+  if (cached && (batch > 8 || !caro_net_cache_ranges(n0, n1, rg)))
+    return nfail(CARO_E_INVAL, "caro_net_forward_slots_cached: this net form cannot serve a cached launch (caro_net_cache_ranges)");
+  return net_launch(n0, n1 ? n1 : n0, planes_dev, counts_dev, n1 ? 2 : 0, -1, (int64_t)n_games * batch, probs_dev,
+                    values_dev, gpack_dev, n_games, batch, nullptr, stream, n0->p.ww2 ? slot_list_dev : nullptr,
+                    cached ? 1 : 0);
+}
+
 int caro_net_forward_stamped(caro_net* n, const float* planes_dev, const int32_t* counts_dev, int which,
                              int64_t max_rows, float* probs_dev, float* values_dev, uint64_t* stamps_dev,
                              void* stream) {
diff --git a/caro_ai_amd/csrc/caro_net_kernels.inc b/caro_ai_amd/csrc/caro_net_kernels.inc
--- a/caro_ai_amd/csrc/caro_net_kernels.inc
+++ b/caro_ai_amd/csrc/caro_net_kernels.inc
@@ -174,7 +174,7 @@
                                                            const int32_t* __restrict__ counts, int which, int row1,
                                                            float* __restrict__ probs, float* __restrict__ values,
                                                            unsigned long long* __restrict__ stamps,
-                                                           const int32_t* __restrict__ gpack, int gG, int gB) {
+                                                           const int32_t* __restrict__ gpack, int gG, int gB, int cmode) {
   __shared__ __attribute__((aligned(256))) float lds[LDS_FLOATS];
   float* act = lds;
   float* wbuf = lds + ACT;
@@ -191,6 +191,7 @@
   int L, row0, board0, nb, nb_cap = p0.TB;
   int ks = 1;
   bool second = false;
+  bool cuse = false, cmix = false, split_all = false, mixed = false;
   if (which < 2) {
     L = counts[which];
     row0 = which ? counts[0] : 0;
@@ -200,6 +201,7 @@
       if (p0.TB4 > 0 && L <= p0.ncu * p0.TB4) ks = 4;
       else if (p0.TB2 > 0 && L <= p0.ncu * p0.TB2) ks = 2;
       if (ks > 1) {
+        split_all = true;
         nb_cap = ks == 4 ? p0.TB4 : p0.TB2;
         board0 = (int)blockIdx.x * nb_cap;
       } else if (L > full) {
@@ -207,6 +209,7 @@
         if (p0.TB4 > 0 && over <= p0.ncu * p0.TB4) ks = 4;
         else if (p0.TB2 > 0 && over <= p0.ncu * p0.TB2) ks = 2;
         if (ks > 1) {
+          mixed = true;
           if ((int)blockIdx.x < p0.ncu) {
             ks = 1;
           } else {
@@ -216,6 +219,14 @@
         }
       }
     }
+    if (cmode && gpack && !split_all) {
+      if (!mixed) {
+        cuse = true;
+        L = counts[4 + which];
+      } else if ((int)blockIdx.x < p0.ncu && gpre) {
+        cuse = cmix = true;
+      }
+    }
   } else {
     const int L0 = counts[0], L1 = counts[1];
     if (p0.ncu > 1) {
@@ -229,6 +240,8 @@
     row0 = second ? (row1 >= 0 ? row1 : L0) : 0;
     board0 = (second ? (int)blockIdx.x - t0 : (int)blockIdx.x) * nb_cap;
   }
+  int* const smap0 = reinterpret_cast<int*>(wbuf + 2 * WCH + 1536);
+  if (cmix) L = tile_rows_mixed(gv, gcpt, gB, 0, p0.ncu * p0.TB, board0, p0.TB, smap0 + 64, smap0, (int)threadIdx.x);
   if (board0 >= L) return;
   const NetParams p = second ? p1 : p0;
   unsigned long long t_c0 = 0, t_r0 = 0;
@@ -243,7 +256,8 @@
 
   int gmine = 0;
 #pragma unroll
-  for (int u = 0; u < GP_PRE; ++u) gmine += (gv[u] >> 8) == (second ? 1 : 0) ? (gv[u] & 0xFF) : 0;
+  for (int u = 0; u < GP_PRE; ++u)
+    gmine += ((gv[u] >> 8) & 0xFF) == (second ? 1 : 0) ? (cuse ? __popc(gp_mask(gv[u])) : (gv[u] & 0xFF)) : 0;
   asm volatile("" : "+v"(gmine));
   float* win = wbuf + 2 * WCH;
   if (tid < 320) dma_b128(reinterpret_cast<const float4*>(p.w_in) + tid,
@@ -255,8 +269,9 @@
   static_assert(320 * 4 >= 9 * 2 * NF, "the 320-lane transfer must cover w_in [9][2][64]");
   asm volatile("s_waitcnt vmcnt(8)" ::: "memory");
   int* smap = reinterpret_cast<int*>(win + 1536);
-  if (gpre) tile_rows_pre(gv, gcpt, gmine, gB, second ? 1 : 0, board0, nb, smap + 64, smap, tid);
-  else tile_rows(gpack, gG, gB, second ? 1 : 0, row0 + board0, board0, nb, smap + 64, smap, tid);
+  if (cmix) __syncthreads();
+  else if (gpre) tile_rows_pre(gv, gcpt, gmine, gB, second ? 1 : 0, board0, nb, smap + 64, smap, tid, cuse);
+  else tile_rows(gpack, gG, gB, second ? 1 : 0, row0 + board0, board0, nb, smap + 64, smap, tid, cuse);
   conv_in_mfma(p, planes, smap, act, win, R, tid);
   const int slot_v = tid < nb ? smap[tid] : 0;
   unsigned long long t_trunk0 = 0;
diff --git a/caro_ai_amd/engine.py b/caro_ai_amd/engine.py
--- a/caro_ai_amd/engine.py
+++ b/caro_ai_amd/engine.py
@@ -50,7 +50,7 @@
                  node_cap=None, steps_before_tau_0=cfg.STEPS_BEFORE_TAU_0, first_player_mode=2,
                  c_puct=cfg.C_PUCT, alpha=cfg.ALPHA, explore=cfg.EXPLORE, seed=0, uid_base=0, uid_stride=None,
                  device="cuda:0", searches_hint=cfg.MCTS_SEARCHES, inference="hipw", evict=False, stagger=False,
-                 stagger_recycle=True, games_limit=0):
+                 stagger_recycle=True, games_limit=0, cache_entries=None):
         if not torch.cuda.is_available():
             raise _lib.CaroError("SelfPlayEngine needs a GPU (torch.cuda.is_available() is False); "
                                  "there is no CPU fallback")
@@ -101,6 +101,8 @@
         h = C.c_void_p()
         _lib.check(self.L.caro_engine_create(C.byref(c), C.byref(h)))
         self.h = h
+        if cache_entries is not None:
+            _lib.check(self.L.caro_engine_set_cache(self.h, int(cache_entries)))
         rows = self.G * self.max_batch
         self.planes = torch.zeros((rows,) + self.obs_shape, dtype=torch.float32, device=self.device)
         self.leaf_keys = torch.zeros((rows, self.KW), dtype=torch.int64, device=self.device)
@@ -405,6 +407,14 @@
         self._drain_open = False
         return self.drain_end()
 
+    def cache_counters(self):
+        out = (C.c_int64 * 4)()
+        _lib.check(self.L.caro_engine_cache_counters(self.h, out, self._stream()))
+        return dict(zip(("cache_hits", "net_rows", "cache_rows", "entries"), (int(x) for x in out)))
+
+    def cache_clear(self):
+        _lib.check(self.L.caro_engine_cache_clear(self.h, self._stream()))
+
     def counters(self):
         out = (C.c_int64 * 8)()
         _lib.check(self.L.caro_counters(self.h, out, self._stream()))
diff --git a/include/caro_hip.h b/include/caro_hip.h
--- a/include/caro_hip.h
+++ b/include/caro_hip.h
@@ -119,6 +119,10 @@
 int caro_drain_parked_begin_ex(caro_engine* h, int64_t cap, uint64_t* states_dev, int32_t* players_dev, double* pi_dev,
                                int32_t* z_dev, int64_t* games_dev, const caro_drain_extra* extra, void* stream);
 
+int caro_engine_cache_counters(caro_engine* h, int64_t out[4], void* stream);
+int caro_engine_cache_clear(caro_engine* h, void* stream);
+int caro_engine_set_cache(caro_engine* h, int64_t entries);
+
 int caro_counters(caro_engine* h, int64_t counters[8], void* stream);
 int caro_profile_enable(caro_engine* h, int on);
 int caro_profile_begin(caro_engine* h, int kind, void* stream);
@@ -166,6 +170,8 @@
 int64_t caro_net_stream_evictions(const caro_net* n);
 void caro_net_destroy(caro_net* n);
 int caro_net_boards_per_workgroup(const caro_net* n);
+uint64_t caro_net_serial(const caro_net* n);
+int caro_net_cache_ranges(const caro_net* n0, const caro_net* n1, int32_t ranges[3]);
 int caro_net_uses_slot_list(const caro_net* n);
 int caro_net_forward(caro_net* n, const float* planes_dev, const int32_t* counts_dev, int which, int64_t max_rows,
                      float* probs_dev, float* values_dev, void* stream);
@@ -177,6 +183,10 @@
 int caro_net_forward_slot_list(caro_net* n0, caro_net* n1, const float* planes_dev, const int32_t* counts_dev,
                                const int32_t* gpack_dev, const int32_t* slot_list_dev, int n_games, int batch,
                                float* probs_dev, float* values_dev, void* stream);
+
+int caro_net_forward_slots_cached(caro_net* n0, caro_net* n1, const float* planes_dev, const int32_t* counts_dev,
+                                  const int32_t* gpack_dev, const int32_t* slot_list_dev, int n_games, int batch,
+                                  float* probs_dev, float* values_dev, int cached, void* stream);
 
 int caro_net_create_hash(int H, int W, int A, uint64_t salt, int device_id, caro_net** out);
 
```
